# tobiashepp/torch-mednet

Hardware: AMD Instinct MI355X
Metric: 128^3 patches/sec training, 3D U-Net 32-base-ch (higher is better)
Workload: dtype bf16; 1 GPU; ResidualUNet3D f_maps=[32, 64, 128, 256] 4-class, 128^3 patches, batch 4/GPU, fwd+DiceLoss+bwd+allreduce+Adam (BASELINE config 2); global_batch=4, parallelism=dp1, graph_replay=False, gradient_exchange=none (1 rank)

## Files before the change

### include/mednet_hip.h

```cpp
#ifndef MEDNET_HIP_H
#define MEDNET_HIP_H
#include <stddef.h>
#include <stdint.h>
#ifdef __cplusplus
extern "C" {
#endif

typedef void* mednet_stream;

enum { MEDNET_F32 = 0, MEDNET_BF16 = 1,
       MEDNET_F16 = 2,
       MEDNET_U8 = 3,
       MEDNET_I64 = 4,
       MEDNET_I16 = 5   };
enum { MEDNET_NDHWC = 0, MEDNET_NCDHW = 1 };
enum { MEDNET_ACT_NONE = 0, MEDNET_ACT_RELU = 1, MEDNET_ACT_LEAKY = 2, MEDNET_ACT_ELU = 3 };
enum { MEDNET_POOL_MAX = 0, MEDNET_POOL_AVG = 1 };
enum { MEDNET_ALGO_AUTO = 0, MEDNET_ALGO_DIRECT = 1, MEDNET_ALGO_MFMA = 2, MEDNET_ALGO_EXACT = 3,
       MEDNET_ALGO_EXACT_BIT = 4,
       MEDNET_ALGO_SPLITW_BIT = 8 };
enum { MEDNET_PACK_LOW = 0x100,
       MEDNET_PACK_HIGH_ONLY = 0x200 };
enum { MEDNET_REG_L2 = 0, MEDNET_REG_L1 = 1 };
enum { MEDNET_CLASS_DICE = 0, MEDNET_CLASS_CE = 1, MEDNET_CLASS_DICE_CE = 2 };
// ... 31 lines not shown
int mednet_conv3d_cm_supported(int cin, int cout, int ksize, int x_dtype, int y_dtype, int algo);
int mednet_conv3d_act_supported(int n, int d, int h, int w, int cin, int cout, int algo);
int mednet_conv3d_act_fwd(const void* x, const void* packed, void* y, int n, int d, int h, int w, int cin, int cout,
                          int act, int algo, float* gn_partial, int dtype, mednet_stream stream);
int mednet_conv3d_dgrad_add(const void* dy, const void* packed, const void* add, void* dx, int n, int d, int h, int w,
                            int cin, int cout, int algo, int dtype, mednet_stream stream);
int mednet_conv3d_dgrad_gn_rows(int n, int d, int h, int w, int cin, int cout, int algo);
int mednet_conv3d_dgrad_gn_rows_dt(int n, int d, int h, int w, int cin, int cout, int algo, int dtype);
int mednet_conv3d_dgrad_add_supported(int n, int d, int h, int w, int cin, int cout, int algo, int dtype);
int mednet_conv3d_dgrad_gn(const void* dy, const void* packed, const void* add, void* dx, const void* gn_y,
                           const float* gn_coef, int gn_act, float* gn_partial, int n, int d, int h, int w, int cin,
                           int cout, int algo, int dtype, mednet_stream stream);
int mednet_head_dgrad_gn_rows(int n, int d, int h, int w, int cin, int dtype);
int mednet_head_dgrad_gn(const void* dy, const void* packed, void* dx, const void* gn_y, const void* gn_z, int gn_act,
                         float* gn_partial, int n, int d, int h, int w, int cin, int cout, int dtype, mednet_stream stream);
int mednet_convt3d_dgrad_gn_rows(int n, int d, int h, int w, int cin, int cout, int dtype, int algo);
int mednet_convt3d_dgrad_gn(const void* dy, const void* packed, void* dx, const void* gn_y, const void* gn_z, int gn_act,
                            float* gn_partial, int n, int d, int h, int w, int cin, int cout, int dtype, int algo,
                            mednet_stream stream);
int mednet_pool2_bwd_gn_rows(int n, int d, int h, int w, int c, int dtype);
int mednet_pool2_bwd_gn(const void* dy, const void* x, const void* add, void* dx, const void* gn_y, int gn_act,
                        float* gn_partial, int n, int d, int h, int w, int c, int mode, int dtype, mednet_stream stream);
size_t mednet_conv3d_wgrad_ws_bytes(int n, int d, int h, int w, int cin, int cout, int ksize, int workgroups);
int mednet_conv3d_wgrad_coresident(int n, int d, int h, int w, int cin, int cout, int ksize, int x_dtype, int dy_dtype, int algo);
int mednet_conv3d_wgrad_plan(int n, int d, int h, int w, int cin, int cout, int dtype, int workgroups, int* out10);
int mednet_conv3d_wgrad_c1_gn_supported(int cout, int x_dtype, int dtype);
int mednet_conv3d_wgrad_c1_gn(const void* x, const void* dz, const void* y, const float* coef, const float* bcoef, float* dw,
                              int n, int d, int h, int w, int cout, int act, int x_dtype, int dtype, void* ws, size_t ws_bytes,
                              mednet_stream stream);
int mednet_conv3d_wgrad_cm_gn_supported(int cin, int cout, int x_dtype, int dtype);
int mednet_conv3d_wgrad_cm_plan(int n, int d, int h, int w, int cin, int cout, int dtype, int gn, int* out4);
int mednet_conv3d_wgrad_cm_gn(const void* x, int x_layout, const void* dz, const void* y, const float* coef, const float* bcoef,
                              float* dw, int n, int d, int h, int w, int cin, int cout, int act, int x_dtype, int dtype, void* ws,
                              size_t ws_bytes, mednet_stream stream);
int mednet_conv3d_wgrad(const void* x, const void* dy, float* dw, float* dbias, int n, int d, int h, int w,
                        int cin, int cout, int ksize, int x_dtype, int x_layout, int dy_dtype, int dy_layout,
                        int algo, int workgroups, void* ws, size_t ws_bytes, mednet_stream stream);

int mednet_convt3d_fwd(const void* x, const void* packed, const float* bias, const void* skip, void* y, int n,
                       int d, int h, int w, int cin, int cout, int x_dtype, int y_dtype, int algo,
                       mednet_stream stream);
int mednet_convt3d_dgrad(const void* dy, const void* packed, void* dx, int n, int d, int h, int w, int cin,
                         int cout, int dy_dtype, int dx_dtype, int algo, mednet_stream stream);
size_t mednet_convt3d_wgrad_ws_bytes(int n, int d, int h, int w, int cin, int cout, int workgroups);
int mednet_convt3d_wgrad(const void* x, const void* dy, float* dw, float* dbias, int n, int d, int h, int w,
                         int cin, int cout, int x_dtype, int dy_dtype, int algo, int workgroups, void* ws,
                         size_t ws_bytes, mednet_stream stream);

size_t mednet_gn_ws_bytes(int n, int c, size_t spatial);
int mednet_gn_stats(const void* x, const float* gamma, const float* beta, float* stats, float* coef, int n,
                    size_t spatial, int c, int groups, float eps, int dtype, void* ws, size_t ws_bytes,
                    mednet_stream stream);
int mednet_gn_finalize(const float* partial, int chunks, const float* gamma, const float* beta, float* stats,
                       float* coef, int n, size_t spatial, int c, int groups, float eps, void* ws, size_t ws_bytes,
                       mednet_stream stream);
int mednet_gn_act_fwd(const void* x, const float* coef, const void* residual, void* z, int n, size_t spatial,
                      int c, int act, int x_dtype, int z_dtype, mednet_stream stream);
int mednet_gn_act_bwd(const void* dz, const void* dz2, const void* x, const void* z, const float* coef,
                      const float* stats, const float* gamma, void* dx, void* dres, float* dgamma, float* dbeta, int n,
                      size_t spatial, int c, int groups, int act, int in_act, int dtype, void* ws, size_t ws_bytes,
                      mednet_stream stream);
int mednet_gn_act_bwd_fused(const void* dz, const void* x, const float* coef, const float* stats, const float* gamma,
                            const float* partial, int rows, void* dx, float* dgamma, float* dbeta, int n,
                            size_t spatial, int c, int groups, int act, int in_act, int dtype, void* ws, size_t ws_bytes,
                            mednet_stream stream);
int mednet_gn_bwd_coefficients(const float* stats, const float* gamma, const float* partial, int rows, float* bcoef,
                               float* dgamma, float* dbeta, int n, size_t spatial, int c, int groups, void* ws,
                               size_t ws_bytes, mednet_stream stream);
int mednet_gn_act_bwd_fused_res(const void* dz, const void* x, const void* z, const float* coef, const float* stats,
                                const float* gamma, const float* fused_partial, int rows, void* dx, void* dres,
                                float* dgamma, float* dbeta, int n, size_t spatial, int c, int groups, int act, int dtype,
                                void* ws, size_t ws_bytes, mednet_stream stream);
int mednet_gn_act_bwd_fused_res_pool(const void* dy_pool, const void* skip_grad, const void* x, const void* z, const float* stats,
                                     const float* gamma, const float* fused_partial, int rows, void* dx, void* dres, float* dgamma,
                                     float* dbeta, int n, int d, int h, int w, int c, int groups, int act, int pool_mode, int dtype,
                                     void* ws, size_t ws_bytes, mednet_stream stream);
int mednet_gn_act_bwd_fused_res_head_supported(int c, int cout, int dtype, int label_dtype);
int mednet_gn_act_bwd_fused_res_head(const float* logits, const void* labels, int label_dtype, int64_t label_stride_n,
                                     const void* packed, const float* weight, const float* saved, const float* dloss, float eps,
                                     int sigmoid, int ignore_index, int class_kind, int cout, const void* x, const void* z,
                                     const float* stats, const float* gamma, const float* fused_partial, int rows, void* dx, void* dres,
                                     float* dgamma, float* dbeta, int n, size_t spatial, int c, int groups, int act, int dtype, void* ws,
                                     size_t ws_bytes, mednet_stream stream);
int mednet_bn_stats(const void* x, const float* gamma, const float* beta, float* running_mean, float* running_var,
                    long long* num_batches_tracked, float momentum, float* stats, float* coef, int n, size_t spatial, int c,
                    float eps, int dtype, void* ws, size_t ws_bytes, mednet_stream stream);
int mednet_bn_eval_coef(const float* running_mean, const float* running_var, const float* gamma, const float* beta, float* stats,
                        float* coef, int n, int c, float eps, mednet_stream stream);
int mednet_bn_act_bwd(const void* dz, const void* x, const void* z, const float* coef, const float* stats, const float* gamma,
                      void* dx, void* dres, float* dgamma, float* dbeta, int n, size_t spatial, int c, int act, int in_act,
                      int frozen, int dtype, void* ws, size_t ws_bytes, mednet_stream stream);
int mednet_bn_act_bwd_fused(const void* dz, const void* x, const float* coef, const float* stats, const float* gamma,
                            const float* partial, int rows, void* dx, float* dgamma, float* dbeta, int n, size_t spatial, int c,
                            int act, int in_act, int frozen, int dtype, void* ws, size_t ws_bytes, mednet_stream stream);

int mednet_act_fwd(const void* x, void* z, size_t count, int act, int dtype, mednet_stream stream);
int mednet_act_bwd(const void* dz, const void* z, void* dx, size_t count, int act, int dtype,
                   mednet_stream stream);
int mednet_add(const void* a, const void* b, void* out, size_t count, int dtype, mednet_stream stream);

int mednet_pool2_fwd(const void* x, void* y, int n, int d, int h, int w, int c, int mode, int dtype,
                     mednet_stream stream);
int mednet_gn_act_pool_supported(int d, int h, int w, int c, int dtype);
int mednet_gn_act_pool_fwd(const void* x, const float* coef, const void* residual, void* z, void* pooled, int n, int d, int h,
                           int w, int c, int act, int mode, int dtype, mednet_stream stream);
int mednet_pool2_bwd(const void* dy, const void* x, const void* add, void* dx, int n, int d, int h, int w, int c,
                     int mode, int dtype, mednet_stream stream);
int mednet_pool2_bwd_act(const void* dy, const void* x, const void* add, int add_channels, void* dx, int n, int d, int h, int w, int c,
                         int mode, int in_act, int dtype, mednet_stream stream);

int mednet_upcat_fwd(const void* enc, const void* x, void* out, int n, int d, int h, int w, int c_enc, int xd,
                     int xh, int xw, int c_x, int dtype, mednet_stream stream);
int mednet_upcat_stats_chunks(int n, int d, int h, int w, int c_enc, int c_x, int dtype);
int mednet_upcat_fwd_stats(const void* enc, const void* x, void* out, float* partial, int n, int d, int h, int w, int c_enc, int xd,
                           int xh, int xw, int c_x, int dtype, mednet_stream stream);
int mednet_upcat_bwd(const void* dout, void* denc, void* dx, int n, int d, int h, int w, int c_enc, int xd, int xh,
                     int xw, int c_x, int dtype, mednet_stream stream);

size_t mednet_loss_ws_bytes(int n, int c, size_t spatial);
int mednet_dice_fwd(const float* logits, const int64_t* labels, const float* weight, float* loss, float* saved,
                    float* dice_out, int n, int c, size_t spatial, int64_t stride_n, int64_t stride_c, float eps,
                    int sigmoid, int ignore_index, void* ws, size_t ws_bytes, mednet_stream stream);
int mednet_dice_bwd(const float* logits, const int64_t* labels, const float* weight, const float* saved,
                    const float* dloss, float* dlogits, int n, int c, size_t spatial, int64_t stride_n,
                    int64_t stride_c, float eps, int sigmoid, int ignore_index, mednet_stream stream);
int mednet_dice_fwd_lt(const float* logits, const void* labels, int label_dtype, int64_t label_stride_n, const float* weight,
                       float* loss, float* saved, float* dice_out, int n, int c, size_t spatial, int64_t stride_n,
                       int64_t stride_c, float eps, int sigmoid, int ignore_index, void* ws, size_t ws_bytes, mednet_stream stream);
int mednet_dice_bwd_lt(const float* logits, const void* labels, int label_dtype, int64_t label_stride_n, const float* weight,
                       const float* saved, const float* dloss, float* dlogits, int n, int c, size_t spatial, int64_t stride_n,
                       int64_t stride_c, float eps, int sigmoid, int ignore_index, mednet_stream stream);
size_t mednet_dice_ce_ws_bytes(int n, int c, size_t spatial);
int mednet_dice_ce_fwd_lt(const float* logits, const void* labels, int label_dtype, int64_t label_stride_n, const float* weight,
                          float* loss, float* saved, float* dice_out, int n, int c, size_t spatial, int64_t stride_n,
                          int64_t stride_c, float eps, void* ws, size_t ws_bytes, mednet_stream stream);
int mednet_dice_ce_bwd_lt(const float* logits, const void* labels, int label_dtype, int64_t label_stride_n, const float* weight,
                          const float* saved, const float* dloss, float* dlogits, int n, int c, size_t spatial, int64_t stride_n,
                          int64_t stride_c, float eps, mednet_stream stream);
int mednet_head_dice_supported(int cin, int cout, int dtype, int label_dtype);
size_t mednet_head_dice_ws_bytes(int n, size_t spatial, int cin, int cout);
int mednet_head_dice_gn_rows(int n, size_t spatial, int cin);
int mednet_head_dice_fwd(const void* z, const void* packed, const float* bias, const void* labels, int label_dtype,
                         int64_t label_stride_n, const float* weight, float* logits, float* loss, float* saved, int n,
                         size_t spatial, int cin, int cout, float eps, int sigmoid, int ignore_index, int z_dtype, void* ws,
                         size_t ws_bytes, mednet_stream stream);
int mednet_head_dice_bwd(const float* logits, const void* labels, int label_dtype, int64_t label_stride_n, const void* packed,
                         const float* weight, const float* saved, const float* dloss, void* dz, const void* gn_y, const void* z,
                         int gn_act, float* gn_partial, float* dw, float* dbias, int n, size_t spatial, int cin, int cout,
                         float eps, int sigmoid, int ignore_index, int z_dtype, void* ws, size_t ws_bytes, mednet_stream stream);
int mednet_head_dice_bwd_sums(const float* logits, const void* labels, int label_dtype, int64_t label_stride_n, const void* packed,
                              const float* weight, const float* saved, const float* dloss, const void* gn_y, const void* z,
                              int gn_act, float* gn_partial, float* dw, float* dbias, int n, size_t spatial, int cin, int cout,
                              float eps, int sigmoid, int ignore_index, int z_dtype, void* ws, size_t ws_bytes, mednet_stream stream);

int mednet_head_landmark_supported(int cin, int nh, int ncls, int dtype, size_t spatial);
size_t mednet_head_landmark_ws_bytes(int n, size_t spatial, int nh, int ncls);
int mednet_head_landmark_gn_rows(size_t spatial);
int mednet_head_landmark_fwd(const void* z, const void* packed, const float* bias, const void* heatmaps, int64_t heatmap_stride_n,
                             const void* labels, int64_t label_stride_n, const float* class_weight, const float* reg_weight,
                             float* logits, float* class_loss, float* reg_loss, float* saved, int n, size_t spatial, int cin, int nh,
                             int ncls, int kind, float eps, int sigmoid, int ignore_index, int z_dtype, void* ws, size_t ws_bytes,
                             mednet_stream stream);
int mednet_head_landmark_bwd(const void* z, const void* packed, const float* bias, const void* heatmaps, int64_t heatmap_stride_n,
                             const void* labels, int64_t label_stride_n, const float* class_weight, const float* reg_weight,
                             const float* saved, const float* dclass_loss, const float* dreg_loss, void* dz, const void* gn_y,
                             int gn_act, float* gn_partial, float* dw, float* dbias, int n, size_t spatial, int cin, int nh, int ncls,
                             int kind, float eps, int sigmoid, int ignore_index, int z_dtype, void* ws, size_t ws_bytes,
                             mednet_stream stream);
int mednet_head_ce_supported(int cin, int cout, int dtype, int label_dtype);
size_t mednet_head_ce_ws_bytes(int n, size_t spatial, int cin, int cout);
int mednet_head_ce_gn_rows(int n, size_t spatial, int cin);
int mednet_head_ce_fwd(const void* z, const void* packed, const float* bias, const void* labels, int label_dtype,
                       int64_t label_stride_n, const float* weight, float* logits, float* loss, float* saved, int n, size_t spatial,
                       int cin, int cout, int ignore_index, int z_dtype, void* ws, size_t ws_bytes, mednet_stream stream);
int mednet_head_ce_bwd(const float* logits, const void* labels, int label_dtype, int64_t label_stride_n, const void* packed,
                       const float* weight, const float* saved, const float* dloss, void* dz, const void* gn_y, const void* z,
                       int gn_act, float* gn_partial, float* dw, float* dbias, int n, size_t spatial, int cin, int cout,
                       int ignore_index, int z_dtype, void* ws, size_t ws_bytes, mednet_stream stream);
int mednet_head_ce_bwd_sums(const float* logits, const void* labels, int label_dtype, int64_t label_stride_n, const void* packed,
                            const float* weight, const float* saved, const float* dloss, const void* gn_y, const void* z, int gn_act,
                            float* gn_partial, float* dw, float* dbias, int n, size_t spatial, int cin, int cout, int ignore_index,
                            int z_dtype, void* ws, size_t ws_bytes, mednet_stream stream);
int mednet_head_dice_ce_supported(int cin, int cout, int dtype, int label_dtype);
size_t mednet_head_dice_ce_ws_bytes(int n, size_t spatial, int cin, int cout);
int mednet_head_dice_ce_gn_rows(int n, size_t spatial, int cin);
int mednet_head_dice_ce_fwd(const void* z, const void* packed, const float* bias, const void* labels, int label_dtype,
                            int64_t label_stride_n, const float* weight, float* logits, float* loss, float* saved, int n,
                            size_t spatial, int cin, int cout, float eps, int sigmoid, int ignore_index, int z_dtype, void* ws,
                            size_t ws_bytes, mednet_stream stream);
int mednet_head_dice_ce_bwd(const float* logits, const void* labels, int label_dtype, int64_t label_stride_n, const void* packed,
                            const float* weight, const float* saved, const float* dloss, void* dz, const void* gn_y, const void* z,
                            int gn_act, float* gn_partial, float* dw, float* dbias, int n, size_t spatial, int cin, int cout,
                            float eps, int sigmoid, int ignore_index, int z_dtype, void* ws, size_t ws_bytes, mednet_stream stream);
int mednet_head_dice_ce_bwd_sums(const float* logits, const void* labels, int label_dtype, int64_t label_stride_n, const void* packed,
                                 const float* weight, const float* saved, const float* dloss, const void* gn_y, const void* z,
                                 int gn_act, float* gn_partial, float* dw, float* dbias, int n, size_t spatial, int cin, int cout,
                                 float eps, int sigmoid, int ignore_index, int z_dtype, void* ws, size_t ws_bytes, mednet_stream stream);
int mednet_head_landmark_cls_fwd(const void* z, const void* packed, const float* bias, const void* heatmaps, int64_t heatmap_stride_n,
                                 const void* labels, int64_t label_stride_n, const float* class_weight, const float* reg_weight,
                                 float* logits, float* class_loss, float* reg_loss, float* saved, float* dice_metric, int n,
                                 size_t spatial, int cin, int nh, int ncls, int kind, int class_kind, float eps, int sigmoid,
                                 int ignore_index, int z_dtype, void* ws, size_t ws_bytes, mednet_stream stream);
int mednet_head_landmark_cls_bwd(const void* z, const void* packed, const float* bias, const void* heatmaps, int64_t heatmap_stride_n,
                                 const void* labels, int64_t label_stride_n, const float* class_weight, const float* reg_weight,
                                 const float* saved, const float* dclass_loss, const float* dreg_loss, void* dz, const void* gn_y,
                                 int gn_act, float* gn_partial, float* dw, float* dbias, int n, size_t spatial, int cin, int nh,
                                 int ncls, int kind, int class_kind, float eps, int sigmoid, int ignore_index, int z_dtype, void* ws,
                                 size_t ws_bytes, mednet_stream stream);
int mednet_head_seg_supported(int cin, int ncls, int dtype, int label_dtype, size_t spatial);
size_t mednet_head_seg_ws_bytes(int n, size_t spatial, int ncls);
int mednet_head_seg_gn_rows(size_t spatial);
int mednet_head_seg_fwd(const void* z, const void* packed, const float* bias, const void* labels, int64_t label_stride_n,
                        const float* class_weight, float* logits, float* loss, float* saved, int n, size_t spatial, int cin,
                        int ncls, int class_kind, float eps, int sigmoid, int ignore_index, int z_dtype, void* ws, size_t ws_bytes,
                        mednet_stream stream);
int mednet_head_seg_bwd(const void* z, const void* packed, const float* bias, const void* labels, int64_t label_stride_n,
                        const float* class_weight, const float* saved, const float* dloss, void* dz, const void* gn_y, int gn_act,
                        float* gn_partial, float* dw, float* dbias, int n, size_t spatial, int cin, int ncls, int class_kind,
                        float eps, int sigmoid, int ignore_index, int z_dtype, void* ws, size_t ws_bytes, mednet_stream stream);
int mednet_ds_head_supported(int cin, int ncls, int dtype, int label_dtype, int d, int h, int w, int shift);
size_t mednet_ds_head_ws_bytes(int n, int d, int h, int w, int cin, int ncls);
int mednet_ds_head_gn_rows(int d, int h, int w, int cin, int dtype);
int mednet_ds_head_fwd(const void* z, const void* packed, const float* bias, const void* labels, int label_dtype,
                       int64_t label_stride_n, const float* class_weight, float* loss, float* saved, int n, int d, int h, int w, int D,
                       int H, int W, int shift, int cin, int ncls, int class_kind, float eps, int sigmoid, int ignore_index, int z_dtype,
                       void* ws, size_t ws_bytes, mednet_stream stream);
int mednet_ds_head_bwd(const void* z, const void* packed, const float* bias, const void* labels, int label_dtype,
                       int64_t label_stride_n, const float* class_weight, const float* saved, const float* dloss, const void* d_pass,
                       void* dz, const void* gn_y, int gn_act, float* gn_partial, float* dw, float* dbias, int n, int d, int h, int w,
                       int D, int H, int W, int shift, int cin, int ncls, int class_kind, float eps, int sigmoid, int ignore_index,
                       int z_dtype, void* ws, size_t ws_bytes, mednet_stream stream);
int mednet_ce_fwd(const float* logits, const int64_t* labels, const float* weight, float* loss, float* saved,
                  int n, int c, size_t spatial, int64_t stride_n, int64_t stride_c, int ignore_index, void* ws,
                  size_t ws_bytes, mednet_stream stream);
int mednet_ce_bwd(const float* logits, const int64_t* labels, const float* weight, const float* saved,
                  const float* dloss, float* dlogits, int n, int c, size_t spatial, int64_t stride_n,
// ... 117 lines not shown
```

### torch-mednet_amd/csrc/conv.h

```cpp
#pragma once
#include <type_traits>

#include "common.h"

namespace mednet {

enum { MAP_CONV = 0, MAP_CT_FWD = 1, MAP_CT_DG = 2 };

struct ConvGeom {
  int n, od, oh, ow;
  int id, ih, iw;
  int k, m;
  int ks;
  int in_planar, out_planar;
};

struct WgradGeom {
  int n, ad, ah, aw;
  int bd, bh, bw;
  int ka, kb, ks, stride2;
  int a_planar, b_planar;
  size_t chunk;
};


template <int MAP>
int launch_direct(const void* x, const float* P, const float* bias, const void* skip, void* y, const ConvGeom& g,
                  int x_dtype, int y_dtype, hipStream_t s);
size_t wgrad_direct_ws_bytes(size_t nvox, int ka, int kb, int ks);
int launch_wgrad_direct(const void* A, const void* B, float* dw, WgradGeom g, int a_dtype, int b_dtype, void* ws,
                        size_t ws_bytes, hipStream_t s);
size_t channel_sum_ws_bytes(int n, size_t spatial, int c);
int launch_channel_sum(const void* x, float* out, int n, size_t spatial, int c, int planar, int dtype, void* ws,
                       size_t ws_bytes, hipStream_t s);
bool head_dgrad_supported(int cin, int cout, int ksize, int x_dtype, int x_layout, int y_layout);
int launch_head_dgrad(const void* dy, const float* Pb, void* dz, int n, size_t spatial, int m, int k, int out_dtype,
                      hipStream_t s);
int head_dgrad_gn_rows(size_t spatial, int k, int dtype);
int launch_head_dgrad_gn(const void* dy, const float* Pb, void* dz, const void* gy, const void* gz, int act, float* partial,
                         int n, size_t spatial, int m, int k, int dtype, hipStream_t s);
bool head_vox_supported(int k);
int launch_head_fwd_vox(const void* z, const float* Pb, const float* bias, float* y, int n, size_t spatial, int k, int m,
                        int z_dtype, hipStream_t s);
bool wgrad_1x1_supported(int cin, int cout, int ksize, int x_layout, int dy_layout, int dy_dtype);
size_t wgrad_1x1_ws_bytes(int n, size_t spatial, int cin, int cout);
int launch_wgrad_1x1(const void* z, const void* dy, float* dw, int n, size_t spatial, int cin, int cout, int z_dtype,
                     void* ws, size_t ws_bytes, hipStream_t s);
bool wgrad_c1_supported(int cin, int cout, int ksize, int x_layout, int dy_layout);
size_t wgrad_c1_ws_bytes(int n, int d, int h, int w, int cout);
bool wgrad_c1_gn_supported(int cout, int x_dtype, int dtype);
int launch_wgrad_c1_gn(const void* x, const void* dz, const void* y, const float* coef, const float* bcoef, int act, float* dw,
                       int n, int d, int h, int w, int cout, int x_dtype, int dtype, void* ws, size_t ws_bytes, hipStream_t s);
int launch_wgrad_c1(const void* x, const void* dy, float* dw, int n, int d, int h, int w, int cout, int x_dtype,
                    int dy_dtype, void* ws, size_t ws_bytes, hipStream_t s, bool split_bf16 = false);
bool wgrad_cm_supported(int cin, int cout, int ksize, int x_dtype, int dy_dtype, int dy_layout);
bool wgrad_cm_gn_supported(int cin, int cout, int x_dtype, int dtype);
size_t wgrad_cm_ws_bytes(int n, int d, int h, int w, int cin, int cout);
int wgrad_cm_plan(int n, int d, int h, int w, int cin, int cout, int dtype, bool gn, int* out4);
int launch_wgrad_cm(const void* x, int x_layout, const void* dz, const void* y, const float* coef, const float* bcoef, int act,
                    float* dw, int n, int d, int h, int w, int cin, int cout, int dtype, void* ws, size_t ws_bytes, hipStream_t s);
int launch_pack_f32(const float* w, float* Pf, float* Pb, int cin, int cout, int T, int transposed_src, hipStream_t s);

int launch_hm_finalize(const float* partial, const float* cweight, float* loss, int n, int c, int nblocks, size_t spatial,
                       hipStream_t s);
int launch_dice_finalize(const float* partial, const float* weight, float* loss, float* saved, int c, int nblocks, float eps,
                         hipStream_t s, float* dice_out = nullptr);
int launch_ce_finalize(const float* partial, float* loss, float* saved, int nblocks, hipStream_t s);
int launch_dice_ce_finalize(const float* partial, const float* partial_ce, const float* weight, float* loss, float* saved, int c,
                            int nblocks, float eps, hipStream_t s, float* dice_out = nullptr);
int launch_class_finalize(int kind, const float* dice_partial, const float* ce_partial, const float* weight, float* loss, float* saved,
                          int c, int rows, float eps, hipStream_t s);
inline int launch_class_finalize(int kind, const float* partial, const float* weight, float* loss, float* saved, int c, int rows,
                                 float eps, hipStream_t s) {
  const float* ce_partial = kind == MEDNET_CLASS_DICE_CE ? partial + (size_t)rows * c * 2 : partial;
  return launch_class_finalize(kind, partial, ce_partial, weight, loss, saved, c, rows, eps, s);
}

template <class F>
inline void for_class_kind(int ce, F&& f) {
  if (ce == MEDNET_CLASS_DICE_CE) f(std::integral_constant<int, MEDNET_CLASS_DICE_CE>{});
  else if (ce) f(std::integral_constant<int, MEDNET_CLASS_CE>{});
  else f(std::integral_constant<int, MEDNET_CLASS_DICE>{});
}
#define MEDNET_CLASS_KIND_NAME(ce, STEM, DIR) ((ce) == MEDNET_CLASS_DICE_CE ? STEM "_dice_ce" DIR : (ce) ? STEM "_ce" DIR : STEM DIR)

#include "conv_mfma_decl.inc"
inline const float* head_weights_f32(const void* packed, int cin, int cout) {
  return (const float*)((const char*)packed + pack_layout(cin, cout, 1).f32_bwd);
}

bool conv_f32_mfma_enabled();
int launch_conv_f32_mfma(const void* x, const float* P, const float* bias, void* y, int n, int d, int h, int w, int k, int m,
                         hipStream_t s);
int launch_convt_dgrad_f32_mfma(const void* dy, const float* Pb, void* dx, int n, int d, int h, int w, int cin, int cout,
                                hipStream_t s);
int launch_convt_fwd_f32_mfma(const void* x, const float* Pf, const float* bias, const void* skip, void* y, int n, int d, int h,
                              int w, int cin, int cout, hipStream_t s);
size_t wgrad_f32_mfma_ws_bytes(int n, int d, int h, int w, int ka, int kb, int stride2);
int launch_wgrad_f32_mfma(const void* x, const void* dy, float* dw, int n, int d, int h, int w, int cin, int cout, void* ws,
                          size_t ws_bytes, hipStream_t s);
int launch_convt_wgrad_f32_mfma(const void* x, const void* dy, float* dw, int n, int d, int h, int w, int cin, int cout, void* ws,
                                size_t ws_bytes, hipStream_t s);

bool conv_x3_enabled();
bool conv_x3_supported(int cin, int cout, int ksize);
bool conv_x3_fits(int d, int h, int w, int c);
int conv_x3_stats_rows(int n, int d, int h, int w, int cout);
int launch_conv_x3(const void* x, const void* sec_hi, size_t lo_delta, const float* bias, void* y, int n, int d, int h, int w, int k,
                   int m, float* stats, hipStream_t s);
bool conv_c1_x3_supported(int cin, int cout, int ksize);
int conv_c1_x3_stats_rows(int d, int h, int w);
int launch_conv_c1_x3(const void* x, const float* w_pf, const float* bias, void* y, int n, int d, int h, int w, int cout,
                      float* stats, hipStream_t s);
int launch_conv_x3_dgrad(const void* dy, const void* sec_hi, size_t lo_delta, void* dx, int n, int d, int h, int w, int k, int m,
                         const void* add, const void* gn_y, const float* gn_coef, int gn_act, float* gn_partial, hipStream_t s);
int launch_convt_dgrad_x3(const void* dy, const void* sec_hi, size_t lo_delta, void* dx, int n, int d, int h, int w, int cin,
                          int cout, hipStream_t s);
int launch_convt_fwd_x3(const void* x, const void* sec_hi, size_t lo_delta, const float* bias, const void* skip, void* y, int n,
                        int d, int h, int w, int cin, int cout, hipStream_t s);
size_t wgrad_x3_ws_bytes(int n, int d, int h, int w, int cin, int cout, int workgroups);
bool wgrad_c1_x3_supported(int cout, int x_dtype, int dy_dtype);
int wgrad_c1_x3_blocks(int n, int d, int h, int w);
int launch_wgrad_c1_x3(const void* x, const void* dy, float* part, int n, int d, int h, int w, hipStream_t s);
int launch_wgrad_x3(const void* x, const void* dy, float* dw, int n, int d, int h, int w, int cin, int cout, void* ws,
                    size_t ws_bytes, hipStream_t s, int workgroups);

size_t convt_wgrad_x3_ws_bytes(int n, int d, int h, int w, int cin, int cout, int workgroups);
int launch_convt_wgrad_x3(const void* x, const void* dy, float* dw, int n, int d, int h, int w, int cin, int cout, void* ws,
                          size_t ws_bytes, hipStream_t s, int workgroups);

}
```

### torch-mednet_amd/csrc/head_loss.hip

```cpp
#include "common.h"
#include "conv.h"
#include "loss_blocks.inc"

namespace mednet {

constexpr int HL_BLOCK_VOX = 256 * 8;
constexpr int HL_MAXC = 4;
constexpr int HL_VPT = 32;

template <typename T>
struct Raw8;
template <>
struct Raw8<bf16> {
  bf16x8 r;
  __device__ __forceinline__ void load(const bf16* p, size_t i) { r = *reinterpret_cast<const bf16x8*>(p + i); }
  __device__ __forceinline__ float at(int j) const { return (float)r[j]; }
};
template <>
struct Raw8<f16> {
  f16x8 r;
  __device__ __forceinline__ void load(const f16* p, size_t i) { r = *reinterpret_cast<const f16x8*>(p + i); }
  __device__ __forceinline__ float at(int j) const { return (float)r[j]; }
};
template <>
struct Raw8<float> {
  f32x4 a, b;
  __device__ __forceinline__ void load(const float* p, size_t i) {
    a = *reinterpret_cast<const f32x4*>(p + i);
    b = *reinterpret_cast<const f32x4*>(p + i + 4);
  }
  __device__ __forceinline__ float at(int j) const { return j < 4 ? a[j] : b[j - 4]; }
};

template <typename TI, int K, typename TL, int KIND = MEDNET_CLASS_DICE>
__global__ __launch_bounds__(256) void head_dice_fwd_kernel(const TI* __restrict__ z, const float* __restrict__ Pb ,
                                                            const float* __restrict__ bias, const TL* __restrict__ lab,
                                                            int64_t lab_sn, float* __restrict__ y, float* __restrict__ partial,
                                                            size_t spatial, int m, int sigmoid, int ignore,
                                                            const float* __restrict__ cw = nullptr) {
  __shared__ float scratch[4];
  const int n = blockIdx.y;
  ClassSums<HL_MAXC> sums;
  const size_t v0 = (size_t)blockIdx.x * HL_BLOCK_VOX;
  for (int it = 0; it < 8; ++it) {
    const size_t v = v0 + (size_t)it * 256 + threadIdx.x;
    if (v < spatial) {
      float zv[K];
#pragma unroll
      for (int q = 0; q < K / 8; ++q) {
        const F8 t = ld8(z, ((size_t)n * spatial + v) * K + q * 8);
#pragma unroll
        for (int j = 0; j < 8; ++j) zv[q * 8 + j] = t.v[j];
      }
      const int yl = label_at(lab, (size_t)n * lab_sn + v, ignore);
      float lg[HL_MAXC];
#pragma unroll
      for (int i = 0; i < HL_MAXC; ++i) {
        lg[i] = 0.f;
        if (i < m) {
          float s0 = bias ? bias[i] : 0.f, s1 = 0.f;
#pragma unroll
          for (int j = 0; j < K; j += 2) {
            s0 = fmaf(zv[j], Pb[(size_t)i * K + j], s0);
            s1 = fmaf(zv[j + 1], Pb[(size_t)i * K + j + 1], s1);
          }
          lg[i] = s0 + s1;
          y[((size_t)n * m + i) * spatial + v] = lg[i];
        }
      }
      class_fwd_voxel<KIND, HL_MAXC>(sums, [&](int k) { return lg[k]; }, yl, m, sigmoid, ignore, cw);
    }
  }
  class_fwd_writeout<KIND, HL_MAXC>(sums, partial, m, scratch);
}

template <typename TO, int K, typename TL, bool FOLD = false, int KIND = MEDNET_CLASS_DICE, bool STORE = true>
__global__ __launch_bounds__(256, (sizeof(TO) == 2 && !FOLD) ? 3 : 2) void head_dice_bwd_kernel(const float* __restrict__ lgs, const TL* __restrict__ lab, int64_t lab_sn,
                                                            const float* __restrict__ Pb , const float* __restrict__ weight,
                                                            const float* __restrict__ saved, const float* __restrict__ dloss,
                                                            float eps, int sigmoid, int ignore, TO* __restrict__ dz,
                                                            const TO* __restrict__ gy , const TO* __restrict__ gz, int act,
                                                            float* __restrict__ gn_partial , float* __restrict__ wpart,
                                                            size_t spatial, int m) {
  constexpr int CG = K / 8, VPW = 256 / CG;
  const int n = blockIdx.y;
  const int cgi = threadIdx.x % CG, vi = threadIdx.x / CG;
  float wreg[HL_MAXC][8];
#pragma unroll
  for (int i = 0; i < HL_MAXC; ++i)
#pragma unroll
    for (int j = 0; j < 8; ++j) wreg[i][j] = i < m ? Pb[(size_t)i * K + cgi * 8 + j] : 0.f;
  const float go = *dloss;
  std::conditional_t<KIND == MEDNET_CLASS_DICE_CE, ClassCoefLds<HL_MAXC>, ClassCoefRegs<HL_MAXC>> coef;
  if constexpr (KIND == MEDNET_CLASS_DICE_CE) {
    __shared__ float hk_s[3 * HL_MAXC];
    coef.row = hk_s;
    if (threadIdx.x < HL_MAXC) coef.template fill<KIND>(threadIdx.x, m, weight, saved, eps, go);
    __syncthreads();
  } else {
    coef.template fill<KIND>(m, weight, saved, eps, go);
  }
  float ss[8], sq[8], wacc[HL_MAXC][8], bacc[HL_MAXC];
#pragma unroll
  for (int j = 0; j < 8; ++j) ss[j] = sq[j] = 0.f;
#pragma unroll
  for (int i = 0; i < HL_MAXC; ++i) {
    bacc[i] = 0.f;
#pragma unroll
    for (int j = 0; j < 8; ++j) wacc[i][j] = 0.f;
  }
  const size_t v0 = (size_t)blockIdx.x * (VPW * HL_VPT) + vi;
  for (int it = 0; it < HL_VPT; it += 2) {
    const size_t v = v0 + (size_t)it * VPW;
    if (v >= spatial) break;
    const size_t vb = v + VPW;
    const bool hb = (it + 1 < HL_VPT) && vb < spatial;
    const size_t vbs = hb ? vb : v;
    float la[HL_MAXC], lb[HL_MAXC];
    [[maybe_unused]] float oa = 0.f, ob = 0.f;
    if constexpr (CG == 4) {
      const int cq = threadIdx.x & 3;
      oa = cq < m ? lgs[((size_t)n * m + cq) * spatial + v] : 0.f;
      ob = cq < m ? lgs[((size_t)n * m + cq) * spatial + vbs] : 0.f;
      static_assert(HL_MAXC == 4, "one class per lane of a quad");
    } else {
#pragma unroll
      for (int i = 0; i < HL_MAXC; ++i) {
        la[i] = i < m ? lgs[((size_t)n * m + i) * spatial + v] : 0.f;
        lb[i] = i < m ? lgs[((size_t)n * m + i) * spatial + vbs] : 0.f;
      }
    }
    const int ya = label_at(lab, (size_t)n * lab_sn + v, ignore), yb = label_at(lab, (size_t)n * lab_sn + vbs, ignore);
    const size_t rowa = ((size_t)n * spatial + v) * K + cgi * 8, rowb = ((size_t)n * spatial + vbs) * K + cgi * 8;
    Raw8<TO> zva, zvb, yva, yvb;
    zva.load(gz, rowa);
    zvb.load(gz, rowb);
    if (!STORE || gy) {
      yva.load(gy, rowa);
      yvb.load(gy, rowb);
    } else {
      yva = zva;
      yvb = zvb;
    }
    if constexpr (KIND == MEDNET_CLASS_DICE_CE) asm volatile("" : "+v"(coef.off));
    float (&da)[HL_MAXC] = la, (&db)[HL_MAXC] = lb;
    if constexpr (CG == 4) {
      class_logit_grad_quad<KIND>(da, db, oa, ob, ya, yb, m, sigmoid, ignore, coef);
    } else {
      class_logit_grad<KIND, HL_MAXC>(da, ya, m, sigmoid, ignore, coef);
// ... 20 lines not shown
      for (int j = 0; j < 8; ++j) {
        za[j] = zva.at(j);
        zb[j] = zvb.at(j);
      }
      act_grad_n<8>(t.v, za, act);
      act_grad_n<8>(u.v, zb, act);
    }
    if constexpr (STORE) {
      st8(dz, rowa, t);
      if (hb) st8(dz, rowb, u);
    }
    if (!FOLD && (!STORE || gy)) {
      float za[8], zb[8];
#pragma unroll
      for (int j = 0; j < 8; ++j) {
        za[j] = zva.at(j);
        zb[j] = zvb.at(j);
      }
      act_grad_n<8>(t.v, za, act);
      act_grad_n<8>(u.v, zb, act);
#pragma unroll
      for (int j = 0; j < 8; ++j) {
        ss[j] += t.v[j] + u.v[j];
        sq[j] = fmaf(u.v[j], yvb.at(j), fmaf(t.v[j], yva.at(j), sq[j]));
      }
    }
  }
  const int lane = threadIdx.x & 63, wave = threadIdx.x >> 6;
  const size_t wrow = ((size_t)n * gridDim.x + blockIdx.x) * 4 + wave;
  if (gn_partial) {
    float* out = gn_partial + wrow * K * 2 + cgi * 16;
#pragma unroll
    for (int j = 0; j < 8; ++j) {
      const float a = lane_class_sum<CG>(ss[j]), b = lane_class_sum<CG>(sq[j]);
      if (lane < CG) {
        out[2 * j] = a;
        out[2 * j + 1] = b;
      }
    }
  }
  float* wout = wpart + wrow * ((size_t)m * K + m);
#pragma unroll
  for (int i = 0; i < HL_MAXC; ++i) {
    if (i < m) {
#pragma unroll
      for (int j = 0; j < 8; ++j) {
        const float a = lane_class_sum<CG>(wacc[i][j]);
        if (lane < CG) wout[(size_t)i * K + cgi * 8 + j] = a;
      }
      const float b = lane_class_sum<CG>(bacc[i]);
      if (lane == 0) wout[(size_t)m * K + i] = b;
    }
  }
}

constexpr int HL_WF_GROUPS = 128;
__global__ __launch_bounds__(192) void head_dice_wfinal1_kernel(const float* __restrict__ wpart, double* __restrict__ part2, int rows,
                                                                int width) {
  const int per = (rows + HL_WF_GROUPS - 1) / HL_WF_GROUPS;
  const int r0 = blockIdx.x * per, r1 = r0 + per < rows ? r0 + per : rows;
  for (int e = threadIdx.x; e < width; e += 192) {
    double s0 = 0.0, s1 = 0.0, s2 = 0.0, s3 = 0.0;
    int r = r0;
    for (; r + 3 < r1; r += 4) {
      s0 += (double)wpart[(size_t)r * width + e];
      s1 += (double)wpart[(size_t)(r + 1) * width + e];
      s2 += (double)wpart[(size_t)(r + 2) * width + e];
      s3 += (double)wpart[(size_t)(r + 3) * width + e];
    }
    for (; r < r1; ++r) s0 += (double)wpart[(size_t)r * width + e];
    part2[(size_t)blockIdx.x * width + e] = (s0 + s1) + (s2 + s3);
  }
}
__global__ __launch_bounds__(192) void head_dice_wfinal2_kernel(const double* __restrict__ part2, float* __restrict__ dw,
                                                                float* __restrict__ dbias, int width, int mk) {
  for (int e = threadIdx.x; e < width; e += 192) {
    double s = 0.0;
    for (int g = 0; g < HL_WF_GROUPS; ++g) s += part2[(size_t)g * width + e];
    if (e < mk) dw[e] = (float)s;
    else if (dbias) dbias[e - mk] = (float)s;
  }
}

static inline unsigned hl_fwd_blocks(size_t spatial) { return (unsigned)((spatial + HL_BLOCK_VOX - 1) / HL_BLOCK_VOX); }
static inline unsigned hl_bwd_blocks(size_t spatial, int k) {
  const size_t per_wg = (size_t)(256 / (k / 8)) * HL_VPT;
  return (unsigned)((spatial + per_wg - 1) / per_wg);
}

}

using namespace mednet;

extern "C" int mednet_head_dice_supported(int cin, int cout, int dtype, int label_dtype) {
  return (cin == 16 || cin == 32 || cin == 64) && cout >= 1 && cout <= HL_MAXC && dtype_ok(dtype) &&
         (label_dtype == MEDNET_U8 || label_dtype == MEDNET_I64) && tuning_option("head_loss_fuse", 1);
}
extern "C" size_t mednet_head_dice_ws_bytes(int n, size_t spatial, int cin, int cout) {
  const size_t fwd = ((size_t)n * hl_fwd_blocks(spatial) * cout * 2 + 64) * sizeof(float);
  const size_t width = (size_t)cout * cin + cout;
  const size_t bwd = ((size_t)n * hl_bwd_blocks(spatial, cin) * 4 * width + 64) * sizeof(float) + (size_t)HL_WF_GROUPS * width * sizeof(double) + 16;
  return fwd > bwd ? fwd : bwd;
}
extern "C" int mednet_head_dice_gn_rows(int n, size_t spatial, int cin) {
  (void)n;
  return 4 * (int)hl_bwd_blocks(spatial, cin);
}
extern "C" size_t mednet_head_dice_ce_ws_bytes(int n, size_t spatial, int cin, int cout) {
  const size_t fwd = ((size_t)n * hl_fwd_blocks(spatial) * ((size_t)cout * 2 + 2) + 64) * sizeof(float);
  const size_t bwd = mednet_head_dice_ws_bytes(n, spatial, cin, cout);
  return fwd > bwd ? fwd : bwd;
}

template <int KIND>
static int head_loss_fwd(const char* what, const void* z, const void* packed, const float* bias, const void* labels, int label_dtype,
                         int64_t label_stride_n, const float* weight, float* logits, float* loss, float* saved, int n, size_t spatial,
                         int cin, int cout, float eps, int sigmoid, int ignore_index, int z_dtype, void* ws, size_t ws_bytes,
                         mednet_stream stream) {
  MEDNET_REQUIRE(mednet_head_dice_supported(cin, cout, z_dtype, label_dtype), MEDNET_E_UNSUPPORTED,
                 "%s: %d -> %d classes, dtype %d, labels %d", what, cin, cout, z_dtype, label_dtype);
  MEDNET_REQUIRE(n > 0 && spatial > 0 && z && packed && labels && logits && loss && saved, MEDNET_E_SHAPE, "%s: bad arguments", what);
  const size_t need = KIND == MEDNET_CLASS_DICE_CE ? mednet_head_dice_ce_ws_bytes(n, spatial, cin, cout) : mednet_head_dice_ws_bytes(n, spatial, cin, cout);
  MEDNET_REQUIRE(ws_bytes >= need, MEDNET_E_WORKSPACE, "%s: workspace too small", what);
  const float* Pb = head_weights_f32(packed, cin, cout);
  hipStream_t s = (hipStream_t)stream;
  const unsigned nb = hl_fwd_blocks(spatial);
  float* partial = (float*)ws;
  const dim3 grid(nb, n);
#define HF(TI_, K_, TL_) hipLaunchKernelGGL((head_dice_fwd_kernel<TI_, K_, TL_, KIND>), grid, dim3(256), 0, s, (const TI_*)z, Pb, bias, (const TL_*)labels, label_stride_n, logits, partial, spatial, cout, sigmoid, ignore_index, KIND != MEDNET_CLASS_DICE ? weight : nullptr)
#define HF_L(TI_, K_) do { if (label_dtype == MEDNET_U8) HF(TI_, K_, uint8_t); else HF(TI_, K_, int64_t); } while (0)
#define HF_K(TI_) do { if (cin == 16) HF_L(TI_, 16); else if (cin == 32) HF_L(TI_, 32); else HF_L(TI_, 64); } while (0)
  if (z_dtype == MEDNET_F32) HF_K(float);
  else if (z_dtype == MEDNET_BF16) HF_K(bf16);
  else HF_K(f16);
#undef HF_K
#undef HF_L
#undef HF
  int rc = check_launch(what);
  if (rc) return rc;
  return launch_class_finalize(KIND, partial, weight, loss, saved, cout, (int)(nb * n), eps, s);
}

template <int KIND>
static int head_loss_bwd(const char* what, const float* logits, const void* labels, int label_dtype, int64_t label_stride_n,
                         const void* packed, const float* weight, const float* saved, const float* dloss, void* dz, const void* gn_y,
                         const void* z, int gn_act, float* gn_partial, float* dw, float* dbias, int n, size_t spatial, int cin, int cout,
                         float eps, int sigmoid, int ignore_index, int z_dtype, void* ws, size_t ws_bytes, mednet_stream stream,
                         bool store = true) {
  MEDNET_REQUIRE(mednet_head_dice_supported(cin, cout, z_dtype, label_dtype), MEDNET_E_UNSUPPORTED,
                 "%s: %d -> %d classes, dtype %d, labels %d", what, cin, cout, z_dtype, label_dtype);
  MEDNET_REQUIRE(n > 0 && spatial > 0 && logits && labels && packed && saved && dloss && (dz || !store) && z && dw, MEDNET_E_SHAPE, "%s: bad arguments", what);
  MEDNET_REQUIRE(store || (cin == 32 && z_dtype != MEDNET_F32), MEDNET_E_UNSUPPORTED, "%s: 32 features in 16-bit storage, not %d in dtype %d", what, cin, z_dtype);
  MEDNET_REQUIRE(store || (gn_y && gn_partial), MEDNET_E_SHAPE, "%s: gn_y and gn_partial are required", what);
  MEDNET_REQUIRE((gn_y == nullptr) == (gn_partial == nullptr), MEDNET_E_SHAPE, "%s: gn_y and gn_partial go together", what);
  const size_t need = KIND == MEDNET_CLASS_DICE_CE ? mednet_head_dice_ce_ws_bytes(n, spatial, cin, cout) : mednet_head_dice_ws_bytes(n, spatial, cin, cout);
  MEDNET_REQUIRE(ws_bytes >= need, MEDNET_E_WORKSPACE, "%s: workspace too small", what);
  const float* Pb = head_weights_f32(packed, cin, cout);
  hipStream_t s = (hipStream_t)stream;
  const unsigned nb = hl_bwd_blocks(spatial, cin);
  float* wpart = (float*)ws;
  const dim3 grid(nb, n);
  const bool fold = gn_y == nullptr && gn_act != MEDNET_ACT_NONE;
#define HB_(TO_, K_, TL_, F_) hipLaunchKernelGGL((head_dice_bwd_kernel<TO_, K_, TL_, F_, KIND>), grid, dim3(256), 0, s, logits, (const TL_*)labels, label_stride_n, Pb, weight, saved, dloss, eps, sigmoid, ignore_index, (TO_*)dz, (const TO_*)gn_y, (const TO_*)z, gn_act, gn_partial, wpart, spatial, cout)
#define HB(TO_, K_, TL_) do { if (fold) HB_(TO_, K_, TL_, true); else HB_(TO_, K_, TL_, false); } while (0)
#define HB_L(TO_, K_) do { if (label_dtype == MEDNET_U8) HB(TO_, K_, uint8_t); else HB(TO_, K_, int64_t); } while (0)
#define HB_K(TO_) do { if (cin == 16) HB_L(TO_, 16); else if (cin == 32) HB_L(TO_, 32); else HB_L(TO_, 64); } while (0)
#define HB_S(TO_, TL_) hipLaunchKernelGGL((head_dice_bwd_kernel<TO_, 32, TL_, false, KIND, false>), grid, dim3(256), 0, s, logits, (const TL_*)labels, label_stride_n, Pb, weight, saved, dloss, eps, sigmoid, ignore_index, (TO_*)nullptr, (const TO_*)gn_y, (const TO_*)z, gn_act, gn_partial, wpart, spatial, cout)
#define HB_SL(TO_) do { if (label_dtype == MEDNET_U8) HB_S(TO_, uint8_t); else HB_S(TO_, int64_t); } while (0)
  if (!store) {
    if (z_dtype == MEDNET_BF16) HB_SL(bf16);
    else HB_SL(f16);
  } else if (z_dtype == MEDNET_F32) HB_K(float);
  else if (z_dtype == MEDNET_BF16) HB_K(bf16);
  else HB_K(f16);
#undef HB_SL
#undef HB_S
#undef HB_K
#undef HB_L
#undef HB_
#undef HB
  int rc = check_launch(what);
  if (rc) return rc;
  const int width = cout * cin + cout, rows = (int)(n * nb * 4);
  double* part2 = (double*)((char*)ws + (((size_t)rows * width + 64) * sizeof(float) + 7) / 8 * 8);
  hipLaunchKernelGGL(head_dice_wfinal1_kernel, dim3(HL_WF_GROUPS), dim3(192), 0, s, wpart, part2, rows, width);
  hipLaunchKernelGGL(head_dice_wfinal2_kernel, dim3(1), dim3(192), 0, s, part2, dw, dbias, width, cout * cin);
  return check_launch("head_dice_wfinal");
}

extern "C" int mednet_head_dice_fwd(const void* z, const void* packed, const float* bias, const void* labels, int label_dtype,
                                    int64_t label_stride_n, const float* weight, float* logits, float* loss, float* saved, int n,
                                    size_t spatial, int cin, int cout, float eps, int sigmoid, int ignore_index, int z_dtype,
                                    void* ws, size_t ws_bytes, mednet_stream stream) {
  return head_loss_fwd<MEDNET_CLASS_DICE>("head_dice_fwd", z, packed, bias, labels, label_dtype, label_stride_n, weight, logits, loss, saved, n, spatial,
                              cin, cout, eps, sigmoid, ignore_index, z_dtype, ws, ws_bytes, stream);
}

extern "C" int mednet_head_dice_bwd(const float* logits, const void* labels, int label_dtype, int64_t label_stride_n,
                                    const void* packed, const float* weight, const float* saved, const float* dloss, void* dz,
                                    const void* gn_y, const void* z, int gn_act, float* gn_partial, float* dw, float* dbias, int n,
                                    size_t spatial, int cin, int cout, float eps, int sigmoid, int ignore_index, int z_dtype,
                                    void* ws, size_t ws_bytes, mednet_stream stream) {
  return head_loss_bwd<MEDNET_CLASS_DICE>("head_dice_bwd", logits, labels, label_dtype, label_stride_n, packed, weight, saved, dloss, dz, gn_y, z, gn_act,
                              gn_partial, dw, dbias, n, spatial, cin, cout, eps, sigmoid, ignore_index, z_dtype, ws, ws_bytes, stream);
}

extern "C" int mednet_head_dice_bwd_sums(const float* logits, const void* labels, int label_dtype, int64_t label_stride_n,
                                         const void* packed, const float* weight, const float* saved, const float* dloss,
                                         const void* gn_y, const void* z, int gn_act, float* gn_partial, float* dw, float* dbias, int n,
                                         size_t spatial, int cin, int cout, float eps, int sigmoid, int ignore_index, int z_dtype,
                                         void* ws, size_t ws_bytes, mednet_stream stream) {
  return head_loss_bwd<MEDNET_CLASS_DICE>("head_dice_bwd_sums", logits, labels, label_dtype, label_stride_n, packed, weight, saved, dloss, nullptr, gn_y, z,
                              gn_act, gn_partial, dw, dbias, n, spatial, cin, cout, eps, sigmoid, ignore_index, z_dtype, ws, ws_bytes, stream, false);
}

extern "C" int mednet_head_ce_supported(int cin, int cout, int dtype, int label_dtype) {
  return mednet_head_dice_supported(cin, cout, dtype, label_dtype);
}
extern "C" size_t mednet_head_ce_ws_bytes(int n, size_t spatial, int cin, int cout) {
  return mednet_head_dice_ws_bytes(n, spatial, cin, cout);
}
extern "C" int mednet_head_ce_gn_rows(int n, size_t spatial, int cin) { return mednet_head_dice_gn_rows(n, spatial, cin); }

extern "C" int mednet_head_ce_fwd(const void* z, const void* packed, const float* bias, const void* labels, int label_dtype,
                                  int64_t label_stride_n, const float* weight, float* logits, float* loss, float* saved, int n,
                                  size_t spatial, int cin, int cout, int ignore_index, int z_dtype, void* ws, size_t ws_bytes,
                                  mednet_stream stream) {
  return head_loss_fwd<MEDNET_CLASS_CE>("head_ce_fwd", z, packed, bias, labels, label_dtype, label_stride_n, weight, logits, loss, saved, n, spatial,
                             cin, cout, 0.f, 0, ignore_index, z_dtype, ws, ws_bytes, stream);
}

extern "C" int mednet_head_ce_bwd(const float* logits, const void* labels, int label_dtype, int64_t label_stride_n, const void* packed,
                                  const float* weight, const float* saved, const float* dloss, void* dz, const void* gn_y, const void* z,
                                  int gn_act, float* gn_partial, float* dw, float* dbias, int n, size_t spatial, int cin, int cout,
                                  int ignore_index, int z_dtype, void* ws, size_t ws_bytes, mednet_stream stream) {
  return head_loss_bwd<MEDNET_CLASS_CE>("head_ce_bwd", logits, labels, label_dtype, label_stride_n, packed, weight, saved, dloss, dz, gn_y, z, gn_act,
                             gn_partial, dw, dbias, n, spatial, cin, cout, 0.f, 0, ignore_index, z_dtype, ws, ws_bytes, stream);
}

extern "C" int mednet_head_ce_bwd_sums(const float* logits, const void* labels, int label_dtype, int64_t label_stride_n, const void* packed,
                                       const float* weight, const float* saved, const float* dloss, const void* gn_y, const void* z,
                                       int gn_act, float* gn_partial, float* dw, float* dbias, int n, size_t spatial, int cin, int cout,
                                       int ignore_index, int z_dtype, void* ws, size_t ws_bytes, mednet_stream stream) {
  return head_loss_bwd<MEDNET_CLASS_CE>("head_ce_bwd_sums", logits, labels, label_dtype, label_stride_n, packed, weight, saved, dloss, nullptr, gn_y, z, gn_act,
                             gn_partial, dw, dbias, n, spatial, cin, cout, 0.f, 0, ignore_index, z_dtype, ws, ws_bytes, stream, false);
}

extern "C" int mednet_head_dice_ce_supported(int cin, int cout, int dtype, int label_dtype) {
  return mednet_head_dice_supported(cin, cout, dtype, label_dtype);
}
extern "C" int mednet_head_dice_ce_gn_rows(int n, size_t spatial, int cin) { return mednet_head_dice_gn_rows(n, spatial, cin); }

extern "C" int mednet_head_dice_ce_fwd(const void* z, const void* packed, const float* bias, const void* labels, int label_dtype,
                                       int64_t label_stride_n, const float* weight, float* logits, float* loss, float* saved, int n,
                                       size_t spatial, int cin, int cout, float eps, int sigmoid, int ignore_index, int z_dtype,
                                       void* ws, size_t ws_bytes, mednet_stream stream) {
  MEDNET_REQUIRE(sigmoid == 0 && ignore_index == MEDNET_NO_IGNORE, MEDNET_E_UNSUPPORTED,
                 "head_dice_ce_fwd: Dice + cross-entropy is a softmax form without ignore_index");
  return head_loss_fwd<MEDNET_CLASS_DICE_CE>("head_dice_ce_fwd", z, packed, bias, labels, label_dtype, label_stride_n, weight, logits, loss, saved, n,
                                   spatial, cin, cout, eps, 0, MEDNET_NO_IGNORE, z_dtype, ws, ws_bytes, stream);
}

extern "C" int mednet_head_dice_ce_bwd(const float* logits, const void* labels, int label_dtype, int64_t label_stride_n,
                                       const void* packed, const float* weight, const float* saved, const float* dloss, void* dz,
                                       const void* gn_y, const void* z, int gn_act, float* gn_partial, float* dw, float* dbias, int n,
                                       size_t spatial, int cin, int cout, float eps, int sigmoid, int ignore_index, int z_dtype,
                                       void* ws, size_t ws_bytes, mednet_stream stream) {
  MEDNET_REQUIRE(sigmoid == 0 && ignore_index == MEDNET_NO_IGNORE, MEDNET_E_UNSUPPORTED,
                 "head_dice_ce_bwd: Dice + cross-entropy is a softmax form without ignore_index");
  return head_loss_bwd<MEDNET_CLASS_DICE_CE>("head_dice_ce_bwd", logits, labels, label_dtype, label_stride_n, packed, weight, saved, dloss, dz, gn_y, z,
                                   gn_act, gn_partial, dw, dbias, n, spatial, cin, cout, eps, 0, MEDNET_NO_IGNORE, z_dtype, ws, ws_bytes,
                                   stream);
}

extern "C" int mednet_head_dice_ce_bwd_sums(const float* logits, const void* labels, int label_dtype, int64_t label_stride_n,
                                            const void* packed, const float* weight, const float* saved, const float* dloss,
                                            const void* gn_y, const void* z, int gn_act, float* gn_partial, float* dw, float* dbias,
                                            int n, size_t spatial, int cin, int cout, float eps, int sigmoid, int ignore_index,
                                            int z_dtype, void* ws, size_t ws_bytes, mednet_stream stream) {
  MEDNET_REQUIRE(sigmoid == 0 && ignore_index == MEDNET_NO_IGNORE, MEDNET_E_UNSUPPORTED,
// ... 6 lines not shown
```

### torch-mednet_amd/csrc/loss_blocks.inc

```
#pragma once

namespace mednet {

template <typename TL>
__device__ __forceinline__ int label_at(const TL* __restrict__ lab, size_t i, int ignore) {
  const int64_t y = (int64_t)lab[i];
  if (y == (int64_t)(int)y) return (int)y;
  return ignore == -1 ? -2 : -1;
}

template <int MAXC>
__device__ __forceinline__ void cl_keep_branch() {
  if constexpr (MAXC > 4) asm volatile("");
}

template <int MAXC, class Z>
__device__ __forceinline__ float cl_load_max(float* p, Z&& logit, int c, int y, float& zy) {
  float mx = -INFINITY;
#pragma unroll
  for (int k = 0; k < MAXC; ++k)
    if (k < c) {
      cl_keep_branch<MAXC>();
      p[k] = logit(k);
      mx = fmaxf(mx, p[k]);
      if (k == y) zy = p[k];
    }
  return mx;
}
template <int MAXC>
__device__ __forceinline__ float cl_exp_sum(float* p, int c, float mx) {
  float den = 0.f;
#pragma unroll
  for (int k = 0; k < MAXC; ++k)
    if (k < c) {
      cl_keep_branch<MAXC>();
      p[k] = expf(p[k] - mx);
      den += p[k];
    }
  return den;
}
template <int MAXC, class Z>
__device__ __forceinline__ void cl_probs(float* p, Z&& logit, int c, int sigmoid) {
  if (sigmoid) {
#pragma unroll
    for (int k = 0; k < MAXC; ++k)
      if (k < c) p[k] = 1.f / (1.f + expf(-logit(k)));
  } else {
    [[maybe_unused]] float zy;
    const float mx = cl_load_max<MAXC>(p, logit, c, -1, zy);
    const float den = cl_exp_sum<MAXC>(p, c, mx);
    const float inv = 1.f / den;
#pragma unroll
    for (int k = 0; k < MAXC; ++k)
      if (k < c) p[k] *= inv;
  }
}

template <int MAXC>
struct ClassSums {
  float I[MAXC], D[MAXC];
  float num = 0.f, den = 0.f;
  bool bad = false;
  __device__ __forceinline__ ClassSums() {
#pragma unroll
    for (int k = 0; k < MAXC; ++k) I[k] = D[k] = 0.f;
  }
};

template <int MAXC>
__device__ __forceinline__ void cl_dice_terms_masked(ClassSums<MAXC>& a, const float* p, int y, int c, int ignore) {
#pragma unroll
  for (int k = 0; k < MAXC; ++k)
    if (k < c) {
      cl_keep_branch<MAXC>();
      const float t = (k == y) ? 1.f : 0.f;
      const float m = (ignore != MEDNET_NO_IGNORE && t == (float)ignore) ? 0.f : 1.f;
      a.I[k] = fmaf(p[k] * m, t * m, a.I[k]);
      a.D[k] += (p[k] + t) * m;
    }
}
template <int MAXC>
__device__ __forceinline__ void cl_dice_terms(ClassSums<MAXC>& a, float* p, float inv, int y, int c) {
#pragma unroll
  for (int k = 0; k < MAXC; ++k)
    if (k < c) {
      cl_keep_branch<MAXC>();
      p[k] *= inv;
      const float t = (k == y) ? 1.f : 0.f;
      a.I[k] = fmaf(p[k], t, a.I[k]);
      a.D[k] += p[k] + t;
    }
}
template <int MAXC>
__device__ __forceinline__ void cl_ce_term(ClassSums<MAXC>& a, const float* __restrict__ weight, int y, float mx, float s, float zy) {
  const float w = weight ? weight[y] : 1.f;
  a.num = fmaf(w, (mx + logf(s)) - zy, a.num);
  a.den += w;
}

template <int KIND, int MAXC, class Z>
__device__ __forceinline__ void class_fwd_voxel(ClassSums<MAXC>& a, Z&& logit, int y, int c, int sigmoid, int ignore,
                                                const float* __restrict__ weight) {
  const bool ok = (unsigned)y < (unsigned)c;
  if constexpr (KIND == MEDNET_CLASS_CE) {
    if (y != ignore && !ok) a.num = __builtin_nanf("");
    if (y != ignore && ok) {
      float mx = -INFINITY, zy = 0.f;
#pragma unroll
      for (int k = 0; k < MAXC; ++k)
        if (k < c) {
          cl_keep_branch<MAXC>();
          const float z = logit(k);
          mx = fmaxf(mx, z);
          if (k == y) zy = z;
        }
      float s = 0.f;
#pragma unroll
      for (int k = 0; k < MAXC; ++k)
        if (k < c) s += expf(logit(k) - mx);
      cl_ce_term<MAXC>(a, weight, y, mx, s, zy);
    }
  } else {
    float p[MAXC];
    a.bad |= !ok;
    if constexpr (KIND == MEDNET_CLASS_DICE_CE) {
      float zy = 0.f;
      const float mx = cl_load_max<MAXC>(p, logit, c, y, zy);
      const float den = cl_exp_sum<MAXC>(p, c, mx);
      const float inv = 1.f / den;
      cl_dice_terms<MAXC>(a, p, inv, y, c);
      if (ok) cl_ce_term<MAXC>(a, weight, y, mx, den, zy);
    } else {
      cl_probs<MAXC>(p, logit, c, sigmoid);
      cl_dice_terms_masked<MAXC>(a, p, y, c, ignore);
    }
  }
}

// ... 152 lines not shown
```

### torch-mednet_amd/csrc/norm_act.hip

```cpp
#include "common.h"
#include "conv.h"
#include "loss_blocks.inc"

#include <type_traits>

#ifndef GN_NT
#define GN_NT 1
#endif
#ifndef GN_WAVES
#define GN_WAVES 3
#endif
namespace mednet {

template <int VEC>
struct Cols {
  int cols, rows, col, row;
  bool active;
  __device__ __forceinline__ Cols(int c) {
    cols = c / VEC;
    rows = 256 / cols;
    active = (int)threadIdx.x < rows * cols;
    col = threadIdx.x % cols;
    row = threadIdx.x / cols;
  }
// ... 196 lines not shown
    b += (double)p0.y;
  }
  a = wave_sum((a + a1) + (a2 + a3));
  b = wave_sum((b + b1) + (b2 + b3));
  if (threadIdx.x == 0) {
    const int g = cc / (c / groups);
    const double mean = stats[((size_t)n * groups + g) * 2], rstd = stats[((size_t)n * groups + g) * 2 + 1];
    csum[((size_t)n * c + cc) * 2] = (float)a;
    csum[((size_t)n * c + cc) * 2 + 1] = (float)(rstd * (b - mean * a));
  }
}

__global__ __launch_bounds__(1024) void gn_finalize_kernel(const float* __restrict__ partial,
                                                           const float* __restrict__ gamma,
                                                           const float* __restrict__ beta, float* __restrict__ stats,
                                                           float* __restrict__ coef, int c, int groups, int chunks,
                                                           double count, float eps, const void* __restrict__ pivot_x,
                                                           size_t sample_stride, int dtype) {
  __shared__ double sh[2][16];
  const int n = blockIdx.x / groups, g = blockIdx.x % groups;
  const int cg = c / groups, lane = threadIdx.x & 63, wv = threadIdx.x >> 6;
  const int nt = (int)blockDim.x, nwv = nt >> 6;
  double s = 0.0, q = 0.0;
  const float* base = partial + (size_t)n * chunks * c * 2 + (size_t)g * cg * 2;
  const size_t row = (size_t)c * 2;
  if (cg % 2 == 0) {
    auto add_row = [&](const float* p, double& ss, double& qq) {
      for (int i = 0; i < cg / 2; ++i) {
        const f32x4 v = *reinterpret_cast<const f32x4*>(p + 4 * i);
        ss += (double)v[0] + (double)v[2];
        qq += (double)v[1] + (double)v[3];
      }
    };
    double s1 = 0.0, q1 = 0.0, s2 = 0.0, q2 = 0.0, s3 = 0.0, q3 = 0.0;
    int ch = threadIdx.x;
    for (; ch + 3 * nt < chunks; ch += 4 * nt) {
      add_row(base + (size_t)ch * row, s, q);
      add_row(base + (size_t)(ch + nt) * row, s1, q1);
      add_row(base + (size_t)(ch + 2 * nt) * row, s2, q2);
      add_row(base + (size_t)(ch + 3 * nt) * row, s3, q3);
    }
    for (; ch < chunks; ch += nt) add_row(base + (size_t)ch * row, s, q);
    s = (s + s1) + (s2 + s3);
    q = (q + q1) + (q2 + q3);
  } else {
    for (int ch = threadIdx.x; ch < chunks; ch += nt) {
      const float* p = base + (size_t)ch * row;
      for (int i = 0; i < cg; ++i) {
        s += (double)p[2 * i];
        q += (double)p[2 * i + 1];
      }
    }
  }
  s = wave_sum(s);
  q = wave_sum(q);
  if (lane == 0) {
    sh[0][wv] = s;
    sh[1][wv] = q;
  }
  __syncthreads();
  s = q = 0.0;
  for (int k = 0; k < nwv; ++k) {
    s += sh[0][k];
    q += sh[1][k];
  }
  const double ms = s / count;
  const double mean = (double)pivot_of(pivot_x, (size_t)n * sample_stride + (size_t)g * cg, dtype) + ms;
  double var = q / count - ms * ms;
  if (var < 0.0) var = 0.0;
  const float rstd = (float)(1.0 / sqrt(var + (double)eps));
  if (threadIdx.x == 0) {
    stats[((size_t)n * groups + g) * 2] = (float)mean;
    stats[((size_t)n * groups + g) * 2 + 1] = rstd;
  }
  for (int i = threadIdx.x; i < cg; i += nt) {
    const int cc = g * cg + i;
    const float ga = gamma ? gamma[cc] : 1.f, be = beta ? beta[cc] : 0.f;
    const float a = ga * rstd;
    coef[((size_t)n * c + cc) * 2] = a;
    coef[((size_t)n * c + cc) * 2 + 1] = be - (float)mean * a;
  }
}

template <typename TX, typename TZ, int VEC>
__global__ __launch_bounds__(256) void gn_act_fwd_kernel(const TX* __restrict__ x, const float* __restrict__ coef,
                                                         const TZ* __restrict__ res, TZ* __restrict__ z,
                                                         size_t spatial, int c, int act, size_t chunk_vox) {
  const Cols<VEC> L(c);
  if (!L.active) return;
  const int n = blockIdx.y;
  const size_t v0 = (size_t)blockIdx.x * chunk_vox;
  const size_t v1 = v0 + chunk_vox < spatial ? v0 + chunk_vox : spatial;
  float a[VEC], b[VEC];
#pragma unroll
  for (int k = 0; k < VEC; ++k) {
    a[k] = coef[((size_t)n * c + L.col * VEC + k) * 2];
    b[k] = coef[((size_t)n * c + L.col * VEC + k) * 2 + 1];
  }
  const size_t off = (size_t)n * spatial * c + (size_t)L.col * VEC;
  auto one = [&](const F8& xin, const F8& rin, F8& out) {
#pragma unroll
    for (int k = 0; k < VEC; ++k) {
      out.v[k] = fmaf(a[k], xin.v[k], b[k]);
      if (res) out.v[k] += rin.v[k];
    }
    act_apply_n<VEC>(out.v, act);
  };
  size_t v = v0 + L.row;
  const size_t R = (size_t)L.rows;
  for (; v + 3 * R < v1; v += 4 * R) {
    size_t i[4];
    F8 xi[4], ri[4], zo[4];
#pragma unroll
    for (int u = 0; u < 4; ++u) i[u] = off + (v + u * R) * c;
#pragma unroll
    for (int u = 0; u < 4; ++u) xi[u] = VecIO<TX, VEC>::load(x, i[u]);
    if (res) {
#pragma unroll
      for (int u = 0; u < 4; ++u) ri[u] = VecIO<TZ, VEC>::load(res, i[u]);
    }
#pragma unroll
    for (int u = 0; u < 4; ++u) one(xi[u], ri[u], zo[u]);
#pragma unroll
    for (int u = 0; u < 4; ++u) VecIO<TZ, VEC>::store(z, i[u], zo[u]);
  }
  for (; v < v1; v += R) {
    const size_t i = off + v * c;
    const F8 xv = VecIO<TX, VEC>::load(x, i);
    F8 rv, zv;
    if (res) rv = VecIO<TZ, VEC>::load(res, i);
    one(xv, rv, zv);
    VecIO<TZ, VEC>::store(z, i, zv);
  }
}

template <typename T, int VEC>
__global__ __launch_bounds__(256, GN_WAVES) void gn_bwd_partial_kernel(const T* __restrict__ dz, const T* __restrict__ dz2,
                                                             const T* __restrict__ x, const T* __restrict__ z,
                                                             const float* __restrict__ coef,
                                                             const float* __restrict__ stats,
                                                             float* __restrict__ partial, size_t spatial, int c,
                                                             int groups, int act, size_t chunk_vox, int rpw) {
  __shared__ float lds[256 * 2 * VEC];
  const Cols<VEC> L(c);
  const int n = blockIdx.y;
  const size_t v0 = (size_t)blockIdx.x * chunk_vox;
  const size_t v1 = v0 + chunk_vox < spatial ? v0 + chunk_vox : spatial;
  float acc[2 * VEC];
#pragma unroll
  for (int k = 0; k < 2 * VEC; ++k) acc[k] = 0.f;
  if (L.active) {
    const int cg = c / groups;
    float mean[VEC], rstd[VEC], ca[VEC], cb[VEC];
#pragma unroll
    for (int k = 0; k < VEC; ++k) {
      const int g = (L.col * VEC + k) / cg;
      mean[k] = stats[((size_t)n * groups + g) * 2];
      rstd[k] = stats[((size_t)n * groups + g) * 2 + 1];
      ca[k] = z ? 0.f : coef[((size_t)n * c + L.col * VEC + k) * 2];
      cb[k] = z ? 0.f : coef[((size_t)n * c + L.col * VEC + k) * 2 + 1];
    }
    const size_t off = (size_t)n * spatial * c + (size_t)L.col * VEC;
    auto one = [&](size_t i) {
      F8 g1 = VecIO<T, VEC>::load(dz, i);
      F8 g2, zv;
      if (dz2) g2 = VecIO<T, VEC>::load(dz2, i);
      if (act != MEDNET_ACT_NONE && z) zv = VecIO<T, VEC>::load(z, i);
      const F8 xv = VecIO<T, VEC>::load(x, i);
      if (dz2) {
#pragma unroll
        for (int k = 0; k < VEC; ++k) g1.v[k] += g2.v[k];
      }
      if (z) {
        act_grad_n<VEC>(g1.v, zv.v, act);
      } else {
#pragma unroll
        for (int k = 0; k < VEC; ++k) zv.v[k] = fmaf(ca[k], xv.v[k], cb[k]);
        act_grad_pre_n<VEC>(g1.v, zv.v, act);
      }
#pragma unroll
      for (int k = 0; k < VEC; ++k) {
        const float xh = (xv.v[k] - mean[k]) * rstd[k];
        acc[2 * k] += g1.v[k];
        acc[2 * k + 1] = fmaf(g1.v[k], xh, acc[2 * k + 1]);
      }
    };
    size_t v = v0 + L.row;
    for (; v + (size_t)L.rows < v1; v += 2 * (size_t)L.rows) {
      one(off + v * c);
      one(off + (v + L.rows) * c);
// ... 562 lines not shown

template <typename T, typename TL, int KIND>
__global__ __launch_bounds__(256, GN_WAVES) void gn_bwd_apply_head_kernel(const float* __restrict__ lgs, const TL* __restrict__ lab,
                                                                          int64_t lab_sn, const float* __restrict__ Pb ,
                                                                          const float* __restrict__ weight, const float* __restrict__ saved,
                                                                          const float* __restrict__ dloss, float eps, int sigmoid, int ignore,
                                                                          int m, const T* __restrict__ x, const T* __restrict__ z,
                                                                          const float* __restrict__ bcoef, T* __restrict__ dx,
                                                                          T* __restrict__ dres, size_t spatial, int act, size_t chunk_vox,
                                                                          GnParamGrad pg) {
  constexpr int C = 32, VEC = 8, MAXC = 4, ROWS = 256 / (C / VEC);
  static_assert(sizeof(T) == 2, "16-bit storage");
  if (pg.csum && blockIdx.x == 0 && blockIdx.y == 0) {
    for (int cc = threadIdx.x; cc < C; cc += 256) {
      double a = 0.0, b = 0.0;
      for (int i = 0; i < pg.n; ++i) {
        a += (double)pg.csum[((size_t)i * C + cc) * 2];
        b += (double)pg.csum[((size_t)i * C + cc) * 2 + 1];
      }
      if (pg.dbeta) pg.dbeta[cc] = (float)a;
      if (pg.dgamma) pg.dgamma[cc] = (float)b;
    }
  }
  const int n = blockIdx.y, col = threadIdx.x & 3, row = threadIdx.x >> 2;
  const size_t v0 = (size_t)blockIdx.x * chunk_vox;
  const size_t v1 = v0 + chunk_vox < spatial ? v0 + chunk_vox : spatial;
  float k1[VEC], k2[VEC], k3[VEC], wreg[MAXC][VEC];
#pragma unroll
  for (int k = 0; k < VEC; ++k) {
    const float* o = bcoef + ((size_t)n * C + col * VEC + k) * 3;
    k1[k] = o[0];
    k2[k] = o[1];
    k3[k] = o[2];
#pragma unroll
    for (int i = 0; i < MAXC; ++i) wreg[i][k] = i < m ? Pb[(size_t)i * C + col * VEC + k] : 0.f;
  }
  const float go = *dloss;
  std::conditional_t<KIND == MEDNET_CLASS_DICE_CE, ClassCoefLds<MAXC>, ClassCoefRegs<MAXC>> coef;
  if constexpr (KIND == MEDNET_CLASS_DICE_CE) {
    __shared__ float hk_s[3 * MAXC];
    coef.row = hk_s;
    if (threadIdx.x < MAXC) coef.template fill<KIND>(threadIdx.x, m, weight, saved, eps, go);
    __syncthreads();
  } else {
    coef.template fill<KIND>(m, weight, saved, eps, go);
  }
  const size_t off = (size_t)n * spatial * C + (size_t)col * VEC;
  auto finish = [&](size_t i, F8& g1, const F8& zv, const F8& xv) {
    act_grad_n<VEC>(g1.v, zv.v, act);
    F8 o;
#pragma unroll
    for (int k = 0; k < VEC; ++k) {
      float xf = xv.v[k];
      asm volatile("" : "+v"(xf));
      o.v[k] = fmaf(k1[k], g1.v[k], fmaf(k2[k], xf, k3[k]));
      asm volatile("" : "+v"(o.v[k]));
    }
    VecIO<T, VEC>::store(dx, i, o);
    VecIO<T, VEC>::store(dres, i, g1);
  };
  auto two = [&](size_t va, size_t vb, bool hb) {
    const float oa = col < m ? lgs[((size_t)n * m + col) * spatial + va] : 0.f;
    const float ob = col < m ? lgs[((size_t)n * m + col) * spatial + vb] : 0.f;
    const int ya = label_at(lab, (size_t)n * lab_sn + va, ignore), yb = label_at(lab, (size_t)n * lab_sn + vb, ignore);
    const size_t ia = off + va * C, ib = off + vb * C;
    F8 zva, zvb;
    if (act != MEDNET_ACT_NONE) {
      zva = VecIO<T, VEC>::load(z, ia);
      zvb = VecIO<T, VEC>::load(z, ib);
    }
    const F8 xva = VecIO<T, VEC>::load_last(x, ia), xvb = VecIO<T, VEC>::load_last(x, ib);
    if constexpr (KIND == MEDNET_CLASS_DICE_CE) asm volatile("" : "+v"(coef.off));
    float da[MAXC], db[MAXC];
    class_logit_grad_quad<KIND>(da, db, oa, ob, ya, yb, m, sigmoid, ignore, coef);
    F8 ga, gb;
    head_dz_row<T, MAXC>(ga.v, da, wreg, m);
    head_dz_row<T, MAXC>(gb.v, db, wreg, m);
    finish(ia, ga, zva, xva);
    if (hb) finish(ib, gb, zvb, xvb);
  };
  size_t v = v0 + row;
  for (; v + (size_t)ROWS < v1; v += 2 * (size_t)ROWS) two(v, v + ROWS, true);
  for (; v < v1; v += ROWS) two(v, v, false);
}

__device__ __forceinline__ int nearest_src(int dst, int in, int out) {
  const float scale = (float)in / (float)out;
  const int s = (int)floorf((float)dst * scale);
  return s < in - 1 ? s : in - 1;
}
template <typename T, int VEC>
__global__ __launch_bounds__(256) void upcat_fwd_kernel(const T* __restrict__ enc, const T* __restrict__ x,
                                                        T* __restrict__ out, int n, int d, int h, int w, int ce, int xd,
                                                        int xh, int xw, int cx) {
  const int ct = ce + cx, pv = ct / VEC;
  const size_t total = (size_t)n * d * h * w * pv;
  const size_t i = (size_t)blockIdx.x * 256 + threadIdx.x;
  if (i >= total) return;
  const int cc = (int)(i % pv) * VEC;
  size_t v = i / pv;
  if (cc < ce) {
    VecIO<T, VEC>::store(out, v * ct + cc, VecIO<T, VEC>::load(enc, v * ce + cc));
    return;
  }
  const int ox = (int)(v % w);
  size_t r = v / w;
  const int oy = (int)(r % h);
  r /= h;
  const int oz = (int)(r % d);
  const int nn = (int)(r / d);
  const int sz = nearest_src(oz, xd, d), sy = nearest_src(oy, xh, h), sx = nearest_src(ox, xw, w);
  VecIO<T, VEC>::store(out, v * ct + cc,
                       VecIO<T, VEC>::load(x, ((((size_t)nn * xd + sz) * xh + sy) * xw + sx) * cx + (cc - ce)));
}
template <typename T, int VEC>
__global__ __launch_bounds__(256) void upcat_stats_fwd_kernel(const T* __restrict__ enc, const T* __restrict__ x, T* __restrict__ out,
                                                              float* __restrict__ partial, int d, int h, int w, int ce, int xd, int xh,
                                                              int xw, int cx, size_t chunk_vox) {
  __shared__ float lds[256 * 2 * VEC];
  const int ct = ce + cx;
  const Cols<VEC> L(ct);
  const int n = blockIdx.y;
  const size_t spatial = (size_t)d * h * w;
  const size_t v0 = (size_t)blockIdx.x * chunk_vox;
  const size_t v1 = v0 + chunk_vox < spatial ? v0 + chunk_vox : spatial;
  float acc[2 * VEC];
#pragma unroll
  for (int k = 0; k < 2 * VEC; ++k) acc[k] = 0.f;
  if (L.active) {
    const int cc = L.col * VEC;
    const bool from_enc = cc < ce;
    const T* src = from_enc ? enc + (size_t)n * spatial * ce + cc : x + (size_t)n * xd * xh * xw * cx + (cc - ce);
    T* dst = out + (size_t)n * spatial * ct + cc;
    auto src_index = [&](size_t v) -> size_t {
      if (from_enc) return v * ce;
      const int ox = (int)(v % w);
      const size_t r = v / w;
      const int oy = (int)(r % h), oz = (int)(r / h);
      return ((size_t)(nearest_src(oz, xd, d) * xh + nearest_src(oy, xh, h)) * xw + nearest_src(ox, xw, w)) * cx;
    };
    size_t v = v0 + L.row;
    for (; v + 3 * (size_t)L.rows < v1; v += 4 * (size_t)L.rows) {
      F8 xv[4];
#pragma unroll
      for (int u = 0; u < 4; ++u) xv[u] = VecIO<T, VEC>::load(src, src_index(v + (size_t)u * L.rows));
#pragma unroll
      for (int u = 0; u < 4; ++u) {
        VecIO<T, VEC>::store(dst, (v + (size_t)u * L.rows) * ct, xv[u]);
#pragma unroll
        for (int k = 0; k < VEC; ++k) {
          acc[2 * k] += xv[u].v[k];
          acc[2 * k + 1] = fmaf(xv[u].v[k], xv[u].v[k], acc[2 * k + 1]);
        }
      }
    }
    for (; v < v1; v += L.rows) {
      const F8 xv = VecIO<T, VEC>::load(src, src_index(v));
      VecIO<T, VEC>::store(dst, v * ct, xv);
#pragma unroll
      for (int k = 0; k < VEC; ++k) {
        acc[2 * k] += xv.v[k];
        acc[2 * k + 1] = fmaf(xv.v[k], xv.v[k], acc[2 * k + 1]);
      }
    }
  }
  float* rows = partial + ((size_t)n * gridDim.x + blockIdx.x) * ct * 2;
// ... 283 lines not shown

extern "C" int mednet_gn_act_bwd_fused_res(const void* dz, const void* x, const void* z, const float* coef, const float* stats,
                                           const float* gamma, const float* fused_partial, int rows, void* dx, void* dres,
                                           float* dgamma, float* dbeta, int n, size_t spatial, int c, int groups, int act,
                                           int dtype, void* ws, size_t ws_bytes, mednet_stream stream) {
  MEDNET_REQUIRE(z && dres, MEDNET_E_SHAPE, "gn_act_bwd_fused_res: z and dres are required");
  return gn_act_bwd_fused_impl(dz, x, z, coef, stats, gamma, fused_partial, rows, dx, dres, dgamma, dbeta, n, spatial, c, groups,
                               act, MEDNET_ACT_NONE, dtype, ws, ws_bytes, stream);
}

extern "C" int mednet_gn_act_bwd_fused_res_pool(const void* dy_pool, const void* skip_grad, const void* x, const void* z,
                                                const float* stats, const float* gamma, const float* fused_partial, int rows,
                                                void* dx, void* dres, float* dgamma, float* dbeta, int n, int d, int h, int w, int c,
                                                int groups, int act, int pool_mode, int dtype, void* ws, size_t ws_bytes,
                                                mednet_stream stream) {
  MEDNET_REQUIRE(dtype_ok(dtype), MEDNET_E_DTYPE, "gn_act_bwd_fused_res_pool: bad dtype");
  MEDNET_REQUIRE(c % groups == 0 && rows > 0 && fused_partial && dy_pool && x && z && dx && dres, MEDNET_E_SHAPE,
                 "gn_act_bwd_fused_res_pool: bad arguments");
  MEDNET_REQUIRE(d % 2 == 0 && h % 2 == 0 && w % 2 == 0 && c % 8 == 0, MEDNET_E_UNSUPPORTED,
                 "gn_act_bwd_fused_res_pool: even extents and C %% 8 == 0 (%dx%dx%d, C=%d)", d, h, w, c);
  const size_t spatial = (size_t)d * h * w;
  MEDNET_REQUIRE(ws_bytes >= mednet_gn_ws_bytes(n, c, spatial), MEDNET_E_WORKSPACE, "gn_act_bwd_fused_res_pool: workspace too small");
  const GnPlan p = gn_plan(n, spatial, c, dtype, ws);
  hipStream_t s = (hipStream_t)stream;
  GnParamGrad pg;
  const int rc = gn_bwd_coefs<true>(fused_partial, rows, stats, gamma, p.csum, p.bcoef, dgamma, dbeta, n, spatial, c, groups, 0, &pg, s);
  if (rc) return rc;
  by_type(dtype, [&](auto t) {
    using T = typename decltype(t)::type;
    constexpr int V = std::is_same<T, float>::value ? 4 : 8;
    const size_t total = (size_t)n * (d / 2) * (h / 2) * (w / 2) * (c / V);
    hipLaunchKernelGGL((gn_bwd_apply_pool_kernel<T, V>), dim3((unsigned)((total + 255) / 256)), dim3(256), 0, s, (const T*)dy_pool,
                       (const T*)skip_grad, (const T*)x, (const T*)z, p.bcoef, (T*)dx, (T*)dres, n, d, h, w, c, act, pool_mode, pg);
  });
  return check_launch("gn_bwd_apply_pool");
}

extern "C" int mednet_gn_act_bwd_fused_res_head_supported(int c, int cout, int dtype, int label_dtype) {
  return c == 32 && cout >= 1 && cout <= 4 && (dtype == MEDNET_BF16 || dtype == MEDNET_F16) &&
         (label_dtype == MEDNET_U8 || label_dtype == MEDNET_I64);
}
extern "C" int mednet_gn_act_bwd_fused_res_head(const float* logits, const void* labels, int label_dtype, int64_t label_stride_n,
                                                const void* packed, const float* weight, const float* saved, const float* dloss,
                                                float eps, int sigmoid, int ignore_index, int class_kind, int cout, const void* x,
                                                const void* z, const float* stats, const float* gamma, const float* fused_partial,
                                                int rows, void* dx, void* dres, float* dgamma, float* dbeta, int n, size_t spatial,
                                                int c, int groups, int act, int dtype, void* ws, size_t ws_bytes,
                                                mednet_stream stream) {
  MEDNET_REQUIRE(mednet_gn_act_bwd_fused_res_head_supported(c, cout, dtype, label_dtype), MEDNET_E_UNSUPPORTED,
                 "gn_act_bwd_fused_res_head: %d features -> %d classes, dtype %d, labels %d", c, cout, dtype, label_dtype);
  MEDNET_REQUIRE(class_kind == MEDNET_CLASS_DICE || class_kind == MEDNET_CLASS_CE || class_kind == MEDNET_CLASS_DICE_CE,
                 MEDNET_E_UNSUPPORTED, "gn_act_bwd_fused_res_head: class loss %d", class_kind);
  MEDNET_REQUIRE(class_kind != MEDNET_CLASS_DICE_CE || (sigmoid == 0 && ignore_index == MEDNET_NO_IGNORE), MEDNET_E_UNSUPPORTED,
                 "gn_act_bwd_fused_res_head: Dice + cross-entropy is a softmax form without ignore_index");
  MEDNET_REQUIRE(n > 0 && spatial > 0 && c % groups == 0 && rows > 0 && fused_partial && logits && labels && packed && saved && dloss &&
                     x && z && dx && dres && stats && gamma,
                 MEDNET_E_SHAPE, "gn_act_bwd_fused_res_head: bad arguments");
  MEDNET_REQUIRE(ws_bytes >= mednet_gn_ws_bytes(n, c, spatial), MEDNET_E_WORKSPACE, "gn_act_bwd_fused_res_head: workspace too small");
  const GnPlan p = gn_plan(n, spatial, c, dtype, ws);
  hipStream_t s = (hipStream_t)stream;
  GnParamGrad pg;
  const int rc = gn_bwd_coefs<true>(fused_partial, rows, stats, gamma, p.csum, p.bcoef, dgamma, dbeta, n, spatial, c, groups, 0, &pg, s);
  if (rc) return rc;
  const float* Pb = head_weights_f32(packed, c, cout);
  if (class_kind == MEDNET_CLASS_CE) eps = 0.f, sigmoid = 0;
  for_class_kind(class_kind, [&](auto kind) {
    by_type(dtype, [&](auto t) {
      using T = typename decltype(t)::type;
      if constexpr (sizeof(T) == 2) {
        auto go = [&](auto l) {
          using TL = typename decltype(l)::type;
          hipLaunchKernelGGL((gn_bwd_apply_head_kernel<T, TL, decltype(kind)::value>), p.grid, dim3(256), 0, s, logits, (const TL*)labels,
                             label_stride_n, Pb, weight, saved, dloss, eps, sigmoid, ignore_index, cout, (const T*)x, (const T*)z, p.bcoef,
                             (T*)dx, (T*)dres, spatial, act, p.chunk_vox, pg);
        };
        if (label_dtype == MEDNET_U8) go(Tag<uint8_t>{});
        else go(Tag<int64_t>{});
      }
    });
  });
  return check_launch("gn_bwd_apply_head");
}


namespace mednet {
constexpr int BN_NT = 1024;
__device__ __forceinline__ void bn_column_sums(const float* __restrict__ partial, int rows, int c, int c0, int cw, double* sha,
                                               double* shb, double& ra, double& rb) {
  const int t = threadIdx.x, i = t % cw, r0 = t / cw, rstep = BN_NT / cw;
  const float* base = partial + (size_t)(c0 + i) * 2;
  const size_t rs = (size_t)c * 2;
  constexpr int U = 8;
  double a[U], b[U];
#pragma unroll
  for (int k = 0; k < U; ++k) a[k] = b[k] = 0.0;
  int r = r0;
  for (; r + (U - 1) * rstep < rows; r += U * rstep) {
    float2 p[U];
#pragma unroll
    for (int k = 0; k < U; ++k) p[k] = *reinterpret_cast<const float2*>(base + (size_t)(r + k * rstep) * rs);
#pragma unroll
    for (int k = 0; k < U; ++k) {
      a[k] += (double)p[k].x;
      b[k] += (double)p[k].y;
    }
  }
  for (; r < rows; r += rstep) {
    const float2 p0 = *reinterpret_cast<const float2*>(base + (size_t)r * rs);
    a[0] += (double)p0.x;
    b[0] += (double)p0.y;
  }
#pragma unroll
  for (int w = 1; w < U; w *= 2) {
#pragma unroll
    for (int k = 0; k < U; k += 2 * w) {
      a[k] += a[k + w];
      b[k] += b[k + w];
    }
  }
  sha[t] = a[0];
  shb[t] = b[0];
  __syncthreads();
  ra = rb = 0.0;
  if (t < cw) {
    for (int k = 0; k < rstep; ++k) {
      ra += sha[k * cw + t];
      rb += shb[k * cw + t];
    }
  }
}
static inline int bn_cw(int c) { return c % 4 == 0 ? 4 : 1; }

__global__ __launch_bounds__(BN_NT) void bn_finalize_kernel(const float* __restrict__ partial, const float* __restrict__ gamma,
                                                            const float* __restrict__ beta, float* __restrict__ running_mean,
                                                            float* __restrict__ running_var, long long* __restrict__ num_batches,
                                                            float* __restrict__ stats, float* __restrict__ coef, int n, int c,
                                                            int cw, int rows, double count, float eps, float momentum,
                                                            const void* __restrict__ pivot_x, int dtype) {
  __shared__ double sha[BN_NT], shb[BN_NT];
  const int c0 = blockIdx.x * cw, t = threadIdx.x;
  double s, q;
  bn_column_sums(partial, rows, c, c0, cw, sha, shb, s, q);
  if (t < cw) {
    const int cc = c0 + t;
    const double ms = s / count;
    const double mean = (double)pivot_of(pivot_x, (size_t)cc, dtype) + ms;
    double var = q / count - ms * ms;
    if (var < 0.0) var = 0.0;
    const float rstd = (float)(1.0 / sqrt(var + (double)eps));
    const float ga = gamma ? gamma[cc] : 1.f, be = beta ? beta[cc] : 0.f;
    const float a = ga * rstd, b = be - (float)mean * a;
    for (int i = 0; i < n; ++i) {
      stats[((size_t)i * c + cc) * 2] = (float)mean;
      stats[((size_t)i * c + cc) * 2 + 1] = rstd;
      coef[((size_t)i * c + cc) * 2] = a;
      coef[((size_t)i * c + cc) * 2 + 1] = b;
    }
    if (running_mean) {
      const double m = (double)momentum;
      const double unbiased = count > 1.0 ? var * (count / (count - 1.0)) : var;
      running_mean[cc] = (float)((1.0 - m) * (double)running_mean[cc] + m * mean);
      running_var[cc] = (float)((1.0 - m) * (double)running_var[cc] + m * unbiased);
    }
  }
  if (num_batches && blockIdx.x == 0 && t == 0) *num_batches += 1;
}
// ... 285 lines not shown
```

### torch-mednet_amd/mednet_hip/_lib.py

```python
from __future__ import annotations

import ctypes as C
import os

import torch

_HERE = os.path.dirname(os.path.abspath(__file__))
LIB_PATH = os.environ.get("MEDNET_LIB_PATH") or os.path.join(_HERE, "libmednet_hip.so")

F32, BF16 = 0, 1
NDHWC, NCDHW = 0, 1
ACT_NONE, ACT_RELU, ACT_LEAKY, ACT_ELU = 0, 1, 2, 3
POOL_MAX, POOL_AVG = 0, 1
ALGO_AUTO, ALGO_DIRECT, ALGO_MFMA, ALGO_EXACT = 0, 1, 2, 3
ALGO_EXACT_BIT = 4
ALGO_SPLITW_BIT = 8
PACK_LOW = 0x100
PACK_HIGH_ONLY = 0x200
REG_L2, REG_L1 = 0, 1
CLASS_DICE, CLASS_CE, CLASS_DICE_CE = 0, 1, 2
PAD_CONSTANT, PAD_SYMMETRIC = 0, 1
MIP_MEAN, MIP_MAX = 0, 1
BLEND_PROBABILITIES, BLEND_LOGITS = 0, 1
INTERP_LINEAR, INTERP_NEAREST = 0, 1
BORDER_CONSTANT, BORDER_EDGE = 0, 1
F16, U8, I64 = 2, 3, 4
I16 = 5
INTENSITY_MAX_RANKS, INTENSITY_TABLE_BYTES = 8, 40
INTENSITY_ALL, INTENSITY_FIRST, INTENSITY_LAST = -1, 1, 2
INTENSITY_ZSCORE, INTENSITY_CT, INTENSITY_RESCALE, INTENSITY_PERCENTILES = 0, 1, 2, 3
NO_IGNORE = -(2 ** 31)
CC_ALL = -1

_vp, _i, _sz, _f, _i64, _dbl = C.c_void_p, C.c_int, C.c_size_t, C.c_float, C.c_int64, C.c_double

SIGNATURES = {
    "mednet_abi_version": (_i, []),
    "mednet_last_error": (C.c_char_p, []),
    "mednet_device_ok": (_i, []),
    "mednet_set_option": (_i, [C.c_char_p, _i]),
    "mednet_get_option": (_i, [C.c_char_p, _i]),
    "mednet_conv3d_pack_bytes": (_sz, [_i, _i, _i]),
    "mednet_conv3d_pack": (_i, [_vp, _vp, _i, _i, _i, _i, _vp]),
    "mednet_conv3d_pack_elt": (_i, [_vp, _vp, _i, _i, _i, _i, _i, _vp]),
    "mednet_conv3d_pack_table_bytes": (_sz, [_i]),
    "mednet_conv3d_pack_table": (_i, [_vp, _i, _vp, _vp]),
    "mednet_conv3d_pack_many": (_i, [_vp, _i, C.c_uint, _i, _vp]),
    "mednet_conv3d_stats_plan": (_i, [_i] * 9 + [_vp]),
    "mednet_conv3d_fused_stats_chunks": (_i, [_i] * 10),
    "mednet_conv3d_fwd": (_i, [_vp, _vp, _vp, _vp] + [_i] * 13 + [_vp, _vp]),
    "mednet_gn_finalize": (_i, [_vp, _i, _vp, _vp, _vp, _vp, _i, _sz, _i, _i, _f, _vp, _sz, _vp]),
    "mednet_conv3d_act_supported": (_i, [_i] * 7),
    "mednet_conv3d_act_fwd": (_i, [_vp, _vp, _vp] + [_i] * 8 + [_vp, _i, _vp]),
    "mednet_conv3d_dgrad_add": (_i, [_vp, _vp, _vp, _vp] + [_i] * 8 + [_vp]),
    "mednet_conv3d_dgrad_gn_rows": (_i, [_i] * 7),
    "mednet_conv3d_dgrad_gn_rows_dt": (_i, [_i] * 8),
    "mednet_conv3d_dgrad_add_supported": (_i, [_i] * 8),
    "mednet_conv3d_dgrad_gn": (_i, [_vp, _vp, _vp, _vp, _vp, _vp, _i, _vp] + [_i] * 8 + [_vp]),
    "mednet_gn_act_bwd_fused": (_i, [_vp] * 6 + [_i, _vp, _vp, _vp, _i, _sz, _i, _i, _i, _i, _i, _vp, _sz, _vp]),
    "mednet_gn_bwd_coefficients": (_i, [_vp, _vp, _vp, _i, _vp, _vp, _vp, _i, _sz, _i, _i, _vp, _sz, _vp]),
    "mednet_gn_act_bwd_fused_res": (_i, [_vp] * 7 + [_i, _vp, _vp, _vp, _vp, _i, _sz, _i, _i, _i, _i, _vp, _sz, _vp]),
    "mednet_gn_act_bwd_fused_res_pool": (_i, [_vp] * 7 + [_i, _vp, _vp, _vp, _vp] + [_i] * 9 + [_vp, _sz, _vp]),
    "mednet_gn_act_bwd_fused_res_head_supported": (_i, [_i] * 4),
    "mednet_gn_act_bwd_fused_res_head": (_i, [_vp, _vp, _i, _i64] + [_vp] * 4 + [_f, _i, _i, _i, _i] + [_vp] * 5 + [_i, _vp, _vp, _vp, _vp,
                                              _i, _sz, _i, _i, _i, _i, _vp, _sz, _vp]),
    "mednet_head_dgrad_gn_rows": (_i, [_i] * 6),
    "mednet_head_dgrad_gn": (_i, [_vp] * 5 + [_i, _vp] + [_i] * 7 + [_vp]),
    "mednet_pool2_bwd_gn_rows": (_i, [_i] * 6),
    "mednet_convt3d_dgrad_gn_rows": (_i, [_i] * 8),
    "mednet_convt3d_dgrad_gn": (_i, [_vp] * 5 + [_i, _vp] + [_i] * 8 + [_vp]),
    "mednet_pool2_bwd_gn": (_i, [_vp] * 5 + [_i, _vp] + [_i] * 7 + [_vp]),
    "mednet_conv3d_wgrad_ws_bytes": (_sz, [_i] * 8),
    "mednet_conv3d_wgrad_coresident": (_i, [_i] * 10),
    "mednet_conv3d_wgrad_plan": (_i, [_i] * 8 + [_vp]),
    "mednet_conv3d_wgrad_c1_gn_supported": (_i, [_i] * 3),
    "mednet_conv3d_wgrad_c1_gn": (_i, [_vp] * 6 + [_i] * 8 + [_vp, _sz, _vp]),
    "mednet_conv3d_cm_supported": (_i, [_i] * 6),
    "mednet_conv3d_wgrad_cm_gn_supported": (_i, [_i] * 4),
    "mednet_conv3d_wgrad_cm_plan": (_i, [_i] * 8 + [_vp]),
    "mednet_conv3d_wgrad_cm_gn": (_i, [_vp, _i] + [_vp] * 5 + [_i] * 9 + [_vp, _sz, _vp]),
    "mednet_conv3d_wgrad": (_i, [_vp, _vp, _vp, _vp] + [_i] * 13 + [_vp, _sz, _vp]),
    "mednet_convt3d_fwd": (_i, [_vp, _vp, _vp, _vp, _vp] + [_i] * 9 + [_vp]),
    "mednet_convt3d_dgrad": (_i, [_vp, _vp, _vp] + [_i] * 9 + [_vp]),
    "mednet_convt3d_wgrad_ws_bytes": (_sz, [_i] * 7),
    "mednet_convt3d_wgrad": (_i, [_vp, _vp, _vp, _vp] + [_i] * 10 + [_vp, _sz, _vp]),
    "mednet_gn_ws_bytes": (_sz, [_i, _i, _sz]),
    "mednet_gn_stats": (_i, [_vp, _vp, _vp, _vp, _vp, _i, _sz, _i, _i, _f, _i, _vp, _sz, _vp]),
    "mednet_gn_act_fwd": (_i, [_vp, _vp, _vp, _vp, _i, _sz, _i, _i, _i, _i, _vp]),
    "mednet_gn_act_bwd": (_i, [_vp] * 11 + [_i, _sz, _i, _i, _i, _i, _i, _vp, _sz, _vp]),
    "mednet_act_fwd": (_i, [_vp, _vp, _sz, _i, _i, _vp]),
    "mednet_act_bwd": (_i, [_vp, _vp, _vp, _sz, _i, _i, _vp]),
    "mednet_add": (_i, [_vp, _vp, _vp, _sz, _i, _vp]),
    "mednet_pool2_fwd": (_i, [_vp, _vp] + [_i] * 7 + [_vp]),
    "mednet_bn_stats": (_i, [_vp] * 6 + [_f, _vp, _vp, _i, _sz, _i, _f, _i, _vp, _sz, _vp]),
    "mednet_bn_eval_coef": (_i, [_vp] * 6 + [_i, _i, _f, _vp]),
    "mednet_bn_act_bwd": (_i, [_vp] * 10 + [_i, _sz, _i, _i, _i, _i, _i, _vp, _sz, _vp]),
    "mednet_bn_act_bwd_fused": (_i, [_vp] * 6 + [_i, _vp, _vp, _vp, _i, _sz, _i, _i, _i, _i, _i, _vp, _sz, _vp]),
    "mednet_gn_act_pool_supported": (_i, [_i] * 5),
    "mednet_gn_act_pool_fwd": (_i, [_vp] * 5 + [_i] * 8 + [_vp]),
    "mednet_pool2_bwd": (_i, [_vp, _vp, _vp, _vp] + [_i] * 7 + [_vp]),
    "mednet_pool2_bwd_act": (_i, [_vp, _vp, _vp, _i, _vp] + [_i] * 8 + [_vp]),
    "mednet_upcat_fwd": (_i, [_vp, _vp, _vp] + [_i] * 10 + [_vp]),
    "mednet_upcat_stats_chunks": (_i, [_i] * 7),
    "mednet_upcat_fwd_stats": (_i, [_vp, _vp, _vp, _vp] + [_i] * 10 + [_vp]),
    "mednet_upcat_bwd": (_i, [_vp, _vp, _vp] + [_i] * 10 + [_vp]),
    "mednet_loss_ws_bytes": (_sz, [_i, _i, _sz]),
    "mednet_dice_fwd": (_i, [_vp] * 6 + [_i, _i, _sz, _i64, _i64, _f, _i, _i, _vp, _sz, _vp]),
    "mednet_dice_bwd": (_i, [_vp] * 6 + [_i, _i, _sz, _i64, _i64, _f, _i, _i, _vp]),
    "mednet_head_landmark_supported": (_i, [_i, _i, _i, _i, _sz]),
    "mednet_head_landmark_ws_bytes": (_sz, [_i, _sz, _i, _i]),
    "mednet_head_landmark_gn_rows": (_i, [_sz]),
    "mednet_head_landmark_fwd": (_i, [_vp, _vp, _vp, _vp, _i64, _vp, _i64] + [_vp] * 6 + [_i, _sz, _i, _i, _i, _i, _f, _i, _i, _i,
                                      _vp, _sz, _vp]),
    "mednet_head_landmark_bwd": (_i, [_vp, _vp, _vp, _vp, _i64, _vp, _i64] + [_vp] * 7 + [_i, _vp, _vp, _vp, _i, _sz, _i, _i, _i,
                                      _i, _f, _i, _i, _i, _vp, _sz, _vp]),
    "mednet_head_landmark_cls_fwd": (_i, [_vp, _vp, _vp, _vp, _i64, _vp, _i64] + [_vp] * 7 + [_i, _sz, _i, _i, _i, _i, _i, _f, _i,
                                          _i, _i, _vp, _sz, _vp]),
    "mednet_head_landmark_cls_bwd": (_i, [_vp, _vp, _vp, _vp, _i64, _vp, _i64] + [_vp] * 7 + [_i, _vp, _vp, _vp, _i, _sz, _i, _i,
                                          _i, _i, _i, _f, _i, _i, _i, _vp, _sz, _vp]),
    "mednet_head_seg_supported": (_i, [_i, _i, _i, _i, _sz]),
    "mednet_head_seg_ws_bytes": (_sz, [_i, _sz, _i]),
    "mednet_head_seg_gn_rows": (_i, [_sz]),
    "mednet_head_seg_fwd": (_i, [_vp, _vp, _vp, _vp, _i64] + [_vp] * 4 + [_i, _sz, _i, _i, _i, _f, _i, _i, _i, _vp, _sz, _vp]),
    "mednet_head_seg_bwd": (_i, [_vp, _vp, _vp, _vp, _i64] + [_vp] * 5 + [_i, _vp, _vp, _vp, _i, _sz, _i, _i, _i, _f, _i, _i, _i,
                                 _vp, _sz, _vp]),
    "mednet_ds_head_supported": (_i, [_i] * 8),
    "mednet_ds_head_ws_bytes": (_sz, [_i] * 6),
    "mednet_ds_head_gn_rows": (_i, [_i] * 5),
    "mednet_ds_head_fwd": (_i, [_vp, _vp, _vp, _vp, _i, _i64, _vp, _vp, _vp] + [_i] * 11 + [_f, _i, _i, _i, _vp, _sz, _vp]),
    "mednet_ds_head_bwd": (_i, [_vp, _vp, _vp, _vp, _i, _i64] + [_vp] * 6 + [_i, _vp, _vp, _vp] + [_i] * 11 + [_f, _i, _i, _i,
                                _vp, _sz, _vp]),
    "mednet_head_ce_supported": (_i, [_i] * 4),
    "mednet_head_ce_ws_bytes": (_sz, [_i, _sz, _i, _i]),
    "mednet_head_ce_gn_rows": (_i, [_i, _sz, _i]),
    "mednet_head_ce_fwd": (_i, [_vp] * 4 + [_i, _i64, _vp, _vp, _vp, _vp, _i, _sz, _i, _i, _i, _i, _vp, _sz, _vp]),
    "mednet_head_ce_bwd": (_i, [_vp, _vp, _i, _i64] + [_vp] * 7 + [_i, _vp, _vp, _vp, _i, _sz, _i, _i, _i, _i, _vp, _sz, _vp]),
    "mednet_head_ce_bwd_sums": (_i, [_vp, _vp, _i, _i64] + [_vp] * 6 + [_i, _vp, _vp, _vp, _i, _sz, _i, _i, _i, _i, _vp, _sz, _vp]),
    "mednet_head_dice_bwd_sums": (_i, [_vp, _vp, _i, _i64] + [_vp] * 6 + [_i, _vp, _vp, _vp, _i, _sz, _i, _i, _f, _i, _i, _i, _vp, _sz, _vp]),
    "mednet_head_dice_ce_bwd_sums": (_i, [_vp, _vp, _i, _i64] + [_vp] * 6 + [_i, _vp, _vp, _vp, _i, _sz, _i, _i, _f, _i, _i, _i, _vp, _sz, _vp]),
    "mednet_head_dice_supported": (_i, [_i] * 4),
    "mednet_head_dice_ws_bytes": (_sz, [_i, _sz, _i, _i]),
    "mednet_head_dice_gn_rows": (_i, [_i, _sz, _i]),
    "mednet_head_dice_fwd": (_i, [_vp] * 4 + [_i, _i64, _vp, _vp, _vp, _vp, _i, _sz, _i, _i, _f, _i, _i, _i, _vp, _sz, _vp]),
    "mednet_head_dice_bwd": (_i, [_vp, _vp, _i, _i64] + [_vp] * 7 + [_i, _vp, _vp, _vp, _i, _sz, _i, _i, _f, _i, _i, _i, _vp, _sz, _vp]),
    "mednet_head_dice_ce_supported": (_i, [_i] * 4),
    "mednet_head_dice_ce_ws_bytes": (_sz, [_i, _sz, _i, _i]),
    "mednet_head_dice_ce_gn_rows": (_i, [_i, _sz, _i]),
    "mednet_head_dice_ce_fwd": (_i, [_vp] * 4 + [_i, _i64, _vp, _vp, _vp, _vp, _i, _sz, _i, _i, _f, _i, _i, _i, _vp, _sz, _vp]),
# ... 121 lines not shown
```

### torch-mednet_amd/mednet_hip/block.py

```python
from __future__ import annotations

import torch
from torch.autograd import Function

import os

from . import _lib as L
from . import config, debug, ops

ENABLED = os.environ.get("MEDNET_BLOCK_NODE", "1") == "1"
WGRAD_FIRST = ops.WGRAD_FIRST


def _conv_fwd(x, packed, cout, want_stats, x_layout=L.NDHWC):
    return ops.conv_forward(x, x_layout, packed, None, cout, 3, False, config.act_dtype(), want_stats)


FUSE_POOL = os.environ.get("MEDNET_FUSE_POOL", "1") == "1"


def _gn_fwd(y, partial, gamma, beta, groups, eps, act, residual, pool_mode=None):
    stats, coef = ops.gn_statistics(y, gamma, beta, groups, eps, partial)
    z, pooled = ops.norm_apply(y, coef, residual, act, pool_mode if FUSE_POOL else None)
    return z, stats, coef, pooled


def _gn_bwd(dz, dz2, y, z, coef, stats, gamma_p, beta_p, groups, act, want_dres, partial=None, lazy=None):
    b = ops._NormBackward(y, gamma_p, beta_p, want_dres)
    ops.gn_backward(b, dz, y, z, coef, stats, gamma_p, act, L.ACT_NONE, partial, groups, dz2=dz2, lazy=lazy)
    return (b.dx, b.dres, *b.param_grads())


FUSE_C1GN = os.environ.get("MEDNET_FUSE_C1GN", "1") == "1"
C1GN_COUNT = {"fused": 0}


def _c1_gn_applies(xin, y, partial, need_dx):
    if not (FUSE_C1GN and partial is not None and not need_dx and y.dtype != torch.float32 and config.conv_algo() != L.ALGO_DIRECT):
        return False
    cin = xin.shape[1]
    if cin == 1:
        return bool(L.lib().mednet_conv3d_wgrad_c1_gn_supported(y.shape[1], L.dt(xin), L.dt(y)))
    return bool(L.lib().mednet_conv3d_wgrad_cm_gn_supported(cin, y.shape[1], L.dt(xin), L.dt(y)))


def _c1_gn_bwd(xin, dz, y, coef, stats, gamma_p, beta_p, weight_p, groups, act, partial, x_layout=L.NDHWC):
    n, c, d, h, w = y.shape
    cin = xin.shape[1]
    lib = L.lib()
    C1GN_COUNT["fused"] += 1
    dgamma, dg_direct = ops._grad_target(gamma_p, (c,))
    dbeta, db_direct = ops._grad_target(beta_p, (c,))
    dw, dw_direct = ops._grad_target(weight_p, (c, cin, 3, 3, 3))
    bcoef = torch.empty((n, c, 3), dtype=torch.float32, device=y.device)
    ws = L.workspace(max(lib.mednet_gn_ws_bytes(n, c, d * h * w), lib.mednet_conv3d_wgrad_ws_bytes(n, d, h, w, cin, c, 3, 0)), y.device)
    L.check(lib.mednet_gn_bwd_coefficients(stats.data_ptr(), gamma_p.data_ptr(), partial.data_ptr(), partial.shape[1],
                                           bcoef.data_ptr(), dgamma.data_ptr(), dbeta.data_ptr(), n, d * h * w, c, groups,
                                           ws.data_ptr(), ws.numel(), L.stream()), "gn_bwd_coefficients")
    if cin == 1:
        L.check(lib.mednet_conv3d_wgrad_c1_gn(xin.data_ptr(), dz.data_ptr(), y.data_ptr(), coef.data_ptr(), bcoef.data_ptr(),
                                              dw.data_ptr(), n, d, h, w, c, act, L.dt(xin), L.dt(y), ws.data_ptr(), ws.numel(),
                                              L.stream()), "conv3d_wgrad_c1_gn")
    else:
        L.check(lib.mednet_conv3d_wgrad_cm_gn(xin.data_ptr(), x_layout, dz.data_ptr(), y.data_ptr(), coef.data_ptr(), bcoef.data_ptr(),
                                              dw.data_ptr(), n, d, h, w, cin, c, act, L.dt(xin), L.dt(y), ws.data_ptr(), ws.numel(),
                                              L.stream()), "conv3d_wgrad_cm_gn")
    return (None if dw_direct else dw), (None if dg_direct else dgamma), (None if db_direct else dbeta)


FUSE_DRES = os.environ.get("MEDNET_FUSE_DRES", "1") == "1"


FUSE_GNB = ops.FUSE_GNB


def _conv_bwd(x, dy, packed, weight_p, need_dx, add=None, gnb=None, x_layout=L.NDHWC):
    return ops.conv_backward(x, dy, packed, weight_p, need_dx, ops.block_dx_dtype(x), add=add, gnb=gnb if FUSE_GNB else None,
                             x_layout=x_layout, wgrad_first=WGRAD_FIRST)


class ResBlockFn(Function):
    @staticmethod
    def forward(ctx, x, w1, g1, b1, w2, g2, b2, w3, g3, b3, pk1, pk2, pk3, groups, eps, act, hook=None, pool=None):
        L.require_gpu(x, "ExtResNetBlock")
        ctx.algo = config.conv_algo()
        x = ops._as_act(x)
        cout = w1.shape[0]
        xin, x_layout = ops.first_layer_input(x, cout, 3, config.act_dtype())
        ctx.x_layout = x_layout
        fuse = (cout // groups) % 2 == 0
        y1, p1 = _conv_fwd(xin, pk1, cout, fuse, x_layout)
        z1, s1, c1, _ = _gn_fwd(y1, p1, g1, b1, groups, eps, act, None)
        y2, p2 = _conv_fwd(z1, pk2, cout, fuse)
        z2, s2, c2, _ = _gn_fwd(y2, p2, g2, b2, groups, eps, act, None)
        y3, p3 = _conv_fwd(z2, pk3, cout, fuse)
        out, s3, c3, pooled = _gn_fwd(y3, p3, g3, b3, groups, eps, act, z1, pool_mode=pool.mode if pool is not None else None)
        if pool is not None:
            pool.pooled = pooled
        if debug.TRACE is not None:
            debug.trace("resblock.fwd", y1, p1, s1, c1, z1, y2, p2, s2, c2, z2, y3, p3, s3, c3, out)
        ctx.save_for_backward(xin, y1, z1, y2, z2, y3, out, s1, c1, s2, c2, s3, c3, pk1, pk2, pk3)
        ctx.params = (w1, g1, b1, w2, g2, b2, w3, g3, b3)
        ctx.meta = (groups, act)
        ctx.gn3 = hook
        if hook is not None:
            hook.gn_in, hook.act = y3, act
        return out

    @staticmethod
    @ops._with_algo
    def backward(ctx, dout):
        xin, y1, z1, y2, z2, y3, out, s1, c1, s2, c2, s3, c3, pk1, pk2, pk3 = ctx.saved_tensors
        w1, g1, b1, w2, g2, b2, w3, g3, b3 = ctx.params
        groups, act = ctx.meta
        part3 = ctx.gn3.take(dout) if ctx.gn3 is not None else None
        lazy = None
        if ctx.gn3 is not None and part3 is not None:
            lazy, ctx.gn3.lazy = ctx.gn3.lazy, None
        if lazy is None:
            dout = ops.to_cl(dout.to(out.dtype))
        dy3, dres, dg3, db3 = _gn_bwd(dout, None, y3, out, c3, s3, g3, b3, groups, act, True, partial=part3, lazy=lazy)
        dz2, dw3, part2 = _conv_bwd(z2, dy3, pk3, w3, True, gnb=(y2, c2, act))
        dy2, _, dg2, db2 = _gn_bwd(dz2, None, y2, None, c2, s2, g2, b2, groups, act, False, partial=part2)
        n_, c_, d_, h_, w_ = z1.shape
        fuse = FUSE_DRES and dres.dtype == dy2.dtype and bool(
            L.lib().mednet_conv3d_dgrad_add_supported(n_, d_, h_, w_, c_, c_, config.conv_algo(), L.dt(dy2)))
        dz1, dw2, part1 = _conv_bwd(z1, dy2, pk2, w2, True, add=dres if fuse else None, gnb=(y1, c1, act) if fuse else None)
        if fuse and _c1_gn_applies(xin, y1, part1, ctx.needs_input_grad[0]):
            dy1 = dx = None
            dw1, dg1, db1 = _c1_gn_bwd(xin, dz1, y1, c1, s1, g1, b1, w1, groups, act, part1, ctx.x_layout)
        else:
            dy1, _, dg1, db1 = _gn_bwd(dz1, None if fuse else dres, y1, None, c1, s1, g1, b1, groups, act, False, partial=part1)
            dx, dw1, _ = _conv_bwd(xin, dy1, pk1, w1, ctx.needs_input_grad[0], x_layout=ctx.x_layout)
        if debug.TRACE is not None:
            debug.trace("resblock.bwd", None if lazy is not None else dout, part3, dy3, dres, dz2, part2, dy2, dz1, part1, dy1, dx)
        return (dx, dw1, dg1, db1, dw2, dg2, db2, dw3, dg3, db3) + (None,) * 8


class PoolStash:
    __slots__ = ("mode", "pooled", "version")

    def __init__(self, mode):
        self.mode, self.pooled, self.version = mode, None, -1


def res_block(x, convs, norms, groups, eps, act, pool_mode=None, head_next=False):
    (k1, k2, k3), (n1, n2, n3) = convs, norms
    hook = ops.GN3Hook() if (ops.FUSE_GN3 and torch.is_grad_enabled()) else None
    if hook is not None:
        hook.lazy_head_ok = bool(head_next)
    stash = PoolStash(pool_mode) if (pool_mode is not None and FUSE_POOL) else None
    out = ResBlockFn.apply(x, k1.weight, n1.weight, n1.bias, k2.weight, n2.weight, n2.bias, k3.weight, n3.weight, n3.bias,
                           k1._packed(x, converts=True), k2._packed(x, converts=True), k3._packed(x, converts=True), groups, eps, act,
                           hook, stash)
    if hook is not None:
        out._mednet_gn3 = hook
    if stash is not None and stash.pooled is not None:
        stash.version = out._version
        out._mednet_pooled = stash
    return out
```

### torch-mednet_amd/mednet_hip/ops.py

```python
from __future__ import annotations

import contextlib
import os

import torch
from torch.autograd import Function

from . import _lib as L
from . import config, debug

CL = torch.channels_last_3d

PROFILE = {"enabled": False, "events": [], "match": None}


SIDE = {"enabled": False, "stream": None, "keepalive": [], "wgrad_wgs": int(os.environ.get("MEDNET_SIDE_WGRAD_WGS", "128"))}


SIDE_MIN_VOXELS = int(os.environ.get("MEDNET_SIDE_MIN_VOXELS", "0"))
SIDE_CORESIDENT = os.environ.get("MEDNET_SIDE_CORESIDENT", "1") == "1"


def wgrad_coresident(n, d, h, w, cin, cout, ksize, x, dy) -> bool:
    return bool(L.lib().mednet_conv3d_wgrad_coresident(n, d, h, w, cin, cout, ksize, L.dt(x), L.dt(dy), config.conv_algo()))
# ... 162 lines not shown


def pack_conv_weight(weight: torch.Tensor, ksize: int, transposed: bool, out: torch.Tensor = None) -> torch.Tensor:
    L.require_gpu(weight, "pack_conv_weight")
    w = weight.detach()
    if w.dtype != torch.float32 or not w.is_contiguous():
        w = w.float().contiguous()
    cin, cout = (w.shape[0], w.shape[1]) if transposed else (w.shape[1], w.shape[0])
    nbytes = L.lib().mednet_conv3d_pack_bytes(cin, cout, ksize)
    if out is not None and (out.numel() != nbytes or out.device != w.device):
        raise RuntimeError("pack_conv_weight: `out` is not this layer's pack buffer")
    buf = out if out is not None else torch.empty(nbytes, dtype=torch.uint8, device=w.device)
    elt = config.pack_elt()
    L.check(L.lib().mednet_conv3d_pack_elt(w.data_ptr(), buf.data_ptr(), cin, cout, ksize, int(transposed), elt, L.stream()),
            "conv3d_pack")
    return buf


class GN3Hook:
    __slots__ = ("gn_in", "act", "partial", "dx", "version", "lazy", "lazy_head_ok")

    def __init__(self):
        self.gn_in = None
        self.act = 0
        self.partial = self.dx = None
        self.version = -1
        self.lazy = None
        self.lazy_head_ok = False

    def offer(self, dx, partial, lazy=None):
        self.dx, self.partial, self.version, self.lazy = dx, partial, dx._version, lazy

    def take(self, dout):
        partial, dx, version, lazy = self.partial, self.dx, self.version, self.lazy
        self.partial = self.dx = self.lazy = None
        ok = partial is not None and dout is dx and dout._version == version
        if lazy is not None and not ok:
            raise RuntimeError("mednet_hip: the block output handed to skip_pool2(sole_consumer=True), or to a fused head as its sole "
                               "consumer, has another consumer (or its gradient was replaced by a hook): the pooling / head backward did "
                               "not materialise its gradient (MEDNET_LAZY_POOL=0 / MEDNET_LAZY_HEAD=0 turn the optimisation off)")
        GN3_COUNT["taken" if ok else ("declined" if partial is not None else "absent")] += 1
        GN3_COUNT["lazy_head"] += int(ok and lazy is not None and isinstance(lazy[0], str))
        self.lazy = lazy if ok else None
        return partial if ok else None


FUSE_GN3 = os.environ.get("MEDNET_FUSE_GN3", "1") == "1"


class GNBHook(GN3Hook):
    __slots__ = ("coef",)

    def __init__(self):
        super().__init__()
        self.coef = None


class BNBHook(GNBHook):
    __slots__ = ()


class ActMaskHook:
    __slots__ = ("act", "dx", "version")

    def __init__(self, act):
        self.act, self.dx, self.version = act, None, -1

    def offer(self, dx):
        self.dx, self.version = dx, dx._version

    def take(self, dz):
        dx, version = self.dx, self.version
        self.dx = None
        ok = dx is not None and dz is dx and dz._version == version
        GN3_COUNT["masked"] += int(ok)
        return ok


def _gnb_hook_of(x, dtype):
    h = getattr(x, "_mednet_gnb", None) if FUSE_GN3 else None
    if h is None or h.gn_in is None or h.gn_in.shape != x.shape or h.gn_in.dtype != dtype or dtype not in config.HALF_TYPES:
        return None
    return h
GN3_COUNT = {"taken": 0, "declined": 0, "absent": 0, "masked": 0, "lazy_head": 0}


def _gn3_hook_of(x, dtype):
    h = getattr(x, "_mednet_gn3", None) if FUSE_GN3 else None
    if h is None or h.gn_in is None or h.gn_in.shape != x.shape or h.gn_in.dtype != dtype:
        return None
    return h


FUSE_GNB = os.environ.get("MEDNET_FUSE_GNB", "1") == "1"
WGRAD_FIRST = os.environ.get("MEDNET_WGRAD_FIRST", "1") == "1"


def fused_partial_rows(n, d, h, w, cin, cout, ksize, x_dt, y_dt, device):
    chunks = L.lib().mednet_conv3d_fused_stats_chunks(n, d, h, w, cin, cout, ksize, x_dt, y_dt, config.conv_algo())
    return torch.empty((n, chunks, cout, 2), dtype=torch.float32, device=device) if chunks > 0 else None


def _partial_out(ctx, partial, device):
    if partial is None:
        partial = torch.empty(0, device=device)
    ctx.mark_non_differentiable(partial)
    return partial


def _partial_in(partial):
    return partial if partial.numel() else None


def conv_forward(x, x_layout, packed, bias, cout, ksize, out_planar, out_dtype, want_stats):
    n, cin, d, h, w = x.shape
    if out_planar:
        y = torch.empty((n, cout, d, h, w), dtype=out_dtype, device=x.device)
    else:
        y = empty_cl(n, cout, d, h, w, out_dtype, x.device)
    partial = fused_partial_rows(n, d, h, w, cin, cout, ksize, L.dt(x), L.dt(y), x.device) if want_stats else None
    with profiled_conv(ksize, cin, cout, n, d, h, w):
        L.check(L.lib().mednet_conv3d_fwd(x.data_ptr(), packed.data_ptr(), L.ptr(bias), y.data_ptr(), n, d, h, w, cin, cout, ksize,
                                          L.dt(x), x_layout, L.dt(y), L.NCDHW if out_planar else L.NDHWC, 0, config.conv_algo(),
                                          L.ptr(partial), L.stream()), "conv3d_fwd")
    return y, partial


def conv_dgrad(dy, packed, x_shape, cout, ksize, dx_dtype, dy_planar=False, head=None, gnb=None, add=None, profiled=False):
    n, cin, d, h, w = x_shape
    lib, algo = L.lib(), config.conv_algo()
    dx = empty_cl(n, cin, d, h, w, dx_dtype, dy.device)
    head_rows = lib.mednet_head_dgrad_gn_rows(n, d, h, w, cin, L.dt(dx)) if head is not None else 0
    gn_rows = 0
    if head_rows == 0 and gnb is not None and dx.dtype == dy.dtype and (add is None or add.dtype == dy.dtype):
        gn_rows = lib.mednet_conv3d_dgrad_gn_rows_dt(n, d, h, w, cin, cout, algo, L.dt(dy))
    rows = head_rows or gn_rows
    variant = ("add+gn" if add is not None else "gn") if rows > 0 else ("add" if add is not None else "plain")
    with profiled_dgrad(variant, ksize, cout, cin, n, d, h, w) if profiled else contextlib.nullcontext():
        partial = torch.empty((n, rows, cin, 2), dtype=torch.float32, device=dy.device) if rows > 0 else None
        if head_rows > 0:
            y3, out, act = head
            L.check(lib.mednet_head_dgrad_gn(dy.data_ptr(), packed.data_ptr(), dx.data_ptr(), y3.data_ptr(), out.data_ptr(), act,
                                             partial.data_ptr(), n, d, h, w, cin, cout, L.dt(dx), L.stream()), "head_dgrad_gn")
        elif gn_rows > 0:
            y_prev, coef_prev, act_prev = gnb
            L.check(lib.mednet_conv3d_dgrad_gn(dy.data_ptr(), packed.data_ptr(), L.ptr(add), dx.data_ptr(), y_prev.data_ptr(),
                                               coef_prev.data_ptr(), act_prev, partial.data_ptr(), n, d, h, w, cin, cout, algo,
                                               L.dt(dy), L.stream()), "conv3d_dgrad_gn")
        elif add is not None:
            L.check(lib.mednet_conv3d_dgrad_add(dy.data_ptr(), packed.data_ptr(), add.data_ptr(), dx.data_ptr(), n, d, h, w, cin, cout,
                                                algo, L.dt(dy), L.stream()), "conv3d_dgrad_add")
        else:
            L.check(lib.mednet_conv3d_fwd(dy.data_ptr(), packed.data_ptr(), None, dx.data_ptr(), n, d, h, w, cout, cin, ksize, L.dt(dy),
                                          L.NCDHW if dy_planar else L.NDHWC, L.dt(dx), L.NDHWC, 1, algo, None, L.stream()), "conv3d_dgrad")
    return dx, partial


def conv_wgrad(x, dy, weight_p, bias_p, ksize, x_layout=L.NDHWC, dy_planar=False, coresident=False, profiled=False, transposed=False,
               want_dw=True):
    n, cin, d, h, w = x.shape
    cout = dy.shape[1]
    lib = L.lib()
    w_shape = (cin, cout, 3, 3, 3) if transposed else (cout, cin, ksize, ksize, ksize)
    if want_dw:
        dw, direct_w = _grad_target(weight_p, w_shape)
    else:
        dw, direct_w = torch.empty(w_shape, dtype=torch.float32, device=dy.device), False
# ... 774 lines not shown
        lab, lab_args = _labels_i64(labels, (n,) + tuple(lg.shape[2:])), ()
    else:
        lab, lab_sn, lab_dt = _label_view(labels, n, tuple(lg.shape[2:]))
        lab_args = (lab_dt, lab_sn)
    return lg, lab, _loss_weight(weight, lg.device), (n, c, lg[0, 0].numel(), sn, sc), lab_args


def _class_loss_fwd(ctx, name, logits, opnd, saved_shape, scalars, ws, dice=None):
    lg, lab, wt, geom, lab_args = opnd
    loss = None if ctx is None else torch.empty((), dtype=torch.float32, device=lg.device)
    saved = torch.empty(saved_shape, dtype=torch.float32, device=lg.device)
    outs = (L.ptr(loss), saved.data_ptr()) + ((L.ptr(dice),) if lab_args else ())
    entry = getattr(L.lib(), f"mednet_{name}_fwd" + ("_lt" if lab_args else ""))
    L.check(entry(lg.data_ptr(), lab.data_ptr(), *lab_args, L.ptr(wt), *outs, *geom, *scalars, ws.data_ptr(), ws.numel(), L.stream()),
            name + "_fwd")
    if ctx is None:
        return None
    ctx.save_for_backward(lg, lab, wt, saved)
    ctx.meta = (name, lab_args, geom, scalars, logits.dtype)
    ctx.split = getattr(logits, "_mednet_split", None) if lg is logits else None
    if debug.TRACE is not None and name != "ce":
        debug.trace(name + ".fwd", lg, loss, saved)
    return loss


def _class_loss_bwd(ctx, dloss, n_inputs):
    lg, lab, wt, saved = ctx.saved_tensors
    name, lab_args, geom, scalars, in_dtype = ctx.meta
    dl = dloss.to(torch.float32).contiguous()
    dlogits = _loss_grad_like(lg, ctx.split)
    entry = getattr(L.lib(), f"mednet_{name}_bwd" + ("_lt" if lab_args else ""))
    L.check(entry(lg.data_ptr(), lab.data_ptr(), *lab_args, L.ptr(wt), saved.data_ptr(), dl.data_ptr(), dlogits.data_ptr(), *geom,
                  *scalars, L.stream()), name + "_bwd")
    if debug.TRACE is not None and name != "ce":
        debug.trace(name + ".bwd", dlogits)
    return (dlogits.to(in_dtype),) + (None,) * (n_inputs - 1)


def _head_supported(x: torch.Tensor, *targets, mfma: bool) -> bool:
    if not (FUSE_HEAD_LOSS and x.is_cuda and x.dim() == 5 and all(t.is_cuda for t in targets)):
        return False
    if x.dtype != config.act_dtype() or not x.is_contiguous(memory_format=CL):
        return False
    if not mfma:
        return True
    if x.dtype == torch.float32 or any(t.dtype != torch.uint8 for t in targets):
        return False
    return getattr(x, "_mednet_actmask", None) is None or _gn3_hook_of(x, x.dtype) is not None


def _label_dt(labels):
    return L.U8 if labels.dtype == torch.uint8 else L.I64


class _HeadBackward:

    def __init__(self, ctx, x, cout, gn_rows, ws_bytes):
        weight, self.bias = ctx.params
        n, cin = x.shape[:2]
        self.dx = torch.empty_like(x, memory_format=CL)
        self.dw, self.direct_w = _grad_target(weight, (cout, cin, 1, 1, 1))
        self.db, self.direct_b = (None, True) if self.bias is None else _grad_target(self.bias, (cout,))
        self.hook, self.inmask = ctx.gn3, getattr(ctx, "inmask", None)
        self.partial = None if self.hook is None else torch.empty((n, gn_rows(), cin, 2), dtype=torch.float32, device=x.device)
        self.gn_in = None if self.hook is None else self.hook.gn_in.data_ptr()
        self.act = self.hook.act if self.hook is not None else (self.inmask.act if self.inmask is not None else 0)
        self.ws = L.workspace(ws_bytes, x.device)

    def finish(self, name, n_inputs, lazy=None):
        if self.hook is not None:
            self.hook.offer(self.dx, self.partial, lazy)
        elif self.inmask is not None:
            self.inmask.offer(self.dx)
        if debug.TRACE is not None:
            debug.trace(name + ".bwd", None if lazy is not None else self.dx, self.partial, self.dw, self.db)
        return (self.dx, (None if self.direct_w else self.dw),
                (None if (self.bias is None or self.direct_b) else self.db)) + (None,) * (n_inputs - 3)


def head_dice_supported(x: torch.Tensor, cin: int, cout: int, labels: torch.Tensor) -> bool:
    return _head_supported(x, labels, mfma=False) and bool(L.lib().mednet_head_dice_supported(cin, cout, L.dt(x), _label_dt(labels)))


def _valu_head_fwd(ctx, name, x, weight, bias, packed, labels, loss_weight, saved_shape, scalars):
    L.require_gpu(x, name)
    n, cin, d, h, w = x.shape
    cout = weight.shape[0]
    spatial = d * h * w
    lab, lab_sn, lab_dt = _label_view(labels, n, (d, h, w))
    wt = _loss_weight(loss_weight, x.device)
    logits = torch.empty((n, cout, d, h, w), dtype=torch.float32, device=x.device)
    loss = torch.empty((), dtype=torch.float32, device=x.device)
    saved = torch.empty(saved_shape, dtype=torch.float32, device=x.device)
    lib = L.lib()
    ws = L.workspace(getattr(lib, f"mednet_{name}_ws_bytes")(n, spatial, cin, cout), x.device)
    L.check(getattr(lib, f"mednet_{name}_fwd")(x.data_ptr(), packed.data_ptr(), L.ptr(bias), lab.data_ptr(), lab_dt, lab_sn, L.ptr(wt),
                                               logits.data_ptr(), loss.data_ptr(), saved.data_ptr(), n, spatial, cin, cout, *scalars,
                                               L.dt(x), ws.data_ptr(), ws.numel(), L.stream()), name + "_fwd")
    ctx.save_for_backward(x, packed, logits, lab, wt, saved)
    ctx.meta = (scalars, lab_sn, lab_dt)
    ctx.params = (weight, bias)
    ctx.gn3 = _gn3_hook_of(x, x.dtype)
    ctx.inmask = getattr(x, "_mednet_actmask", None) if (ctx.gn3 is None and FUSE_GN3 and POOL_ACT_MASK) else None
    ctx.lazy_ok = (LAZY_HEAD and ctx.gn3 is not None and ctx.gn3.lazy_head_ok and not _reads_grad(x)
                   and bool(lib.mednet_gn_act_bwd_fused_res_head_supported(cin, cout, L.dt(x), lab_dt)))
    ctx.mark_non_differentiable(logits)
    if debug.TRACE is not None:
        debug.trace(name + ".fwd", logits, loss, saved)
    return logits, loss


LAZY_HEAD = os.environ.get("MEDNET_LAZY_HEAD", "1") == "1"
_HEAD_KIND = {"head_dice": L.CLASS_DICE, "head_ce": L.CLASS_CE, "head_dice_ce": L.CLASS_DICE_CE}


def _reads_grad(x) -> bool:
    return bool(x._backward_hooks) or bool(getattr(x, "retains_grad", False))


def _valu_head_bwd(ctx, name, dloss, n_inputs):
    x, packed, logits, lab, wt, saved = ctx.saved_tensors
    scalars, lab_sn, lab_dt = ctx.meta
    n, cin = x.shape[:2]
    cout = logits.shape[1]
    spatial = x[0, 0].numel()
    lib = L.lib()
    dl = dloss.to(torch.float32).contiguous()
    b = _HeadBackward(ctx, x, cout, lambda: getattr(lib, f"mednet_{name}_gn_rows")(n, spatial, cin),
                      getattr(lib, f"mednet_{name}_ws_bytes")(n, spatial, cin, cout))
    if ctx.lazy_ok and b.hook is not None and debug.TRACE is None and not _reads_grad(x):
        L.check(getattr(lib, f"mednet_{name}_bwd_sums")(logits.data_ptr(), lab.data_ptr(), lab_dt, lab_sn, packed.data_ptr(), L.ptr(wt),
                                                        saved.data_ptr(), dl.data_ptr(), b.gn_in, x.data_ptr(), b.act,
                                                        b.partial.data_ptr(), b.dw.data_ptr(), L.ptr(b.db), n, spatial, cin, cout,
                                                        *scalars, L.dt(x), b.ws.data_ptr(), b.ws.numel(), L.stream()), name + "_bwd_sums")
        eps, sigmoid, ii = scalars if len(scalars) == 3 else (0.0, 0, scalars[0])
        return b.finish(name, n_inputs, lazy=("head", logits, lab, lab_dt, lab_sn, packed, wt, saved, dl, eps, sigmoid, ii,
                                             _HEAD_KIND[name]))
    L.check(getattr(lib, f"mednet_{name}_bwd")(logits.data_ptr(), lab.data_ptr(), lab_dt, lab_sn, packed.data_ptr(), L.ptr(wt),
                                               saved.data_ptr(), dl.data_ptr(), b.dx.data_ptr(), b.gn_in, x.data_ptr(), b.act,
                                               L.ptr(b.partial), b.dw.data_ptr(), L.ptr(b.db), n, spatial, cin, cout, *scalars,
                                               L.dt(x), b.ws.data_ptr(), b.ws.numel(), L.stream()), name + "_bwd")
    return b.finish(name, n_inputs)


class HeadDiceFn(Function):

    @staticmethod
    def forward(ctx, x, weight, bias, packed, labels, loss_weight, eps, sigmoid, ignore_index):
        ii = L.NO_IGNORE if ignore_index is None else int(ignore_index)
        return _valu_head_fwd(ctx, "head_dice", x, weight, bias, packed, labels, loss_weight, (weight.shape[0], 2),
                              (eps, int(sigmoid), ii))

    @staticmethod
    def backward(ctx, _dlogits, dloss):
        return _valu_head_bwd(ctx, "head_dice", dloss, 9)


def head_dice(x, weight, bias, packed, labels, loss_weight=None, eps=1e-5, sigmoid=False, ignore_index=None):
    return HeadDiceFn.apply(x, weight, bias, packed, labels, loss_weight, eps, sigmoid, ignore_index)


def head_ce_supported(x: torch.Tensor, cin: int, cout: int, labels: torch.Tensor) -> bool:
    return _head_supported(x, labels, mfma=False) and bool(L.lib().mednet_head_ce_supported(cin, cout, L.dt(x), _label_dt(labels)))


class HeadCEFn(Function):

    @staticmethod
    def forward(ctx, x, weight, bias, packed, labels, loss_weight, ignore_index):
        return _valu_head_fwd(ctx, "head_ce", x, weight, bias, packed, labels, loss_weight, (2,), (int(ignore_index),))

    @staticmethod
    def backward(ctx, _dlogits, dloss):
        return _valu_head_bwd(ctx, "head_ce", dloss, 7)


def head_ce(x, weight, bias, packed, labels, loss_weight=None, ignore_index=-100):
    return HeadCEFn.apply(x, weight, bias, packed, labels, loss_weight, ignore_index)


def head_dice_ce_supported(x: torch.Tensor, cin: int, cout: int, labels: torch.Tensor) -> bool:
    return _head_supported(x, labels, mfma=False) and bool(L.lib().mednet_head_dice_ce_supported(cin, cout, L.dt(x), _label_dt(labels)))


class HeadDiceCEFn(Function):

    @staticmethod
    def forward(ctx, x, weight, bias, packed, labels, loss_weight, eps):
        return _valu_head_fwd(ctx, "head_dice_ce", x, weight, bias, packed, labels, loss_weight, (2 * weight.shape[0] + 1,),
                              (eps, 0, L.NO_IGNORE))

    @staticmethod
    def backward(ctx, _dlogits, dloss):
        return _valu_head_bwd(ctx, "head_dice_ce", dloss, 7)


# ... 377 lines not shown
```

### torch-mednet_amd/mednet_hip/train.py

```python
from __future__ import annotations

import os

import torch
import torch.distributed as dist

from . import ops, vis
from .unet import loss as HL


class FlatParams:

    def __init__(self, module: torch.nn.Module):
        self.flags = [(k, p, p.requires_grad) for k, p in module.named_parameters()]
        self.params = [p for p in module.parameters() if p.requires_grad]
        if not self.params:
            raise RuntimeError("FlatParams: the module has no trainable parameter")
        dev = self.params[0].device
        self.offsets = []
        total = 0
        for p in self.params:
            self.offsets.append(total)
            total += (p.numel() + 63) // 64 * 64
        self.total = total
# ... 412 lines not shown
        if self.scaler is None:
            self.opt.step(grad_scale=scale)
        else:
            self.opt.step_scaled(self.scaler, inv_world=scale)

    def _norm_runs(self) -> bool:
        return self.opt._norm_runs(self.scaler)

    @property
    def grad_norm(self):
        if not self._norm_runs():
            raise RuntimeError("grad_norm: this step takes no gradient norm (pass clip_grad_norm=... or skip_nonfinite=True)")
        return self.opt.opt_state[1]

    def skipped_steps(self) -> int:
        if self.scaler is not None:
            return self.scaler.skipped_steps()
        return int(self.opt.opt_state[5].item()) if self._norm_runs() else 0


def use_side_stream():
    ops.SIDE["enabled"] = os.environ.get("MEDNET_SIDE_STREAM", "1") == "1"


def _call_is_hooked(model, final_conv) -> bool:
    import torch.nn.modules.module as M
    for name in ("_global_forward_hooks", "_global_forward_pre_hooks", "_global_forward_hooks_always_called"):
        if getattr(M, name, None):
            return True
    return any(bool(getattr(mod, attr, None)) for mod in (model, final_conv) for attr in ("_forward_hooks", "_forward_pre_hooks"))


def _class_criterion(loss, w):
    if loss == "DICE_CE":
        return HL.DiceCELoss(weight=w)
    return HL.DiceLoss(weight=w) if loss == "DICE" else HL.CrossEntropyLoss(weight=w)


def _class_spec(crit):
    if isinstance(crit, HL.DiceCELoss):
        return "DICE_CE", dict(loss_weight=crit.weight, eps=crit.epsilon)
    if isinstance(crit, HL.DiceLoss):
        return "DICE", dict(loss_weight=crit.weight, eps=crit.epsilon, sigmoid=crit.sigmoid_normalization, ignore_index=crit.ignore_index)
    if isinstance(crit, HL.CrossEntropyLoss):
        return "CE", dict(loss_weight=crit.weight, ignore_index=crit.ignore_index)
    return None, {}


def _head_fusable(model, crit, inputs) -> bool:
    from .unet.model import _UNetCore
    fc = getattr(model, "final_conv", None)
    return (isinstance(model, _UNetCore) and not model.testing and _class_spec(crit)[0] is not None
            and not getattr(crit, "skip_last_target", False) and fc is not None and getattr(fc, "planar_output", False)
            and fc.kernel_size[0] == 1 and inputs.is_cuda and not _call_is_hooked(model, fc))


def deep_supervision_weights(k, ds_weights=None):
    if ds_weights is None:
        total = sum(2.0 ** -t for t in range(k + 1))
        return [2.0 ** -s / total for s in range(k + 1)]
    ws = [float(v) for v in ds_weights]
    if len(ws) != k + 1:
        raise ValueError(f"ds_weights: {k + 1} weights expected (levels 0 .. {k}), got {len(ws)}")
    if any(not v >= 0.0 for v in ws):
        raise ValueError(f"ds_weights must be non-negative, got {ws}")
    return ws


class SegmentationStep(_GraphedStep):

    def __init__(self, model, loss_weight=None, lr=1e-3, loss="DICE", world_size=1, graph=None, optimizer="adam", optimizer_args=None,
                 clip_grad_norm=None, skip_nonfinite=False, ds_weights=None):
        dev = next(model.parameters()).device
        w = None if loss_weight is None else torch.tensor(loss_weight, dtype=torch.float32, device=dev)
        self.loss = _class_criterion(loss, w).to(dev)
        self.ds_weights = deep_supervision_weights(len(getattr(model, "ds_heads", ())), ds_weights)
        self.scale_losses = []
        self._setup(model, world_size, graph, optimizer, optimizer_args, lr, clip_grad_norm, skip_nonfinite)

    def _head_loss(self, inputs, label_u8):
        m, fc = self.model, getattr(self.model, "final_conv", None)
        kind, kw = _class_spec(self.loss)
        if _head_fusable(m, self.loss, inputs):
            feats = m.forward_features(inputs)
            small = "head_" + kind.lower()
            if getattr(ops, small + "_supported")(feats, fc.in_channels, fc.out_channels, label_u8):
                return getattr(ops, small)(feats, fc.weight, fc.bias, fc._packed(), label_u8, **kw)
            if ops.head_seg_supported(feats, fc.in_channels, fc.out_channels, label_u8):
                return ops.head_seg(feats, fc.weight, fc.bias, fc._packed(), label_u8, class_loss=kind, **kw)
            outputs = fc(feats)
        else:
            outputs = m(inputs)
        return outputs, self.loss(outputs, label_u8 if kind == "DICE_CE" else label_u8.long())

    def _ds_level(self, s, feats, label_u8, inputs, aux):
        head, crit = self.model.ds_heads[s - 1], self.loss
        kind, kw = _class_spec(crit)
        if (inputs.is_cuda and label_u8.dtype == torch.uint8 and not _call_is_hooked(self.model, head) and kind is not None
                and not getattr(crit, "skip_last_target", False)
                and ops.ds_head_supported(feats, head.in_channels, head.out_channels, label_u8, s)):
            feats, aux[s] = ops.ds_head(feats, head.weight, head.bias, head._packed(), label_u8, s, class_loss=kind, **kw)
            return feats
        d, h, w = feats.shape[2:]
        lab = label_u8[:, :d << s:1 << s, :h << s:1 << s, :w << s:1 << s].contiguous()
        aux[s] = crit(head(feats), lab if kind == "DICE_CE" else lab.long())
        return feats

    def _fwd_bwd(self, batch):
        inputs = batch["data"].float()
        label_u8 = batch["label"][:, -1, ...]
        k = len(self.ds_weights) - 1
        if k == 0:
            _, loss = self._head_loss(inputs, label_u8)
            self.scale_losses = [loss.detach()]
        else:
            from . import config
            aux = {}
            self.model._ds_tap = lambda s, feats: self._ds_level(s, feats, label_u8, inputs, aux)
            try:
                with config.exact_products(not config.is_half_mode()):
                    _, aux[0] = self._head_loss(inputs, label_u8)
            finally:
                del self.model._ds_tap
            loss = aux[0] * self.ds_weights[0]
            for s in range(1, k + 1):
                loss = loss + aux[s] * self.ds_weights[s]
            self.scale_losses = [aux[s].detach() for s in range(k + 1)]
        self._backward(loss)
        return (loss.detach(),)

    def __call__(self, batch):
        (loss,) = super().__call__(batch)
        return loss


class _Validation:

    def _setup(self, model, log_interval, log_vis_mip, on_samples):
        self.model = model
        self.log_interval, self.log_vis_mip, self.on_samples = log_interval, log_vis_mip, on_samples

    def _logs_samples(self, batch_nb) -> bool:
        return bool(self.log_interval) and self.on_samples is not None and batch_nb % self.log_interval == 0

    def _in_eval_mode(self, fn, *args):
        was_training = self.model.training
        self.model.eval()
        try:
            return fn(*args)
        finally:
            self.model.train(was_training)

    @staticmethod
    def _with_dice(results, per_channel_dice):
        for c in range(per_channel_dice.shape[0]):
            results[f"val_dice{c}"] = per_channel_dice[c]
        return results

    @staticmethod
    def validation_epoch_end(outputs):
        logs = {k: torch.stack([o[k] for o in outputs]).mean() for k in outputs[0]}
        return {"val_loss": logs["val_loss"], "log": logs, "progress_bar": logs}


class SegmentationValidation(_Validation):

    def __init__(self, model, loss_weight=None, loss="DICE", log_interval=None, log_vis_mip="mean", on_samples=None):
        dev = next(model.parameters()).device
        w = None if loss_weight is None else torch.tensor(loss_weight, dtype=torch.float32, device=dev)
        self.loss = _class_criterion(loss, w).to(dev)
# ... 114 lines not shown
```

### torch-mednet_amd/mednet_hip/unet/components.py

```python
from __future__ import annotations

import torch
import torch.nn as nn

import os

from .. import _lib as L
from .. import block
from .. import config
from .. import nn as hnn
from .. import ops

_ACT_MODULES = {"r": ("ReLU", hnn.ReLU, L.ACT_RELU), "l": ("LeakyReLU", hnn.LeakyReLU, L.ACT_LEAKY),
                "e": ("ELU", hnn.ELU, L.ACT_ELU)}


def conv3d(in_channels, out_channels, kernel_size, bias, padding=1):
    return hnn.Conv3d(in_channels, out_channels, kernel_size, padding=padding, bias=bias)


def create_conv(in_channels, out_channels, kernel_size, order, num_groups, padding=1):
    assert "c" in order, "Conv layer MUST be present"
    assert order[0] not in "rle", "Non-linearity cannot be the first operation in the layer"
    conv_pos = order.index("c")
# ... 61 lines not shown
                    i += 2
                elif nxt is None and residual is not None:
                    x = m(x, act=final_act, residual=residual, partial=partial)
                    fused_res = True
                    i += 1
                else:
                    x = m(x, partial=partial)
                    i += 1
                partial = None
                continue
            partial = None
            nxt = mods[i + 1] if i + 1 < len(mods) else None
            if isinstance(m, hnn.Conv3d) and isinstance(nxt, hnn.GroupNorm) \
                    and m.bias is None and x.is_cuda and (m.out_channels // nxt.num_groups) % 2 == 0:
                x, partial = m.forward_with_stats(x)
            elif isinstance(m, hnn.Conv3d) and isinstance(nxt, hnn._Act) and m.bias is None and m.kernel_size[0] == 3 \
                    and not m.planar_output and ops.conv3d_act_supported(x, m.in_channels, m.out_channels):
                last = i + 2 == len(mods)
                want = last and stats_for is not None and stats_for.num_channels == m.out_channels \
                    and (m.out_channels // stats_for.num_groups) % 2 == 0
                x, p = ops.conv3d_act(x, m.weight, m._packed(x), nxt.code, want)
                if last:
                    out_partial = p
                i += 2
                continue
            else:
                x = m(x)
            i += 1
        if residual is not None and not fused_res:
            x = ops.activation(ops.AddFn.apply(x, residual), final_act)
        if stats_for is not None:
            return x, out_partial
        return x


class DoubleConv(nn.Sequential):
    def __init__(self, in_channels, out_channels, encoder, kernel_size=3, order="crg", num_groups=8):
        super().__init__()
        if encoder:
            c1_in, c1_out = in_channels, max(out_channels // 2, in_channels)
            c2_in, c2_out = c1_out, out_channels
        else:
            c1_in, c1_out, c2_in, c2_out = in_channels, out_channels, out_channels, out_channels
        self.add_module("SingleConv1", SingleConv(c1_in, c1_out, kernel_size, order, num_groups))
        self.add_module("SingleConv2", SingleConv(c2_in, c2_out, kernel_size, order, num_groups))

    def forward(self, x, partial=None):
        sc1, sc2 = self.SingleConv1, self.SingleConv2
        first2 = next(iter(sc2._modules.values()))
        if isinstance(first2, hnn.GroupNorm) and torch.is_tensor(x) and x.is_cuda:
            x, p2 = sc1(x, partial=partial, stats_for=first2)
            return sc2(x, partial=p2)
        return sc2(sc1(x, partial=partial))


class ExtResNetBlock(nn.Module):
    def __init__(self, in_channels, out_channels, kernel_size=3, order="cge", num_groups=8, **kwargs):
        super().__init__()
        self.conv1 = SingleConv(in_channels, out_channels, kernel_size=kernel_size, order=order, num_groups=num_groups)
        self.conv2 = SingleConv(out_channels, out_channels, kernel_size=kernel_size, order=order, num_groups=num_groups)
        stripped = order.translate({ord(c): None for c in "rel"})
        self.conv3 = SingleConv(out_channels, out_channels, kernel_size=kernel_size, order=stripped,
                                num_groups=num_groups)
        key = "l" if "l" in order else ("e" if "e" in order else "r")
        self.non_linearity = _ACT_MODULES[key][1](inplace=True)
        self._kinked = key != "e" or "b" in order

    def _plain(self):
        convs, norms = [], []
        for sc, want_act in ((self.conv1, True), (self.conv2, True), (self.conv3, False)):
            mods = list(sc._modules.values())
            if len(mods) != (3 if want_act else 2) or not isinstance(mods[0], hnn.Conv3d) or not isinstance(mods[1], hnn.GroupNorm):
                return None
            if want_act and (not isinstance(mods[2], hnn._Act) or mods[2].code != self.non_linearity.code):
                return None
            if mods[0].bias is not None or mods[0].kernel_size[0] != 3 or not mods[1].affine:
                return None
            convs.append(mods[0])
            norms.append(mods[1])
        if len({m.num_groups for m in norms}) != 1 or len({m.eps for m in norms}) != 1:
            return None
        return convs, norms

    def forward(self, x, pool_mode=None, head_next=False):
        with config.exact_products(self._kinked):
            return self._forward(x, pool_mode, head_next)

    def _forward(self, x, pool_mode=None, head_next=False):
        plain = self._plain() if (x.is_cuda and block.ENABLED) else None
        if plain is not None:
            convs, norms = plain
            return block.res_block(x, convs, norms, norms[0].num_groups, norms[0].eps, self.non_linearity.code, pool_mode=pool_mode,
                                   head_next=head_next)
        residual = self.conv1(x)
        out = self.conv2(residual)
        return self.conv3(out, residual=residual, final_act=self.non_linearity.code)


def _module_kinked(module) -> bool:
    return any(getattr(m, "_kinked", False) for m in module.modules())


_FUSE_SKIP_POOL = os.environ.get("MEDNET_SKIP_POOL", "1") == "1"


class Encoder(nn.Module):
    def __init__(self, in_channels, out_channels, conv_kernel_size=3, apply_pooling=True, pool_kernel_size=(2, 2, 2),
                 pool_type="max", basic_module=DoubleConv, conv_layer_order="crg", num_groups=8):
        super().__init__()
        assert pool_type in ["max", "avg"]
        if apply_pooling:
            self.pooling = (hnn.MaxPool3d if pool_type == "max" else hnn.AvgPool3d)(kernel_size=pool_kernel_size)
        else:
            self.pooling = None
        self.basic_module = basic_module(in_channels, out_channels, encoder=True, kernel_size=conv_kernel_size,
                                         order=conv_layer_order, num_groups=num_groups)

    def forward(self, x, with_skip=False, pool_next=None, sole_consumer=False):
        def body(t):
            if pool_next is not None and isinstance(self.basic_module, ExtResNetBlock):
                return self.basic_module(t, pool_mode=pool_next)
            return self.basic_module(t)

        if not with_skip:
            if self.pooling is not None:
                x = self.pooling(x)
            return body(x)
        if _FUSE_SKIP_POOL and isinstance(self.pooling, hnn._Pool2) and torch.is_tensor(x) and x.is_cuda and x.requires_grad:
            skip, pooled = ops.skip_pool2(x, self.pooling.mode, sole_consumer=sole_consumer)
            return skip, body(pooled)
        return x, self.forward(x, pool_next=pool_next)

    def forward_with_skip(self, x):
        return self(x, with_skip=True)


class Decoder(nn.Module):
    def __init__(self, in_channels, out_channels, kernel_size=3, scale_factor=(2, 2, 2), basic_module=DoubleConv,
                 conv_layer_order="crg", num_groups=8):
        super().__init__()
        if basic_module == DoubleConv:
            self.upsample = None
        else:
            self.upsample = hnn.ConvTranspose3d(in_channels, out_channels, kernel_size=kernel_size, stride=scale_factor,
                                                padding=1, output_padding=1)
            in_channels = out_channels
        self.basic_module = basic_module(in_channels, out_channels, encoder=False, kernel_size=kernel_size,
                                         order=conv_layer_order, num_groups=num_groups)

    def forward(self, encoder_features, x, head_next=False):
        with config.exact_products(_module_kinked(self.basic_module)):
            if self.upsample is None:
                bm = self.basic_module
                first = next(iter(bm.SingleConv1._modules.values())) if isinstance(bm, DoubleConv) else None
                if isinstance(first, hnn.GroupNorm) and torch.is_tensor(x) and x.is_cuda and first.num_channels % (2 * first.num_groups) == 0:
                    x, partial = ops.upsample_concat(encoder_features, x, want_stats=True)
                    return bm(x, partial=partial)
                x = ops.upsample_concat(encoder_features, x)
            else:
                x = self.upsample(x, skip=encoder_features)
            if head_next and isinstance(self.basic_module, ExtResNetBlock):
                return self.basic_module(x, head_next=True)
            return self.basic_module(x)


class FinalConv(nn.Sequential):
    def __init__(self, in_channels, out_channels, kernel_size=3, order="crg", num_groups=8):
        super().__init__()
        self.add_module("SingleConv", SingleConv(in_channels, in_channels, kernel_size, order, num_groups))
        self.add_module("final_conv", hnn.Conv3d(in_channels, out_channels, 1))
```

### torch-mednet_amd/mednet_hip/unet/model.py

```python
from __future__ import annotations

import torch
import torch.nn as nn

from .. import config
from .. import nn as hnn
from .. import ops
from .components import Decoder, DoubleConv, Encoder, ExtResNetBlock, SingleConv

try:
    import pytorch_lightning as _pl

    _Base = _pl.LightningModule
except Exception:
    _Base = nn.Module


def create_feature_maps(init_channel_number, number_of_fmaps):
    return [init_channel_number * 2 ** k for k in range(number_of_fmaps)]


class _Softmax1(nn.Module):

    def forward(self, x):
# ... 1 lines not shown


class _CheckpointCompat:

    CHECKPOINT_HYPER_PARAMS_KEY = "hyper_parameters"
    CHECKPOINT_HYPER_PARAMS_NAME = "hparams_name"

    @classmethod
    def load_from_checkpoint(cls, checkpoint_path, *args, map_location=None, **kwargs):
        import argparse
        import inspect
        ckpt = torch.load(checkpoint_path, map_location=map_location if map_location is not None else "cpu",
                          weights_only=False)
        init_args = inspect.getfullargspec(cls.__init__).args[1:]
        hp = ckpt.get(cls.CHECKPOINT_HYPER_PARAMS_KEY, ckpt.get("hparams"))
        if hp is not None:
            hp = dict(vars(hp)) if isinstance(hp, argparse.Namespace) else dict(hp)
            hp.update(kwargs)
            name = ckpt.get(cls.CHECKPOINT_HYPER_PARAMS_NAME)
            if name is None and "hparams" in init_args:
                name = "hparams"
            if name == "kwargs" or name is None:
                kwargs = {k: v for k, v in hp.items() if k in init_args} if name is None else hp
            else:
                kwargs = {name: argparse.Namespace(**hp)}
        model = cls(*args, **kwargs)
        model.load_state_dict(ckpt["state_dict"])
        hook = getattr(model, "on_load_checkpoint", None)
        if callable(hook):
            hook(ckpt)
        return model

    def freeze(self):
        for p in self.parameters():
            p.requires_grad = False
        self.eval()

    def unfreeze(self):
        for p in self.parameters():
            p.requires_grad = True
        self.train()


class _UNetCore(*((_Base,) if _Base is not nn.Module else (_CheckpointCompat, nn.Module))):
    def _assemble(self, in_channels, out_channels, f_maps, order, num_groups, block, default_levels, deep_supervision=0):
        if isinstance(f_maps, int):
            f_maps = create_feature_maps(f_maps, number_of_fmaps=default_levels)
        f_maps = list(f_maps)
        concat = block is DoubleConv
        self.encoders = nn.ModuleList(
            Encoder(in_channels if i == 0 else f_maps[i - 1], f, apply_pooling=(i != 0), basic_module=block,
                    conv_layer_order=order, num_groups=num_groups) for i, f in enumerate(f_maps))
        rev = f_maps[::-1]
        self.decoders = nn.ModuleList(
            Decoder(rev[i] + rev[i + 1] if concat else rev[i], rev[i + 1], basic_module=block, conv_layer_order=order,
                    num_groups=num_groups) for i in range(len(rev) - 1))
        self.final_conv = hnn.Conv3d(f_maps[0], out_channels, 1, planar_output=True)
        k = int(deep_supervision)
        if not 0 <= k <= max(0, len(f_maps) - 2):
            raise ValueError(f"deep_supervision must be in 0 .. {max(0, len(f_maps) - 2)} for {len(f_maps)} feature levels, not {deep_supervision}")
        if k > 0:
            self.ds_heads = nn.ModuleList(hnn.Conv3d(f_maps[s], out_channels, 1, planar_output=True) for s in range(1, k + 1))

    @property
    def deep_supervision(self) -> int:
        return len(self.ds_heads) if hasattr(self, "ds_heads") else 0

    def forward_pyramid(self, x):
        kinked = any(getattr(m, "_kinked", False) for m in self.modules())
        taps = {}
        with config.exact_products(kinked):
            taps[0] = self._features(x, tap=lambda s, f: taps.setdefault(s, f))
        return [taps[s] for s in range(self.deep_supervision + 1)]

    def forward_deep(self, x):
        feats = self.forward_pyramid(x)
        return [self.final_conv(feats[0])] + [head(f) for head, f in zip(getattr(self, "ds_heads", ()), feats[1:])]

    def forward(self, x):
        kinked = any(getattr(m, "_kinked", False) for m in self.modules())
        with config.exact_products(kinked):
            return self._forward(x)

    def forward_features(self, x):
        kinked = any(getattr(m, "_kinked", False) for m in self.modules())
        with config.exact_products(kinked):
            return self._features(x)

    def _forward(self, x):
        x = self.final_conv(self._features(x))
        if self.testing and self.final_activation is not None:
            x = self.final_activation(x)
        return x

    def _features(self, x, tap=None):
        tap = tap if tap is not None else getattr(self, "_ds_tap", None)
        k = self.deep_supervision if tap is not None else 0
        skips = []
        for i, enc in enumerate(self.encoders):
            nxt = self.encoders[i + 1] if i + 1 < len(self.encoders) else None
            pool_next = nxt.pooling.mode if (nxt is not None and isinstance(nxt.pooling, hnn._Pool2)) else None
            if i == 0:
                x = enc(x, pool_next=pool_next)
            else:
                skips[0], x = enc(x, with_skip=True, pool_next=pool_next, sole_consumer=not _has_forward_hooks(self.encoders[i - 1]))
            skips.insert(0, x)
        top = len(self.decoders) - 1
        for i, (dec, skip) in enumerate(zip(self.decoders, skips[1:])):
            if i == top:
                x = dec(skip, x, head_next=not _has_forward_hooks(dec))
                continue
            x = dec(skip, x)
            if 1 <= top - i <= k:
                x = tap(top - i, x)
        return x


def _has_forward_hooks(module) -> bool:
    import torch.nn.modules.module as M
    if getattr(M, "_global_forward_hooks", None) or getattr(M, "_global_forward_hooks_always_called", None):
        return True
    return any(m._forward_hooks for m in module.modules())


class UNet3D(_UNetCore):
    def __init__(self, in_channels, out_channels, final_sigmoid, f_maps=64, layer_order="gcr", num_groups=8, **kwargs):
        super().__init__()
        self.testing = kwargs.get("testing", False)
        self._assemble(in_channels, out_channels, f_maps, layer_order, num_groups, DoubleConv, default_levels=4,
                       deep_supervision=kwargs.get("deep_supervision", 0))
        self.final_activation = nn.Sigmoid() if final_sigmoid else _Softmax1()


class ResidualUNet3D(_UNetCore):
    def __init__(self, in_channels, out_channels, final_sigmoid, f_maps=32, conv_layer_order="cge", num_groups=8,
                 skip_final_activation=False, **kwargs):
        super().__init__()
        self.testing = kwargs.get("testing", False)
        self._assemble(in_channels, out_channels, f_maps, conv_layer_order, num_groups, ExtResNetBlock,
                       default_levels=5, deep_supervision=kwargs.get("deep_supervision", 0))
        if skip_final_activation:
            self.final_activation = None
        else:
            self.final_activation = nn.Sigmoid() if final_sigmoid else _Softmax1()
```

Before: 213.2 patches/s.

## Fuse final GroupNorm-residual-activation with segmentation head logits and loss partials

Adds a kernel that applies the last decoder block's GroupNorm affine, residual add and activation, writes z, then uses a DPP quad transpose to give each lane a full 32-channel voxel. Each lane computes head logits and class-loss partial sums in the same pass. The head forward then only runs a small finalize over the stashed rows instead of re-reading z and labels. This removes one full read of the 32-channel activation tensor and a kernel launch per step, at the cost of extra plumbing through the model and a specialized path limited to 32 channels and 16-bit types.

```diff
diff --git a/include/mednet_hip.h b/include/mednet_hip.h
--- a/include/mednet_hip.h
+++ b/include/mednet_hip.h
@@ -137,6 +137,12 @@
                                      const float* stats, const float* gamma, const float* fused_partial, int rows, void* dx, void* dres,
                                      float* dgamma, float* dbeta, int n, size_t spatial, int c, int groups, int act, int dtype, void* ws,
                                      size_t ws_bytes, mednet_stream stream);
+int mednet_gn_act_fwd_res_head_supported(int c, int cout, int dtype, int label_dtype);
+size_t mednet_gn_act_fwd_res_head_rows_bytes(int n, size_t spatial, int cout, int class_kind);
+int mednet_gn_act_fwd_res_head(const void* x, const float* coef, const void* residual, void* out, const void* packed,
+                               const float* bias, const void* labels, int label_dtype, int64_t label_stride_n,
+                               const float* class_weight, int class_kind, int sigmoid, int ignore_index, float* logits, float* rows,
+                               size_t rows_bytes, int n, size_t spatial, int c, int cout, int act, int dtype, mednet_stream stream);
 int mednet_bn_stats(const void* x, const float* gamma, const float* beta, float* running_mean, float* running_var,
                     long long* num_batches_tracked, float momentum, float* stats, float* coef, int n, size_t spatial, int c,
                     float eps, int dtype, void* ws, size_t ws_bytes, mednet_stream stream);
@@ -207,6 +213,12 @@
                               const float* weight, const float* saved, const float* dloss, const void* gn_y, const void* z,
                               int gn_act, float* gn_partial, float* dw, float* dbias, int n, size_t spatial, int cin, int cout,
                               float eps, int sigmoid, int ignore_index, int z_dtype, void* ws, size_t ws_bytes, mednet_stream stream);
+int mednet_head_dice_fwd_rows(const float* rows, const float* weight, float* loss, float* saved, int n, size_t spatial, int cout,
+                              float eps, mednet_stream stream);
+int mednet_head_ce_fwd_rows(const float* rows, const float* weight, float* loss, float* saved, int n, size_t spatial, int cout,
+                            float eps, mednet_stream stream);
+int mednet_head_dice_ce_fwd_rows(const float* rows, const float* weight, float* loss, float* saved, int n, size_t spatial, int cout,
+                                 float eps, mednet_stream stream);
 
 int mednet_head_landmark_supported(int cin, int nh, int ncls, int dtype, size_t spatial);
 size_t mednet_head_landmark_ws_bytes(int n, size_t spatial, int nh, int ncls);
diff --git a/torch-mednet_amd/csrc/conv.h b/torch-mednet_amd/csrc/conv.h
--- a/torch-mednet_amd/csrc/conv.h
+++ b/torch-mednet_amd/csrc/conv.h
@@ -76,6 +76,13 @@
   return launch_class_finalize(kind, partial, ce_partial, weight, loss, saved, c, rows, eps, s);
 }
 
+constexpr int HEAD_FWD_BLOCK_VOX = 256 * 8;
+inline unsigned head_fwd_blocks(size_t spatial) { return (unsigned)((spatial + HEAD_FWD_BLOCK_VOX - 1) / HEAD_FWD_BLOCK_VOX); }
+inline size_t head_fwd_rows_bytes(int kind, int n, size_t spatial, int cout) {
+  const size_t per_row = (size_t)cout * 2 + (kind == MEDNET_CLASS_DICE_CE ? 2 : 0);
+  return ((size_t)n * head_fwd_blocks(spatial) * per_row + 64) * sizeof(float);
+}
+
 template <class F>
 inline void for_class_kind(int ce, F&& f) {
   if (ce == MEDNET_CLASS_DICE_CE) f(std::integral_constant<int, MEDNET_CLASS_DICE_CE>{});
diff --git a/torch-mednet_amd/csrc/head_loss.hip b/torch-mednet_amd/csrc/head_loss.hip
--- a/torch-mednet_amd/csrc/head_loss.hip
+++ b/torch-mednet_amd/csrc/head_loss.hip
@@ -4,7 +4,7 @@
 
 namespace mednet {
 
-constexpr int HL_BLOCK_VOX = 256 * 8;
+constexpr int HL_BLOCK_VOX = HEAD_FWD_BLOCK_VOX;
 constexpr int HL_MAXC = 4;
 constexpr int HL_VPT = 32;
 
@@ -58,13 +58,7 @@
       for (int i = 0; i < HL_MAXC; ++i) {
         lg[i] = 0.f;
         if (i < m) {
-          float s0 = bias ? bias[i] : 0.f, s1 = 0.f;
-#pragma unroll
-          for (int j = 0; j < K; j += 2) {
-            s0 = fmaf(zv[j], Pb[(size_t)i * K + j], s0);
-            s1 = fmaf(zv[j + 1], Pb[(size_t)i * K + j + 1], s1);
-          }
-          lg[i] = s0 + s1;
+          lg[i] = head_logit_row<K>([&](int j) { return zv[j]; }, Pb, bias, i);
           y[((size_t)n * m + i) * spatial + v] = lg[i];
         }
       }
@@ -251,7 +245,7 @@
   }
 }
 
-static inline unsigned hl_fwd_blocks(size_t spatial) { return (unsigned)((spatial + HL_BLOCK_VOX - 1) / HL_BLOCK_VOX); }
+static inline unsigned hl_fwd_blocks(size_t spatial) { return head_fwd_blocks(spatial); }
 static inline unsigned hl_bwd_blocks(size_t spatial, int k) {
   const size_t per_wg = (size_t)(256 / (k / 8)) * HL_VPT;
   return (unsigned)((spatial + per_wg - 1) / per_wg);
@@ -266,7 +260,7 @@
          (label_dtype == MEDNET_U8 || label_dtype == MEDNET_I64) && tuning_option("head_loss_fuse", 1);
 }
 extern "C" size_t mednet_head_dice_ws_bytes(int n, size_t spatial, int cin, int cout) {
-  const size_t fwd = ((size_t)n * hl_fwd_blocks(spatial) * cout * 2 + 64) * sizeof(float);
+  const size_t fwd = head_fwd_rows_bytes(MEDNET_CLASS_DICE, n, spatial, cout);
   const size_t width = (size_t)cout * cin + cout;
   const size_t bwd = ((size_t)n * hl_bwd_blocks(spatial, cin) * 4 * width + 64) * sizeof(float) + (size_t)HL_WF_GROUPS * width * sizeof(double) + 16;
   return fwd > bwd ? fwd : bwd;
@@ -276,7 +270,7 @@
   return 4 * (int)hl_bwd_blocks(spatial, cin);
 }
 extern "C" size_t mednet_head_dice_ce_ws_bytes(int n, size_t spatial, int cin, int cout) {
-  const size_t fwd = ((size_t)n * hl_fwd_blocks(spatial) * ((size_t)cout * 2 + 2) + 64) * sizeof(float);
+  const size_t fwd = head_fwd_rows_bytes(MEDNET_CLASS_DICE_CE, n, spatial, cout);
   const size_t bwd = mednet_head_dice_ws_bytes(n, spatial, cin, cout);
   return fwd > bwd ? fwd : bwd;
 }
@@ -365,6 +359,25 @@
                               cin, cout, eps, sigmoid, ignore_index, z_dtype, ws, ws_bytes, stream);
 }
 
+static int head_loss_fwd_rows(int kind, const char* what, const float* rows, const float* weight, float* loss, float* saved, int n,
+                              size_t spatial, int cout, float eps, mednet_stream stream) {
+  MEDNET_REQUIRE(n > 0 && spatial > 0 && cout >= 1 && cout <= HL_MAXC && rows && loss && saved, MEDNET_E_SHAPE, "%s: bad arguments", what);
+  return launch_class_finalize(kind, rows, weight, loss, saved, cout, (int)(hl_fwd_blocks(spatial) * n), eps, (hipStream_t)stream);
+}
+extern "C" int mednet_head_dice_fwd_rows(const float* rows, const float* weight, float* loss, float* saved, int n, size_t spatial,
+                                         int cout, float eps, mednet_stream stream) {
+  return head_loss_fwd_rows(MEDNET_CLASS_DICE, "head_dice_fwd_rows", rows, weight, loss, saved, n, spatial, cout, eps, stream);
+}
+extern "C" int mednet_head_ce_fwd_rows(const float* rows, const float* weight, float* loss, float* saved, int n, size_t spatial,
+                                       int cout, float eps, mednet_stream stream) {
+  (void)eps;
+  return head_loss_fwd_rows(MEDNET_CLASS_CE, "head_ce_fwd_rows", rows, weight, loss, saved, n, spatial, cout, 0.f, stream);
+}
+extern "C" int mednet_head_dice_ce_fwd_rows(const float* rows, const float* weight, float* loss, float* saved, int n, size_t spatial,
+                                            int cout, float eps, mednet_stream stream) {
+  return head_loss_fwd_rows(MEDNET_CLASS_DICE_CE, "head_dice_ce_fwd_rows", rows, weight, loss, saved, n, spatial, cout, eps, stream);
+}
+
 extern "C" int mednet_head_dice_bwd(const float* logits, const void* labels, int label_dtype, int64_t label_stride_n,
                                     const void* packed, const float* weight, const float* saved, const float* dloss, void* dz,
                                     const void* gn_y, const void* z, int gn_act, float* gn_partial, float* dw, float* dbias, int n,
diff --git a/torch-mednet_amd/csrc/loss_blocks.inc b/torch-mednet_amd/csrc/loss_blocks.inc
--- a/torch-mednet_amd/csrc/loss_blocks.inc
+++ b/torch-mednet_amd/csrc/loss_blocks.inc
@@ -54,6 +54,17 @@
     for (int k = 0; k < MAXC; ++k)
       if (k < c) p[k] *= inv;
   }
+}
+
+template <int K, class Z>
+__device__ __forceinline__ float head_logit_row(Z&& z, const float* __restrict__ Pb, const float* __restrict__ bias, int i) {
+  float s0 = bias ? bias[i] : 0.f, s1 = 0.f;
+#pragma unroll
+  for (int j = 0; j < K; j += 2) {
+    s0 = fmaf(z(j), Pb[(size_t)i * K + j], s0);
+    s1 = fmaf(z(j + 1), Pb[(size_t)i * K + j + 1], s1);
+  }
+  return s0 + s1;
 }
 
 template <int MAXC>
diff --git a/torch-mednet_amd/csrc/norm_act.hip b/torch-mednet_amd/csrc/norm_act.hip
--- a/torch-mednet_amd/csrc/norm_act.hip
+++ b/torch-mednet_amd/csrc/norm_act.hip
@@ -302,6 +302,17 @@
   }
 }
 
+template <int VEC>
+__device__ __forceinline__ void gn_apply_n(F8& out, const float (&a)[VEC], const float (&b)[VEC], const F8& xin, const F8& rin,
+                                           bool has_res, int act) {
+#pragma unroll
+  for (int k = 0; k < VEC; ++k) {
+    out.v[k] = fmaf(a[k], xin.v[k], b[k]);
+    if (has_res) out.v[k] += rin.v[k];
+  }
+  act_apply_n<VEC>(out.v, act);
+}
+
 template <typename TX, typename TZ, int VEC>
 __global__ __launch_bounds__(256) void gn_act_fwd_kernel(const TX* __restrict__ x, const float* __restrict__ coef,
                                                          const TZ* __restrict__ res, TZ* __restrict__ z,
@@ -318,14 +329,7 @@
     b[k] = coef[((size_t)n * c + L.col * VEC + k) * 2 + 1];
   }
   const size_t off = (size_t)n * spatial * c + (size_t)L.col * VEC;
-  auto one = [&](const F8& xin, const F8& rin, F8& out) {
-#pragma unroll
-    for (int k = 0; k < VEC; ++k) {
-      out.v[k] = fmaf(a[k], xin.v[k], b[k]);
-      if (res) out.v[k] += rin.v[k];
-    }
-    act_apply_n<VEC>(out.v, act);
-  };
+  auto one = [&](const F8& xin, const F8& rin, F8& out) { gn_apply_n<VEC>(out, a, b, xin, rin, res != nullptr, act); };
   size_t v = v0 + L.row;
   const size_t R = (size_t)L.rows;
   for (; v + 3 * R < v1; v += 4 * R) {
@@ -1054,6 +1058,115 @@
   size_t v = v0 + row;
   for (; v + (size_t)ROWS < v1; v += 2 * (size_t)ROWS) two(v, v + ROWS, true);
   for (; v < v1; v += ROWS) two(v, v, false);
+}
+
+typedef __attribute__((ext_vector_type(4))) uint32_t u32x4;
+template <typename T>
+using Half8 = std::conditional_t<std::is_same<T, bf16>::value, bf16x8, f16x8>;
+template <typename T>
+__device__ __forceinline__ u32x4 pack8(const F8& r) {
+  Half8<T> a;
+#pragma unroll
+  for (int k = 0; k < 8; ++k) a[k] = (T)r.v[k];
+  return __builtin_bit_cast(u32x4, a);
+}
+template <int CTRL>
+__device__ __forceinline__ uint32_t dpp_b32(uint32_t v) {
+  return (uint32_t)__builtin_amdgcn_update_dpp(0, (int)v, CTRL, 0xF, 0xF, true);
+}
+__device__ __forceinline__ void quad_transpose(u32x4 (&r)[4]) {
+  const bool o1 = threadIdx.x & 1, o2 = threadIdx.x & 2;
+#pragma unroll
+  for (int d = 0; d < 4; ++d) {
+#pragma unroll
+    for (int j = 0; j < 4; j += 2) {
+      const uint32_t lo = dpp_b32<0xB1>(r[j][d]), hi = dpp_b32<0xB1>(r[j + 1][d]);
+      r[j][d] = o1 ? hi : r[j][d];
+      r[j + 1][d] = o1 ? r[j + 1][d] : lo;
+    }
+#pragma unroll
+    for (int j = 0; j < 2; ++j) {
+      const uint32_t lo = dpp_b32<0x4E>(r[j][d]), hi = dpp_b32<0x4E>(r[j + 2][d]);
+      r[j][d] = o2 ? hi : r[j][d];
+      r[j + 2][d] = o2 ? r[j + 2][d] : lo;
+    }
+  }
+}
+
+template <typename T, typename TL, int KIND>
+__global__ __launch_bounds__(256) void gn_act_fwd_head_kernel(const T* __restrict__ x, const float* __restrict__ coef,
+                                                              const T* __restrict__ res, T* __restrict__ z,
+                                                              const float* __restrict__ Pb , const float* __restrict__ bias,
+                                                              const TL* __restrict__ lab, int64_t lab_sn, const float* __restrict__ cw,
+                                                              float* __restrict__ y, float* __restrict__ partial, size_t spatial,
+                                                              int act, int m, int sigmoid, int ignore) {
+  constexpr int C = 32, VEC = 8, MAXC = 4;
+  static_assert(sizeof(T) == 2, "16-bit storage");
+  __shared__ float scratch[4];
+  const int n = blockIdx.y, col = threadIdx.x & 3;
+  float a[VEC], b[VEC];
+#pragma unroll
+  for (int k = 0; k < VEC; ++k) {
+    a[k] = coef[((size_t)n * C + col * VEC + k) * 2];
+    b[k] = coef[((size_t)n * C + col * VEC + k) * 2 + 1];
+  }
+  const size_t off = (size_t)n * spatial * C + (size_t)col * VEC;
+  const size_t v0 = (size_t)blockIdx.x * HEAD_FWD_BLOCK_VOX;
+  const int wave = __builtin_amdgcn_readfirstlane(threadIdx.x >> 6);
+  ClassSums<MAXC> sums;
+  for (int it = 0; it < 8; ++it) {
+    const size_t vw = v0 + (size_t)it * 256 + (size_t)wave * 64;
+    if (vw >= spatial) break;
+    const size_t vq = vw + ((threadIdx.x & 63) & ~3);
+    F8 xi[4], ri[4];
+#pragma unroll
+    for (int j = 0; j < 4; ++j) {
+#pragma unroll
+      for (int k = 0; k < VEC; ++k) xi[j].v[k] = ri[j].v[k] = 0.f;
+    }
+#pragma unroll
+    for (int j = 0; j < 4; ++j)
+      if (vq + j < spatial) xi[j] = ld8(x, off + (vq + j) * C);
+#pragma unroll
+    for (int j = 0; j < 4; ++j)
+      if (vq + j < spatial) ri[j] = ld8(res, off + (vq + j) * C);
+    u32x4 pk[4];
+#pragma unroll
+    for (int j = 0; j < 4; ++j) {
+      F8 zo;
+      gn_apply_n<VEC>(zo, a, b, xi[j], ri[j], true, act);
+      pk[j] = pack8<T>(zo);
+    }
+#pragma unroll
+    for (int j = 0; j < 4; ++j)
+      if (vq + j < spatial) *reinterpret_cast<u32x4*>(z + off + (vq + j) * C) = pk[j];
+    quad_transpose(pk);
+    const size_t v = vq + col;
+    if (v < spatial) {
+      const Half8<T> h0 = __builtin_bit_cast(Half8<T>, pk[0]), h1 = __builtin_bit_cast(Half8<T>, pk[1]);
+      const Half8<T> h2 = __builtin_bit_cast(Half8<T>, pk[2]), h3 = __builtin_bit_cast(Half8<T>, pk[3]);
+      float zv[C];
+#pragma unroll
+      for (int k = 0; k < VEC; ++k) {
+        zv[k] = (float)h0[k];
+        zv[VEC + k] = (float)h1[k];
+        zv[2 * VEC + k] = (float)h2[k];
+        zv[3 * VEC + k] = (float)h3[k];
+      }
+      const int yl = label_at(lab, (size_t)n * lab_sn + v, ignore);
+      float lg[MAXC];
+#pragma unroll
+      for (int i = 0; i < MAXC; ++i) {
+        lg[i] = 0.f;
+        if (i < m) {
+          lg[i] = head_logit_row<C>([&](int j) { return zv[j]; }, Pb, bias, i);
+          y[((size_t)n * m + i) * spatial + v] = lg[i];
+        }
+      }
+      class_fwd_voxel<KIND, MAXC>(sums, [&](int k) { return lg[k]; }, yl, m, sigmoid, ignore, cw);
+    }
+  }
+  class_fwd_writeout<KIND, MAXC>(sums, partial, m, scratch);
 }
 
 __device__ __forceinline__ int nearest_src(int dst, int in, int out) {
@@ -1503,6 +1616,49 @@
   return check_launch("gn_bwd_apply_head");
 }
 
+extern "C" int mednet_gn_act_fwd_res_head_supported(int c, int cout, int dtype, int label_dtype) {
+  return mednet_gn_act_bwd_fused_res_head_supported(c, cout, dtype, label_dtype);
+}
+extern "C" size_t mednet_gn_act_fwd_res_head_rows_bytes(int n, size_t spatial, int cout, int class_kind) {
+  return head_fwd_rows_bytes(class_kind, n, spatial, cout);
+}
+extern "C" int mednet_gn_act_fwd_res_head(const void* x, const float* coef, const void* residual, void* out, const void* packed,
+                                          const float* bias, const void* labels, int label_dtype, int64_t label_stride_n,
+                                          const float* class_weight, int class_kind, int sigmoid, int ignore_index, float* logits,
+                                          float* rows, size_t rows_bytes, int n, size_t spatial, int c, int cout, int act, int dtype,
+                                          mednet_stream stream) {
+  MEDNET_REQUIRE(mednet_gn_act_fwd_res_head_supported(c, cout, dtype, label_dtype), MEDNET_E_UNSUPPORTED,
+                 "gn_act_fwd_res_head: %d features -> %d classes, dtype %d, labels %d", c, cout, dtype, label_dtype);
+  MEDNET_REQUIRE(class_kind == MEDNET_CLASS_DICE || class_kind == MEDNET_CLASS_CE || class_kind == MEDNET_CLASS_DICE_CE,
+                 MEDNET_E_UNSUPPORTED, "gn_act_fwd_res_head: class loss %d", class_kind);
+  MEDNET_REQUIRE(class_kind != MEDNET_CLASS_DICE_CE || (sigmoid == 0 && ignore_index == MEDNET_NO_IGNORE), MEDNET_E_UNSUPPORTED,
+                 "gn_act_fwd_res_head: Dice + cross-entropy is a softmax form without ignore_index");
+  MEDNET_REQUIRE(n > 0 && spatial > 0 && x && coef && residual && out && packed && labels && logits && rows, MEDNET_E_SHAPE,
+                 "gn_act_fwd_res_head: bad arguments");
+  MEDNET_REQUIRE(rows_bytes >= head_fwd_rows_bytes(class_kind, n, spatial, cout), MEDNET_E_WORKSPACE, "gn_act_fwd_res_head: rows too small");
+  hipStream_t s = (hipStream_t)stream;
+  const float* Pb = head_weights_f32(packed, c, cout);
+  if (class_kind == MEDNET_CLASS_CE) sigmoid = 0;
+  const float* cw = class_kind != MEDNET_CLASS_DICE ? class_weight : nullptr;
+  const dim3 grid(head_fwd_blocks(spatial), n);
+  for_class_kind(class_kind, [&](auto kind) {
+    by_type(dtype, [&](auto t) {
+      using T = typename decltype(t)::type;
+      if constexpr (sizeof(T) == 2) {
+        auto go = [&](auto l) {
+          using TL = typename decltype(l)::type;
+          hipLaunchKernelGGL((gn_act_fwd_head_kernel<T, TL, decltype(kind)::value>), grid, dim3(256), 0, s, (const T*)x, coef,
+                             (const T*)residual, (T*)out, Pb, bias, (const TL*)labels, label_stride_n, cw, logits, rows, spatial, act,
+                             cout, sigmoid, ignore_index);
+        };
+        if (label_dtype == MEDNET_U8) go(Tag<uint8_t>{});
+        else go(Tag<int64_t>{});
+      }
+    });
+  });
+  return check_launch("gn_act_fwd_head");
+}
+
 
 namespace mednet {
 constexpr int BN_NT = 1024;
diff --git a/torch-mednet_amd/mednet_hip/_lib.py b/torch-mednet_amd/mednet_hip/_lib.py
--- a/torch-mednet_amd/mednet_hip/_lib.py
+++ b/torch-mednet_amd/mednet_hip/_lib.py
@@ -64,6 +64,12 @@
     "mednet_gn_act_bwd_fused_res_head_supported": (_i, [_i] * 4),
     "mednet_gn_act_bwd_fused_res_head": (_i, [_vp, _vp, _i, _i64] + [_vp] * 4 + [_f, _i, _i, _i, _i] + [_vp] * 5 + [_i, _vp, _vp, _vp, _vp,
                                               _i, _sz, _i, _i, _i, _i, _vp, _sz, _vp]),
+    "mednet_gn_act_fwd_res_head_supported": (_i, [_i] * 4),
+    "mednet_gn_act_fwd_res_head_rows_bytes": (_sz, [_i, _sz, _i, _i]),
+    "mednet_gn_act_fwd_res_head": (_i, [_vp] * 7 + [_i, _i64, _vp, _i, _i, _i, _vp, _vp, _sz, _i, _sz, _i, _i, _i, _i, _vp]),
+    "mednet_head_dice_fwd_rows": (_i, [_vp] * 4 + [_i, _sz, _i, _f, _vp]),
+    "mednet_head_ce_fwd_rows": (_i, [_vp] * 4 + [_i, _sz, _i, _f, _vp]),
+    "mednet_head_dice_ce_fwd_rows": (_i, [_vp] * 4 + [_i, _sz, _i, _f, _vp]),
     "mednet_head_dgrad_gn_rows": (_i, [_i] * 6),
     "mednet_head_dgrad_gn": (_i, [_vp] * 5 + [_i, _vp] + [_i] * 7 + [_vp]),
     "mednet_pool2_bwd_gn_rows": (_i, [_i] * 6),
diff --git a/torch-mednet_amd/mednet_hip/block.py b/torch-mednet_amd/mednet_hip/block.py
--- a/torch-mednet_amd/mednet_hip/block.py
+++ b/torch-mednet_amd/mednet_hip/block.py
@@ -19,8 +19,10 @@
 FUSE_POOL = os.environ.get("MEDNET_FUSE_POOL", "1") == "1"
 
 
-def _gn_fwd(y, partial, gamma, beta, groups, eps, act, residual, pool_mode=None):
+def _gn_fwd(y, partial, gamma, beta, groups, eps, act, residual, pool_mode=None, head=None):
     stats, coef = ops.gn_statistics(y, gamma, beta, groups, eps, partial)
+    if head is not None and pool_mode is None and head.applies(y, residual):
+        return ops.norm_apply_head(y, coef, residual, act, head), stats, coef, None
     z, pooled = ops.norm_apply(y, coef, residual, act, pool_mode if FUSE_POOL else None)
     return z, stats, coef, pooled
 
@@ -81,7 +83,7 @@
 
 class ResBlockFn(Function):
     @staticmethod
-    def forward(ctx, x, w1, g1, b1, w2, g2, b2, w3, g3, b3, pk1, pk2, pk3, groups, eps, act, hook=None, pool=None):
+    def forward(ctx, x, w1, g1, b1, w2, g2, b2, w3, g3, b3, pk1, pk2, pk3, groups, eps, act, hook=None, pool=None, head=None):
         L.require_gpu(x, "ExtResNetBlock")
         ctx.algo = config.conv_algo()
         x = ops._as_act(x)
@@ -94,7 +96,8 @@
         y2, p2 = _conv_fwd(z1, pk2, cout, fuse)
         z2, s2, c2, _ = _gn_fwd(y2, p2, g2, b2, groups, eps, act, None)
         y3, p3 = _conv_fwd(z2, pk3, cout, fuse)
-        out, s3, c3, pooled = _gn_fwd(y3, p3, g3, b3, groups, eps, act, z1, pool_mode=pool.mode if pool is not None else None)
+        out, s3, c3, pooled = _gn_fwd(y3, p3, g3, b3, groups, eps, act, z1, pool_mode=pool.mode if pool is not None else None,
+                                      head=head if pool is None else None)
         if pool is not None:
             pool.pooled = pooled
         if debug.TRACE is not None:
@@ -134,7 +137,7 @@
             dx, dw1, _ = _conv_bwd(xin, dy1, pk1, w1, ctx.needs_input_grad[0], x_layout=ctx.x_layout)
         if debug.TRACE is not None:
             debug.trace("resblock.bwd", None if lazy is not None else dout, part3, dy3, dres, dz2, part2, dy2, dz1, part1, dy1, dx)
-        return (dx, dw1, dg1, db1, dw2, dg2, db2, dw3, dg3, db3) + (None,) * 8
+        return (dx, dw1, dg1, db1, dw2, dg2, db2, dw3, dg3, db3) + (None,) * 9
 
 
 class PoolStash:
@@ -144,18 +147,22 @@
         self.mode, self.pooled, self.version = mode, None, -1
 
 
-def res_block(x, convs, norms, groups, eps, act, pool_mode=None, head_next=False):
+def res_block(x, convs, norms, groups, eps, act, pool_mode=None, head_next=False, head=None):
     (k1, k2, k3), (n1, n2, n3) = convs, norms
     hook = ops.GN3Hook() if (ops.FUSE_GN3 and torch.is_grad_enabled()) else None
     if hook is not None:
         hook.lazy_head_ok = bool(head_next)
     stash = PoolStash(pool_mode) if (pool_mode is not None and FUSE_POOL) else None
+    head = head if (head_next and pool_mode is None) else None
     out = ResBlockFn.apply(x, k1.weight, n1.weight, n1.bias, k2.weight, n2.weight, n2.bias, k3.weight, n3.weight, n3.bias,
                            k1._packed(x, converts=True), k2._packed(x, converts=True), k3._packed(x, converts=True), groups, eps, act,
-                           hook, stash)
+                           hook, stash, head)
     if hook is not None:
         out._mednet_gn3 = hook
     if stash is not None and stash.pooled is not None:
         stash.version = out._version
         out._mednet_pooled = stash
+    if head is not None and head.logits is not None:
+        head.version = out._version
+        out._mednet_head_fwd = head
     return out
diff --git a/torch-mednet_amd/mednet_hip/ops.py b/torch-mednet_amd/mednet_hip/ops.py
--- a/torch-mednet_amd/mednet_hip/ops.py
+++ b/torch-mednet_amd/mednet_hip/ops.py
@@ -268,7 +268,7 @@
     if h is None or h.gn_in is None or h.gn_in.shape != x.shape or h.gn_in.dtype != dtype or dtype not in config.HALF_TYPES:
         return None
     return h
-GN3_COUNT = {"taken": 0, "declined": 0, "absent": 0, "masked": 0, "lazy_head": 0}
+GN3_COUNT = {"taken": 0, "declined": 0, "absent": 0, "masked": 0, "lazy_head": 0, "head_fwd": 0}
 
 
 def _gn3_hook_of(x, dtype):
@@ -1209,6 +1209,84 @@
     return _head_supported(x, labels, mfma=False) and bool(L.lib().mednet_head_dice_supported(cin, cout, L.dt(x), _label_dt(labels)))
 
 
+FUSED_HEAD_FWD = os.environ.get("MEDNET_FUSED_HEAD_FWD", "1") == "1"
+_HEAD_KIND = {"head_dice": L.CLASS_DICE, "head_ce": L.CLASS_CE, "head_dice_ce": L.CLASS_DICE_CE}
+_UNSET = object()
+
+
+def _same_tensor(a, b, version) -> bool:
+    if a is None or b is None:
+        return a is None and b is None
+    return a.data_ptr() == b.data_ptr() and a.dtype == b.dtype and a._version == version
+
+
+class HeadFwdSpec:
+    __slots__ = ("name", "scalars", "cin", "cout", "packed", "bias", "lab", "lab_sn", "lab_dt", "wt", "versions", "logits", "rows",
+                 "version")
+
+    def __init__(self, name, scalars, cin, cout, packed, bias, lab, lab_sn, lab_dt, wt):
+        self.name, self.scalars, self.cin, self.cout = name, tuple(scalars), cin, cout
+        self.packed, self.bias, self.lab, self.lab_sn, self.lab_dt, self.wt = packed, bias, lab, lab_sn, lab_dt, wt
+        self.versions = tuple(None if t is None else t._version for t in (packed, bias, lab, wt))
+        self.logits = self.rows = None
+        self.version = -1
+
+    def applies(self, y, residual) -> bool:
+        if not (FUSED_HEAD_FWD and residual is not None and y.is_cuda and y.dtype == config.act_dtype() and y.dim() == 5):
+            return False
+        if y.shape[0] != self.lab.shape[0] or y.shape[1] != self.cin or tuple(y.shape[2:]) != tuple(self.lab.shape[1:]):
+            return False
+        return bool(L.lib().mednet_gn_act_fwd_res_head_supported(self.cin, self.cout, L.dt(y), self.lab_dt))
+
+    def matches(self, x, name, scalars, cout, packed, bias, lab, lab_sn, lab_dt, wt) -> bool:
+        if self.logits is None or x._version != self.version or name != self.name or tuple(scalars) != self.scalars or cout != self.cout:
+            return False
+        if packed is not self.packed or (lab_sn, lab_dt) != (self.lab_sn, self.lab_dt) or tuple(lab.shape) != tuple(self.lab.shape):
+            return False
+        return all(_same_tensor(a, b, v) for a, b, v in zip((packed, bias, lab, wt), (self.packed, self.bias, self.lab, self.wt),
+                                                            self.versions))
+
+
+def head_fwd_spec(name, x_shape, conv, packed, labels, loss_weight=None, eps=1e-5, sigmoid=False, ignore_index=_UNSET):
+    if not (FUSED_HEAD_FWD and FUSE_HEAD_LOSS and labels.is_cuda and labels.dtype in (torch.uint8, torch.int64)):
+        return None
+    lab_dt = _label_dt(labels)
+    if not L.lib().mednet_gn_act_fwd_res_head_supported(conv.in_channels, conv.out_channels, L.dt_of(config.act_dtype()), lab_dt):
+        return None
+    n, spatial_shape = x_shape[0], tuple(x_shape[2:])
+    if tuple(labels.shape) != (n,) + spatial_shape:
+        return None
+    lab, lab_sn, _ = _label_view(labels, n, spatial_shape)
+    if lab.data_ptr() != labels.data_ptr():
+        return None
+    if name == "head_ce":
+        scalars = (int(-100 if ignore_index is _UNSET else ignore_index),)
+    elif name == "head_dice_ce":
+        scalars = (eps, 0, L.NO_IGNORE)
+    else:
+        ii = None if ignore_index is _UNSET else ignore_index
+        scalars = (eps, int(sigmoid), L.NO_IGNORE if ii is None else int(ii))
+    return HeadFwdSpec(name, scalars, conv.in_channels, conv.out_channels, packed, conv.bias, lab, lab_sn, lab_dt,
+                       _loss_weight(loss_weight, labels.device))
+
+
+def norm_apply_head(x, coef, residual, act, spec):
+    n, c, d, h, w = x.shape
+    spatial = d * h * w
+    lib = L.lib()
+    kind = _HEAD_KIND[spec.name]
+    sigmoid, ii = (0, spec.scalars[0]) if len(spec.scalars) == 1 else spec.scalars[1:]
+    z = torch.empty_like(x, memory_format=CL)
+    logits = torch.empty((n, spec.cout, d, h, w), dtype=torch.float32, device=x.device)
+    rows = torch.empty((lib.mednet_gn_act_fwd_res_head_rows_bytes(n, spatial, spec.cout, kind) + 3) // 4, dtype=torch.float32, device=x.device)
+    L.check(lib.mednet_gn_act_fwd_res_head(x.data_ptr(), coef.data_ptr(), residual.data_ptr(), z.data_ptr(), spec.packed.data_ptr(),
+                                           L.ptr(spec.bias), spec.lab.data_ptr(), spec.lab_dt, spec.lab_sn, L.ptr(spec.wt), kind, sigmoid,
+                                           ii, logits.data_ptr(), rows.data_ptr(), rows.numel() * 4, n, spatial, c, spec.cout, act,
+                                           L.dt(x), L.stream()), "gn_act_fwd_res_head")
+    spec.logits, spec.rows = logits, rows
+    return z
+
+
 def _valu_head_fwd(ctx, name, x, weight, bias, packed, labels, loss_weight, saved_shape, scalars):
     L.require_gpu(x, name)
     n, cin, d, h, w = x.shape
@@ -1216,14 +1294,22 @@
     spatial = d * h * w
     lab, lab_sn, lab_dt = _label_view(labels, n, (d, h, w))
     wt = _loss_weight(loss_weight, x.device)
-    logits = torch.empty((n, cout, d, h, w), dtype=torch.float32, device=x.device)
     loss = torch.empty((), dtype=torch.float32, device=x.device)
     saved = torch.empty(saved_shape, dtype=torch.float32, device=x.device)
     lib = L.lib()
-    ws = L.workspace(getattr(lib, f"mednet_{name}_ws_bytes")(n, spatial, cin, cout), x.device)
-    L.check(getattr(lib, f"mednet_{name}_fwd")(x.data_ptr(), packed.data_ptr(), L.ptr(bias), lab.data_ptr(), lab_dt, lab_sn, L.ptr(wt),
-                                               logits.data_ptr(), loss.data_ptr(), saved.data_ptr(), n, spatial, cin, cout, *scalars,
-                                               L.dt(x), ws.data_ptr(), ws.numel(), L.stream()), name + "_fwd")
+    stash = getattr(x, "_mednet_head_fwd", None)
+    if stash is not None and FUSED_HEAD_FWD and stash.matches(x, name, scalars, cout, packed, bias, lab, lab_sn, lab_dt, wt):
+        (logits, rows), stash.logits, stash.rows = (stash.logits, stash.rows), None, None
+        eps = scalars[0] if len(scalars) == 3 else 0.0
+        L.check(getattr(lib, f"mednet_{name}_fwd_rows")(rows.data_ptr(), L.ptr(wt), loss.data_ptr(), saved.data_ptr(), n, spatial, cout,
+                                                        eps, L.stream()), name + "_fwd_rows")
+        GN3_COUNT["head_fwd"] += 1
+    else:
+        logits = torch.empty((n, cout, d, h, w), dtype=torch.float32, device=x.device)
+        ws = L.workspace(getattr(lib, f"mednet_{name}_ws_bytes")(n, spatial, cin, cout), x.device)
+        L.check(getattr(lib, f"mednet_{name}_fwd")(x.data_ptr(), packed.data_ptr(), L.ptr(bias), lab.data_ptr(), lab_dt, lab_sn, L.ptr(wt),
+                                                   logits.data_ptr(), loss.data_ptr(), saved.data_ptr(), n, spatial, cin, cout, *scalars,
+                                                   L.dt(x), ws.data_ptr(), ws.numel(), L.stream()), name + "_fwd")
     ctx.save_for_backward(x, packed, logits, lab, wt, saved)
     ctx.meta = (scalars, lab_sn, lab_dt)
     ctx.params = (weight, bias)
@@ -1238,7 +1324,6 @@
 
 
 LAZY_HEAD = os.environ.get("MEDNET_LAZY_HEAD", "1") == "1"
-_HEAD_KIND = {"head_dice": L.CLASS_DICE, "head_ce": L.CLASS_CE, "head_dice_ce": L.CLASS_DICE_CE}
 
 
 def _reads_grad(x) -> bool:
diff --git a/torch-mednet_amd/mednet_hip/train.py b/torch-mednet_amd/mednet_hip/train.py
--- a/torch-mednet_amd/mednet_hip/train.py
+++ b/torch-mednet_amd/mednet_hip/train.py
@@ -518,10 +518,12 @@
         m, fc = self.model, getattr(self.model, "final_conv", None)
         kind, kw = _class_spec(self.loss)
         if _head_fusable(m, self.loss, inputs):
-            feats = m.forward_features(inputs)
             small = "head_" + kind.lower()
+            packed = fc._packed()
+            spec = ops.head_fwd_spec(small, inputs.shape, fc, packed, label_u8, **kw)
+            feats = m.forward_features(inputs, head=spec) if spec is not None else m.forward_features(inputs)
             if getattr(ops, small + "_supported")(feats, fc.in_channels, fc.out_channels, label_u8):
-                return getattr(ops, small)(feats, fc.weight, fc.bias, fc._packed(), label_u8, **kw)
+                return getattr(ops, small)(feats, fc.weight, fc.bias, packed, label_u8, **kw)
             if ops.head_seg_supported(feats, fc.in_channels, fc.out_channels, label_u8):
                 return ops.head_seg(feats, fc.weight, fc.bias, fc._packed(), label_u8, class_loss=kind, **kw)
             outputs = fc(feats)
diff --git a/torch-mednet_amd/mednet_hip/unet/components.py b/torch-mednet_amd/mednet_hip/unet/components.py
--- a/torch-mednet_amd/mednet_hip/unet/components.py
+++ b/torch-mednet_amd/mednet_hip/unet/components.py
@@ -167,16 +167,16 @@
             return None
         return convs, norms
 
-    def forward(self, x, pool_mode=None, head_next=False):
+    def forward(self, x, pool_mode=None, head_next=False, head=None):
         with config.exact_products(self._kinked):
-            return self._forward(x, pool_mode, head_next)
-
-    def _forward(self, x, pool_mode=None, head_next=False):
+            return self._forward(x, pool_mode, head_next, head)
+
+    def _forward(self, x, pool_mode=None, head_next=False, head=None):
         plain = self._plain() if (x.is_cuda and block.ENABLED) else None
         if plain is not None:
             convs, norms = plain
             return block.res_block(x, convs, norms, norms[0].num_groups, norms[0].eps, self.non_linearity.code, pool_mode=pool_mode,
-                                   head_next=head_next)
+                                   head_next=head_next, head=head)
         residual = self.conv1(x)
         out = self.conv2(residual)
         return self.conv3(out, residual=residual, final_act=self.non_linearity.code)
@@ -233,7 +233,7 @@
         self.basic_module = basic_module(in_channels, out_channels, encoder=False, kernel_size=kernel_size,
                                          order=conv_layer_order, num_groups=num_groups)
 
-    def forward(self, encoder_features, x, head_next=False):
+    def forward(self, encoder_features, x, head_next=False, head=None):
         with config.exact_products(_module_kinked(self.basic_module)):
             if self.upsample is None:
                 bm = self.basic_module
@@ -245,7 +245,7 @@
             else:
                 x = self.upsample(x, skip=encoder_features)
             if head_next and isinstance(self.basic_module, ExtResNetBlock):
-                return self.basic_module(x, head_next=True)
+                return self.basic_module(x, head_next=True, head=head)
             return self.basic_module(x)
 
 
diff --git a/torch-mednet_amd/mednet_hip/unet/model.py b/torch-mednet_amd/mednet_hip/unet/model.py
--- a/torch-mednet_amd/mednet_hip/unet/model.py
+++ b/torch-mednet_amd/mednet_hip/unet/model.py
@@ -107,10 +107,10 @@
         with config.exact_products(kinked):
             return self._forward(x)
 
-    def forward_features(self, x):
+    def forward_features(self, x, head=None):
         kinked = any(getattr(m, "_kinked", False) for m in self.modules())
         with config.exact_products(kinked):
-            return self._features(x)
+            return self._features(x, head=head)
 
     def _forward(self, x):
         x = self.final_conv(self._features(x))
@@ -118,7 +118,7 @@
             x = self.final_activation(x)
         return x
 
-    def _features(self, x, tap=None):
+    def _features(self, x, tap=None, head=None):
         tap = tap if tap is not None else getattr(self, "_ds_tap", None)
         k = self.deep_supervision if tap is not None else 0
         skips = []
@@ -133,7 +133,8 @@
         top = len(self.decoders) - 1
         for i, (dec, skip) in enumerate(zip(self.decoders, skips[1:])):
             if i == top:
-                x = dec(skip, x, head_next=not _has_forward_hooks(dec))
+                head_next = not _has_forward_hooks(dec)
+                x = dec(skip, x, head_next=head_next, head=head) if (head_next and head is not None) else dec(skip, x, head_next=head_next)
                 continue
             x = dec(skip, x)
             if 1 <= top - i <= k:
```

Measured after the change: 214.6 patches/s (median of 6 runs). Within noise of the previous version (+0.7%).
